# Simon-Kotchou/ViT.rs

Measured on AMD Instinct MI355X. Metric: images/sec (train step) ViT-B/16 224² bf16 at 1/2/4/8 MI355X; % MFMA roofline, higher is better.
Workload: dtype bf16; 1 GPU; vit_b16 224x224 train step (fwd+bwd+SGD), batch 256/GPU, bf16; model=vit_b16, global_batch=256, seq_len=197, parallelism=dp1

## Files before the change

include/vit_ops.h:

```cpp
#ifndef VIT_OPS_H
#define VIT_OPS_H

#include <stddef.h>
#include <stdint.h>

#ifdef __cplusplus
extern "C" {
#endif

int vit_init(int device);
void vit_set_stream(void* hip_stream);
void* vit_get_stream(void);
int vit_sync(void);
int vit_last_error(const char** msg);
void vit_clear_error(void);
void* vit_malloc(size_t bytes);
void vit_free(void* p);
int vit_memcpy_h2d(void* dst, const void* src, size_t bytes);
int vit_memcpy_d2h(void* dst, const void* src, size_t bytes);
int vit_memcpy_d2d(void* dst, const void* src, size_t bytes);
int vit_memset(void* dst, int value, size_t bytes);
enum {
    VIT_HIT_GEMM_128 = 0,
    VIT_HIT_GEMM_256x256 = 16,
    VIT_HIT_GEMM_256x128 = 32,
    VIT_HIT_GEMM_FP8 = 48,
    VIT_HIT_GEMM_F32 = 64,
    VIT_HIT_SPLITK_REDUCE = 80,
    VIT_HIT_ATTN_FWD_MFMA = 81,
    VIT_HIT_ATTN_BWD_PERSISTENT = 82,
    VIT_HIT_ATTN_BWD_ONEPASS = 83,
    VIT_HIT_ATTN_BWD_PAIR = 84,
    VIT_HIT_ATTN_GENERIC = 85,
    VIT_HIT_ATTN_BWD_XKEY = 86,
    VIT_HIT_QUANT_ROWCOL = 87,
    VIT_HIT_GEMM_PP = 88,
    VIT_HIT_LN_MX = 89,
    VIT_HIT_LNB_MX = 90,
    VIT_HIT_AUGMENT = 91,
    VIT_HIT_COUNT = 96
};
int vit_kernel_hits(long long* out, int n);
void vit_kernel_hits_reset(void);
void* vit_event_create(void);
void vit_event_destroy(void* ev);
int vit_event_record(void* ev);
float vit_event_elapsed_ms(void* start, void* stop);

void residual_forward(float* out, const float* inp1, const float* inp2, int N);
void matmul_forward(float* out, const float* inp, const float* weight, const float* bias,
                    int B, int T, int C, int OC);
void attention_forward(float* out, float* preatt, float* att, const float* inp,
                       int B, int T, int C, int NH);
void layernorm_forward(float* out, float* mean, float* rstd, const float* inp,
                       const float* weight, const float* bias, int B, int T, int C);
void gelu_forward(float* out, const float* inp, int N);
void softmax_forward(float* probs, const float* logits, int B, int T, int V);
void crossentropy_forward(float* losses, const float* probs, const int* targets,
                          int B, int T, int V);
void residual_backward(float* dinp1, float* dinp2, const float* dout, int N);
void matmul_backward(float* dinp, float* dweight, float* dbias, const float* dout,
                     const float* inp, const float* weight, int B, int T, int C, int OC);
void attention_backward(float* dinp, float* dpreatt, float* datt, const float* dout,
                        const float* inp, const float* att, int B, int T, int C, int NH);
void layernorm_backward(float* dinp, float* dweight, float* dbias, const float* dout,
                        const float* inp, const float* weight, const float* mean,
                        const float* rstd, int B, int T, int C);
void gelu_backward(float* dinp, const float* inp, const float* dout, int N);
void crossentropy_softmax_backward(float* dlogits, const float* dlosses, const float* probs,
                                   const int* targets, int B, int T, int V);
void softmax_crossentropy_soft_forward(float* probs, float* losses, const float* logits,
                                       const int* ta, const int* tb, float lam, float eps,
                                       int B, int T, int V);
void crossentropy_soft_softmax_backward(float* dlogits, const float* dlosses, const float* probs,
                                        const int* ta, const int* tb, float lam, float eps,
                                        int B, int T, int V);
void patch_embed_forward(float* encoded, const float* pixels, const float* patch_w,
                         const float* patch_b, const float* cls, const float* wpe,
                         int B, int IMG, int P, int C);
void patch_embed_backward(float* dpatch_w, float* dpatch_b, float* dcls, float* dwpe,
                          const float* dencoded, const float* pixels, int B, int IMG, int P,
                          int C);
void sgd_step(float* params, const float* grads, long long n, float lr);
void grad_sumsq(double* out, const float* x, long long n);

void matmul_forward_bf16(uint16_t* out, const uint16_t* inp, const uint16_t* weight,
                         const float* bias, int B, int T, int C, int OC);
void matmul_backward_bf16(float* dinp, float* dweight, float* dbias, const uint16_t* dout,
                          const uint16_t* inp, const uint16_t* weight, int B, int T, int C,
                          int OC);
int vit_attention_kernel_kind(int T, int C, int NH);
void attention_forward_fused_bf16(uint16_t* out, float* lse, const uint16_t* inp,
                                  int B, int T, int C, int NH);
void attention_backward_fused_bf16(uint16_t* dinp, const uint16_t* dout, const uint16_t* inp,
                                   const uint16_t* out, const float* lse, int B, int T, int C,
                                   int NH);
void attention_backward_fused_bf16_ex(uint16_t* dinp, const uint16_t* dout, const uint16_t* inp,
                                      const uint16_t* out, const float* lse, int B, int T, int C, int NH,
                                      float* dqkv_bias);
void layernorm_forward_bf16(uint16_t* out, float* mean, float* rstd, const float* inp,
                            const float* weight, const float* bias, int B, int T, int C);
void layernorm_backward_bf16(float* dinp, float* dweight, float* dbias, const uint16_t* dout,
                             const float* inp, const float* weight, const float* mean,
                             const float* rstd, int B, int T, int C);
void gelu_forward_bf16(uint16_t* out, const uint16_t* inp, int N);
void gelu_backward_bf16(float* dinp, const uint16_t* inp, const uint16_t* dout, int N);
void gemm_bf16_ex(void* C, long long ldc, const uint16_t* A, long long lda, int a_kcontig,
                  const uint16_t* B, long long ldb, int b_kcontig, const float* bias,
                  float* dbias, int M, int N, int K, int epi, int splitk);
void gemm_bf16_fused(void* C, void* C2, long long ldc, const void* aux, long long ldaux,
                     const uint16_t* A, long long lda, int a_kcontig, const uint16_t* B,
                     long long ldb, int b_kcontig, const float* bias, float* colsum_out, int M,
                     int N, int K, int epi);
long long mx_scale_size(long long rows, int K);
void quantize_mx_bf16_ex(uint8_t* q, uint8_t* scales, const uint16_t* x, long long R, int K,
                         long long ldx, long long ldq);
void quantize_mx_f32_ex(uint8_t* q, uint8_t* scales, const float* x, long long R, int K,
                        long long ldx, long long ldq);
long long mx_cols_padded(long long R);
void quantize_mx_cols_bf16_ex(uint8_t* q, uint8_t* scales, const uint16_t* x, long long R, int C,
                              long long ldx);
void quantize_mx_rowcol_bf16_ex(uint8_t* qr, uint8_t* scales_r, uint8_t* qc, uint8_t* scales_c,
                                const uint16_t* x, long long R, int C, long long ldx, long long ldqc,
                                long long tok_off, long long ntok);
void layernorm_backward_stream(uint16_t* dres_out, uint8_t* lo_out, const uint16_t* dres_in, const uint8_t* lo_in,
                               float* dweight, float* dbias, float* dres_colsum, const uint16_t* dout, const float* inp,
                               const float* weight, const float* mean, const float* rstd, long long R, int C);
void layernorm_backward_stream_mx(uint16_t* dres_out, uint8_t* lo_out, const uint16_t* dres_in, const uint8_t* lo_in,
                                  float* dweight, float* dbias, float* dres_colsum, const uint16_t* dout,
                                  const float* inp, const float* weight, const float* mean, const float* rstd,
                                  long long R, int C, uint8_t* qr, uint8_t* scales_r, uint8_t* qc, uint8_t* scales_c,
                                  long long ldqc, long long tok_off, long long ntok);
void layernorm_forward_mx(uint8_t* qr, uint8_t* scales_r, uint8_t* qc, uint8_t* scales_c, float* mean,
                          float* rstd, const float* inp, const float* weight, const float* bias, long long R,
                          int C, long long ldqc, long long tok_off, long long ntok);
void gemm_fp8_fused(void* C, void* C2, long long ldc, const void* aux, long long ldaux,
                    const uint8_t* A, const uint8_t* a_scale, long long lda, const uint8_t* B,
                    const uint8_t* b_scale, long long ldb, const float* bias, float* colsum_out,
                    int M, int N, int K, int epi);
void gemm_fp8_fused_mx(void* C, void* C2, long long ldc, const void* aux, long long ldaux, const uint8_t* A,
                       const uint8_t* a_scale, long long lda, const uint8_t* B, const uint8_t* b_scale,
                       long long ldb, const float* bias, float* colsum_out, int M, int N, int K, int epi,
                       uint8_t* mx_q, uint8_t* mx_s);
void gemm_fp8_fused_mxc(void* C, void* C2, long long ldc, const void* aux, long long ldaux, const uint8_t* A,
                        const uint8_t* a_scale, long long lda, const uint8_t* B, const uint8_t* b_scale,
                        long long ldb, const float* bias, float* colsum_out, int M, int N, int K, int epi,
                        uint8_t* mx_q, uint8_t* mx_s, uint8_t* mxc_q, uint8_t* mxc_s, long long mxc_ld,
                        long long mxc_off);
void gemm_bf16_set_variant(int variant);
void gemm_bf16_set_debug(int flags);
void gemm_bf16_set_trace(unsigned long long* trace);
void convert_f32_to_bf16(uint16_t* out, const float* inp, long long n);
void convert_bf16_to_f32(float* out, const uint16_t* inp, long long n);

#ifdef __cplusplus
}
#endif
#endif
```

vit.rs_amd/__init__.py:

```python
import ctypes
import os
import sys

import numpy as np

HERE = os.path.dirname(os.path.abspath(__file__))
LIB_PATH = os.environ.get("VIT_LIB") or os.path.join(HERE, "libvit_hip.so")

from . import data
from . import mix
from . import groups
from . import augment

VIT_FP32, VIT_BF16, VIT_FP8 = 0, 1, 2
MIX_NONE, MIX_MIXUP, MIX_CUTMIX = 0, 1, 2
_lib = None


class VitError(RuntimeError):
    pass


class VitConfigC(ctypes.Structure):
    _fields_ = [("img", ctypes.c_int), ("patch", ctypes.c_int), ("in_ch", ctypes.c_int),
                ("channels", ctypes.c_int), ("num_layers", ctypes.c_int),
                ("num_heads", ctypes.c_int), ("num_classes", ctypes.c_int)]


class AdamWC(ctypes.Structure):
    _fields_ = [("beta1", ctypes.c_float), ("beta2", ctypes.c_float), ("eps", ctypes.c_float),
                ("weight_decay", ctypes.c_float)]


class CheckpointInfoC(ctypes.Structure):
    _fields_ = [("cfg", VitConfigC), ("num_params", ctypes.c_longlong), ("has_opt", ctypes.c_int),
                ("step", ctypes.c_int), ("adamw", AdamWC)]


def _cfg_c(cfg):
    return VitConfigC(cfg.img, cfg.patch, cfg.in_ch, cfg.channels, cfg.num_layers, cfg.num_heads,
                      cfg.num_classes)


def build(quiet=True):
    import subprocess
    jobs = str(min(8, os.cpu_count() or 1))
    subprocess.run(["make", "-s", "-j", jobs, "-C", HERE], check=True,
                   stdout=subprocess.DEVNULL if quiet else None)


_VOID = [("vit_clear_error", []), ("vit_set_stream", [ctypes.c_void_p]),
         ("vit_free", [ctypes.c_void_p]), ("vit_event_destroy", [ctypes.c_void_p]),
         ("vit_trainer_destroy", [ctypes.c_void_p]), ("vit_trainer_timing_reset", [ctypes.c_void_p]),
         ("vit_loader_close", [ctypes.c_void_p]), ("vit_jpeg_loader_close", [ctypes.c_void_p]), ("vit_kernel_hits_reset", [])]

P, I, LL, F, S = ctypes.c_void_p, ctypes.c_int, ctypes.c_longlong, ctypes.c_float, ctypes.c_size_t
_SIGS = {
    "vit_init": (I, [I]), "vit_get_stream": (P, []), "vit_sync": (I, []),
    "vit_last_error": (I, [ctypes.POINTER(ctypes.c_char_p)]),
    "vit_malloc": (P, [S]), "vit_memcpy_h2d": (I, [P, P, S]), "vit_memcpy_d2h": (I, [P, P, S]),
    "vit_memcpy_d2d": (I, [P, P, S]), "vit_memset": (I, [P, I, S]),
    "vit_event_create": (P, []), "vit_event_record": (I, [P]), "vit_event_elapsed_ms": (F, [P, P]),
    "residual_forward": (None, [P, P, P, I]),
    "matmul_forward": (None, [P, P, P, P, I, I, I, I]),
    "attention_forward": (None, [P, P, P, P, I, I, I, I]),
    "layernorm_forward": (None, [P, P, P, P, P, P, I, I, I]),
    "gelu_forward": (None, [P, P, I]),
    "softmax_forward": (None, [P, P, I, I, I]),
    "crossentropy_forward": (None, [P, P, P, I, I, I]),
    "residual_backward": (None, [P, P, P, I]),
    "matmul_backward": (None, [P, P, P, P, P, P, I, I, I, I]),
    "attention_backward": (None, [P, P, P, P, P, P, I, I, I, I]),
    "layernorm_backward": (None, [P, P, P, P, P, P, P, P, I, I, I]),
    "gelu_backward": (None, [P, P, P, I]),
    "crossentropy_softmax_backward": (None, [P, P, P, P, I, I, I]),
    "softmax_crossentropy_soft_forward": (None, [P, P, P, P, P, F, F, I, I, I]),
    "crossentropy_soft_softmax_backward": (None, [P, P, P, P, P, F, F, I, I, I]),
    "patch_embed_forward": (None, [P, P, P, P, P, P, I, I, I, I]),
    "patch_embed_backward": (None, [P, P, P, P, P, P, I, I, I, I]),
    "sgd_step": (None, [P, P, LL, F]),
    "grad_sumsq": (None, [P, P, LL]),
    "matmul_forward_bf16": (None, [P, P, P, P, I, I, I, I]),
    "matmul_backward_bf16": (None, [P, P, P, P, P, P, I, I, I, I]),
    "attention_forward_fused_bf16": (None, [P, P, P, I, I, I, I]),
    "vit_attention_kernel_kind": (I, [I, I, I]),
    "attention_backward_fused_bf16": (None, [P, P, P, P, P, I, I, I, I]),
    "attention_backward_fused_bf16_ex": (None, [P, P, P, P, P, I, I, I, I, P]),
    "layernorm_forward_bf16": (None, [P, P, P, P, P, P, I, I, I]),
    "layernorm_backward_bf16": (None, [P, P, P, P, P, P, P, P, I, I, I]),
    "gelu_forward_bf16": (None, [P, P, I]),
    "gelu_backward_bf16": (None, [P, P, P, I]),
    "gemm_bf16_ex": (None, [P, LL, P, LL, I, P, LL, I, P, P, I, I, I, I, I]),
    "gemm_bf16_fused": (None, [P, P, LL, P, LL, P, LL, I, P, LL, I, P, P, I, I, I, I]),
    "mx_scale_size": (LL, [LL, I]),
    "quantize_mx_bf16_ex": (None, [P, P, P, LL, I, LL, LL]),
    "quantize_mx_f32_ex": (None, [P, P, P, LL, I, LL, LL]),
    "mx_cols_padded": (LL, [LL]),
    "quantize_mx_cols_bf16_ex": (None, [P, P, P, LL, I, LL]),
    "quantize_mx_rowcol_bf16_ex": (None, [P, P, P, P, P, LL, I, LL, LL, LL, LL]),
    "layernorm_forward_mx": (None, [P, P, P, P, P, P, P, P, P, LL, I, LL, LL, LL]),
    "layernorm_backward_stream": (None, [P, P, P, P, P, P, P, P, P, P, P, P, LL, I]),
    "layernorm_backward_stream_mx": (None, [P, P, P, P, P, P, P, P, P, P, P, P, LL, I, P, P, P, P, LL, LL, LL]),
    "gemm_fp8_fused": (None, [P, P, LL, P, LL, P, P, LL, P, P, LL, P, P, I, I, I, I]),
    "gemm_fp8_fused_mx": (None, [P, P, LL, P, LL, P, P, LL, P, P, LL, P, P, I, I, I, I, P, P]),
    "gemm_fp8_fused_mxc": (None, [P, P, LL, P, LL, P, P, LL, P, P, LL, P, P, I, I, I, I, P, P, P, P, LL, LL]),
    "gemm_bf16_set_variant": (None, [I]), "gemm_bf16_set_debug": (None, [I]),
    "gemm_bf16_set_trace": (None, [P]),
    "vit_kernel_hits": (I, [P, I]),
    "convert_f32_to_bf16": (None, [P, P, LL]),
    "convert_bf16_to_f32": (None, [P, P, LL]),
    "vit_trainer_create": (P, [ctypes.POINTER(VitConfigC), I, I, I]),
    "vit_trainer_num_params": (LL, [P]), "vit_trainer_device_bytes": (LL, [P]),
    "vit_trainer_set_params": (I, [P, P]), "vit_trainer_get_params": (I, [P, P]),
    "vit_trainer_get_grads": (I, [P, P]), "vit_trainer_set_batch": (I, [P, P, P]),
    "vit_trainer_set_batch_device": (I, [P, P, P]),
    "vit_trainer_set_label_smoothing": (I, [P, F]),
    "vit_trainer_mix_batch": (I, [P, I, F, I, I, I, I]),
    "vit_trainer_get_pixels": (I, [P, P]),
    "vit_trainer_forward": (I, [P, I]), "vit_trainer_zero_grad": (I, [P]),
    "vit_trainer_backward": (I, [P]), "vit_trainer_step": (I, [P, F]),
    "vit_trainer_train_step": (I, [P, F, I]), "vit_trainer_mean_loss": (F, [P]),
    "vit_trainer_get_logits": (I, [P, P]), "vit_trainer_sync": (I, [P]),
    "vit_trainer_stream": (P, [P]),
    "vit_layout_query": (I, [ctypes.POINTER(VitConfigC), P, P, ctypes.POINTER(LL)]),
    "vit_dp_unique_id_size": (I, []), "vit_dp_get_unique_id": (I, [ctypes.c_char_p]),
    "vit_trainer_dp_init": (I, [P, I, I, ctypes.c_char_p, I]),
    "vit_trainer_dp_ranks": (I, [P]),
    "vit_trainer_get_dp_snapshot": (I, [P, P]),
    "vit_trainer_set_timing": (I, [P, I]), "vit_trainer_set_concurrency": (I, [P, I]),
    "vit_trainer_set_option": (I, [P, ctypes.c_char_p, I]),
    "vit_trainer_timing": (I, [P, ctypes.POINTER(ctypes.c_char_p), ctypes.POINTER(ctypes.c_double),
                               ctypes.POINTER(ctypes.c_longlong), ctypes.POINTER(ctypes.c_double), I]),
    "vit_trainer_step_adamw": (I, [P, F, F, F, F, F]),
    "vit_trainer_get_adamw_state": (I, [P, P, P, ctypes.POINTER(I)]),
    "vit_trainer_set_grad_clip": (I, [P, F]), "vit_trainer_grad_norm": (F, [P]),
    "vit_trainer_set_param_groups": (I, [P, P, P]),
    "vit_trainer_get_param_groups": (I, [P, P, P, ctypes.POINTER(I)]),
    "vit_trainer_eval": (I, [P, P, ctypes.POINTER(I)]),
    "vit_config_num_params": (LL, [ctypes.POINTER(VitConfigC)]),
    "vit_checkpoint_read_info": (I, [ctypes.c_char_p, P]),
    "vit_checkpoint_write": (I, [ctypes.c_char_p, ctypes.POINTER(VitConfigC), P, P, P, I, P]),
    "vit_checkpoint_read": (I, [ctypes.c_char_p, ctypes.POINTER(VitConfigC), P, P, P]),
    "vit_loader_open": (P, [ctypes.c_char_p, ctypes.c_char_p, I, I, ctypes.c_ulonglong, I, I, I, I, I]),
    "vit_loader_num_records": (LL, [P]), "vit_loader_steps_per_epoch": (I, [P]),
    "vit_loader_next": (I, [P, ctypes.POINTER(P), ctypes.POINTER(P), ctypes.POINTER(LL), ctypes.POINTER(I)]),
    "vit_trainer_set_batch_u8": (I, [P, P, P, P, P]),
    "vit_augment_u8": (I, [P, I, I, P, I, P, P]),
    "vit_randaugment_draw": (I, [ctypes.c_ulonglong, LL, I, I, I, P]),
    "vit_trainer_set_augment_plan": (I, [P, P, I, P]),
    "vit_jpeg_probe": (I, [P, LL, ctypes.POINTER(I), ctypes.POINTER(I), ctypes.POINTER(I)]),
    "vit_jpeg_coefficients": (I, [P, LL, P, LL, P]),
    "vit_jpeg_loader_open": (P, [ctypes.c_char_p, ctypes.c_char_p, ctypes.c_char_p, I, ctypes.c_ulonglong, I, I,
                                 I, I, I, I]),
    "vit_jpeg_loader_num_records": (LL, [P]), "vit_jpeg_loader_steps_per_epoch": (I, [P]),
    "vit_jpeg_loader_next": (I, [P, ctypes.POINTER(P), ctypes.POINTER(LL), ctypes.POINTER(I)]),
    "vit_jpeg_loader_boxes": (I, [P, P]),
    "vit_jpeg_loader_decode_u8": (I, [P, P, I]),
    "vit_trainer_set_batch_jpeg": (I, [P, P, P, P]),
    "vit_jpeg_loader_set_randaugment": (I, [P, I, I, P]),
    "vit_jpeg_loader_plan": (I, [P, I, P, ctypes.POINTER(I)]),
    "vit_trainer_save_checkpoint": (I, [P, ctypes.c_char_p]),
    "vit_trainer_load_checkpoint": (I, [P, ctypes.c_char_p]),
}


def exported_symbols():
    return sorted(set(_SIGS) | {n for n, _ in _VOID})


def lib():
    global _lib
    if _lib is not None:
        return _lib
    if not os.path.exists(LIB_PATH):
        raise VitError(f"{LIB_PATH} not built; run __graft_entry__.build() or make -C vit.rs_amd")
    L = ctypes.CDLL(LIB_PATH, mode=ctypes.RTLD_GLOBAL)
    for name, (res, args) in _SIGS.items():
        if os.environ.get("VIT_LIB") and not hasattr(L, name):
            continue
        f = getattr(L, name)
        f.restype = res
        f.argtypes = args
    for name, args in _VOID:
        f = getattr(L, name)
        f.restype = None
        f.argtypes = args
    _lib = L
    return L


HIT_GEMM_128, HIT_GEMM_256x256, HIT_GEMM_256x128, HIT_GEMM_FP8, HIT_GEMM_F32 = 0, 16, 32, 48, 64
HIT_SPLITK_REDUCE, HIT_ATTN_FWD_MFMA, HIT_ATTN_BWD_PERSISTENT = 80, 81, 82
HIT_ATTN_BWD_ONEPASS, HIT_ATTN_BWD_PAIR, HIT_ATTN_GENERIC = 83, 84, 85
HIT_ATTN_BWD_XKEY, HIT_QUANT_ROWCOL = 86, 87
HIT_GEMM_PP = 88
HIT_LN_MX = 89
HIT_LNB_MX = 90
HIT_AUGMENT = 91


def kernel_hits():
    n = lib().vit_kernel_hits(None, 0)
    out = (ctypes.c_longlong * n)()
    lib().vit_kernel_hits(ctypes.cast(out, ctypes.c_void_p), n)
    return np.array(out[:], dtype=np.int64)


def kernel_hits_reset():
    lib().vit_kernel_hits_reset()


def check(what=""):
    msg = ctypes.c_char_p()
    if lib().vit_last_error(ctypes.byref(msg)):
        text = msg.value.decode() if msg.value else "unknown"
        lib().vit_clear_error()
        raise VitError(f"{what}: {text}" if what else text)


class DeviceArray:

    def __init__(self, shape, dtype):
        self.shape = tuple(shape) if isinstance(shape, (tuple, list)) else (int(shape),)
        self.dtype = np.dtype(dtype)
        self.nbytes = int(np.prod(self.shape)) * self.dtype.itemsize
        self.ptr = lib().vit_malloc(max(self.nbytes, 16))
        if not self.ptr:
            check("vit_malloc")
            raise VitError("vit_malloc returned NULL")

    @classmethod
    def from_numpy(cls, a, dtype=None):
        a = np.ascontiguousarray(a if dtype is None else a.astype(dtype))
        d = cls(a.shape, a.dtype)
        d.upload(a)
        return d

    @classmethod
    def zeros(cls, shape, dtype):
        d = cls(shape, dtype)
        lib().vit_memset(d.ptr, 0, d.nbytes)
        check("vit_memset")
        return d

    def upload(self, a):
        a = np.ascontiguousarray(a, dtype=self.dtype)
# ... 485 lines not shown
```

vit.rs_amd/csrc/gemm.h:

```cpp
#pragma once
#include "common.h"

namespace vit {

enum Epi {
    EPI_F32_STORE = 0,
    EPI_F32_ACC = 1,
    EPI_F32_ATOMIC = 2,
    EPI_BF16_STORE = 3,
    EPI_BF16_GELU = 4,
    EPI_F32_RESID = 5,
    EPI_BF16_DGELU = 6,
    EPI_F32_SLAB = 7,
    EPI_BF16_GELU_D = 8,
    EPI_BF16_MUL = 9,
};
constexpr bool epi_aux16(int e) { return e == EPI_BF16_DGELU || e == EPI_BF16_MUL; }
constexpr bool epi_bias(int e) { return e != EPI_F32_ATOMIC && e != EPI_F32_SLAB && !epi_aux16(e); }
constexpr bool epi_mx(int e) { return e == EPI_BF16_GELU || e == EPI_BF16_GELU_D || epi_aux16(e); }

struct GemmArgs {
    const void* A = nullptr;
    long long lda = 0;
    bool a_kcontig = true;
    const void* B = nullptr;
    long long ldb = 0;
    bool b_kcontig = true;
    void* C = nullptr;
    long long ldc = 0;
    void* C2 = nullptr;
    const void* aux = nullptr;
    long long ldaux = 0;
    const float* bias = nullptr;
    float* dbias = nullptr;
    float* colsum_out = nullptr;
    float* colsum_part = nullptr;
    int M = 0, N = 0, K = 0;
    int epi = EPI_F32_STORE;
    int splitk = 0;
    int fill_pct = 0;
    bool rows_gathered = false;
    float* ws = nullptr;
    size_t ws_bytes = 0;
    const void* a_scale = nullptr;
    const void* b_scale = nullptr;
    uint8_t* mx_q = nullptr;
    uint8_t* mx_s = nullptr;
    uint8_t* mxc_q = nullptr;
    uint8_t* mxc_s = nullptr;
    long long mxc_ld = 0;
    long long mxc_off = 0;
};

void gemm_f32(const GemmArgs& a, hipStream_t s);
void gemm_bf16(const GemmArgs& a, hipStream_t s);
bool gemm_bf16_supported(const GemmArgs& a);
void gemm_set_variant(int v);
void gemm_set_debug(int flags);
int gemm_cu_count();
int gemm_persist_grid();
struct GemmParams;
void gemm_set_trace(unsigned long long* trace);
bool gemm_pp_shape(const GemmArgs& a);
void gemm_bf16_pp(const GemmArgs& a, const GemmParams& p, hipStream_t s);
int gemm_colsum_rows(const GemmArgs& a, bool fp8);
bool gemm_streaming();

void gemm_fp8(const GemmArgs& a, hipStream_t s);
bool gemm_fp8_supported(const GemmArgs& a);
void quantize_mx_bf16(uint8_t* q, uint8_t* sl, const bf16_t* x, long long R, int K, long long ldx,
                      long long ldq, hipStream_t s);
void quantize_mx_f32(uint8_t* q, uint8_t* sl, const float* x, long long R, int K, long long ldx,
                     long long ldq, hipStream_t s);
void quantize_mx_batched_bf16(uint8_t* q, uint8_t* sl, const bf16_t* x, long long R, int K, int count,
                              long long xs, long long qs, long long ss, hipStream_t s);
void quantize_mx_batched_f32(uint8_t* q, uint8_t* sl, const float* x, long long R, int K, int count,
                             long long xs, long long qs, long long ss, hipStream_t s);
void quantize_mx_cols_bf16(uint8_t* q, uint8_t* sl, const bf16_t* x, long long R, int C, long long ldx, hipStream_t s);
void quantize_mx_cols_batched_bf16(uint8_t* q, uint8_t* sl, const bf16_t* x, long long R, int C, long long ldx,
                                   int count, long long xs, long long qs, long long ss, hipStream_t s);
bool quantize_mx_rowcol_bf16(uint8_t* qr, uint8_t* slr, uint8_t* qc, uint8_t* slc, const bf16_t* x, long long R,
                             int C, long long ldx, long long ldqc, long long tok_off, long long ntok, hipStream_t s);
long long mx_cols_kp(long long R);
long long mx_rows_padded(long long rows);
size_t mx_scale_bytes(long long rows, int K);
bool ln_forward_mx_supported(int C);
bool ln_backward_mx_supported(int C);
bool ln_backward_bf16_stream_mx(bf16_t* dres_out, uint8_t* lo_out, const bf16_t* dres_in, const uint8_t* lo_in,
                                float* dw, float* db, float* dres_colsum, const bf16_t* dout, const float* inp,
                                const float* w, const float* mean, const float* rstd, long long R, int C,
                                hipStream_t s, float* part, uint8_t* qr, uint8_t* slr, uint8_t* qc, uint8_t* slc,
                                long long ldqc, long long tok_off, long long ntok, uint8_t* scratch);
size_t ln_backward_mx_scratch_bytes(int C);
bool ln_forward_mx(uint8_t* qr, uint8_t* slr, uint8_t* qc, uint8_t* slc, float* mean, float* rstd, const float* x,
                   const float* w, const float* b, long long R, int C, long long ldqc, long long tok_off, long long ntok,
                   hipStream_t s, uint8_t* scratch);
size_t ln_mx_scratch_bytes(int C);

void colsum_f32(float* dbias, const float* X, int M, int N, long long ld, hipStream_t s, float* ws = nullptr);
void colsum_bf16(float* dbias, const bf16_t* X, int M, int N, long long ld, hipStream_t s, float* ws = nullptr);
struct RowsJob {
    float* dst;
    const float* src;
    int nrows;
    long long ld;
    int ncols;
};
constexpr int ROWS_MAX_JOBS = 8;
void rows_reduce_add(const RowsJob* jobs, int njobs, hipStream_t s);

}
```

vit.rs_amd/csrc/gemm.hip:

```cpp
#include "gemm_common.h"

#include <cstdlib>

#ifndef VIT_G2_ONEPHASE
#define VIT_G2_ONEPHASE 0
#endif

namespace vit {

namespace bf {
constexpr int BM = 128, BN = 128, BK = 64, NT = 256;
constexpr int SK = 72;
constexpr int SMN = 144;
constexpr int TILE = 9216;
static_assert(BM * SK == TILE && BK * SMN == TILE, "image sizes");

template <bool KC, int ROWS>
struct Stager {
    uint4 r[4];
    __device__ __forceinline__ void load(const bf16_t* __restrict__ base, long long ld, int row0,
                                         int rows_lim, int k0, int k_lim, int tid) {
#pragma unroll
        for (int c = 0; c < 4; c++) {
            const int idx = c * NT + tid;
// ... 470 lines not shown
        bar();
        if (lagging) {
            __builtin_amdgcn_s_setprio(1);
            bar();
        }
        for (int kt = 0; kt < nk; kt++) {
            const char* img = smem + sl * SLOT_BYTES;
            const int sl2 = (sl + 2) & 3;
#pragma unroll
            for (int b = 0; b < 4; b++) fb[b] = frag<true>(img + IMG_BYTES, wn * 64 + b * 16, lane);
#pragma unroll
            for (int a = 0; a < 4; a++) alo[a] = frag<true>(img, wm * 128 + a * 16, lane);
#if VIT_G2_ONEPHASE
#pragma unroll
            for (int a = 0; a < 4; a++) ahi[a] = frag<true>(img, wm * 128 + (4 + a) * 16, lane);
            issue_a(kt + 2, sl2, more);
            issue_b(kt + 2, sl2, more);
            if (kt > 0 || j == 0) {
                if (kt + 2 < nk || more) wait_vm(4);
                else wait_vm(0);
            }
            bar();
            mfma_half(0, alo, fb);
            mfma_half(1, ahi, fb);
            bar();
            sl = (sl + 1) & 3;
            continue;
#endif
            issue_a(kt + 2, sl2, more);
            bar();
            mfma_half(0, alo, fb);
            bar();
#pragma unroll
            for (int a = 0; a < 4; a++) ahi[a] = frag<true>(img, wm * 128 + (4 + a) * 16, lane);
            if (kt > 0 || j == 0) {
                if (kt + 2 < nk || more) wait_vm(2);
                else wait_vm(0);
            }
            issue_b(kt + 2, sl2, more);
            bar();
            mfma_half(1, ahi, fb);
            bar();
            sl = (sl + 1) & 3;
        }
        if (!lagging) bar();
        if (p.trace && tid == 0) p.trace[(long long)cur.t * TRACE_WORDS + 1] = __builtin_amdgcn_s_memrealtime();
        float bpre[8];
        staged_bias_prefetch<EPI>(p, lane, cur.tn0 + wn * 64, bpre);
#if VIT_G2_EPI_WAIT_ASM
        asm volatile("s_waitcnt vmcnt(0) lgkmcnt(0)" ::: "memory");
#else
        __builtin_amdgcn_s_waitcnt(0x0070);
#endif
        __builtin_amdgcn_s_setprio(0);
        __builtin_amdgcn_s_barrier();
        asm volatile("" ::: "memory");
        if (!skip_epilogue(p, acc)) {
            char* stg = smem + ((wave < 4 ? sl + 2 : sl + 3) & 3) * SLOT_BYTES + (wave & 3) * 8192;
            staged_epilogue_q<EPI>(p, acc, reinterpret_cast<float*>(stg), lane, cur.tm0 + wm * 128,
                                   cur.tn0 + wn * 64, bpre);
        }
        if (p.trace && (tid & 63) == 0) {
            const long long rec = (long long)cur.t * TRACE_WORDS;
            const unsigned long long t = __builtin_amdgcn_s_memrealtime();
            p.trace[rec + 4 + wave] = t;
            if (wave == 0) {
                p.trace[rec + 2] = t;
                p.trace[rec + 3] = ((unsigned long long)__builtin_amdgcn_s_getreg((31 << 11) | 20) << 32) |
                                   __builtin_amdgcn_s_getreg((31 << 11) | 4);
            }
        }
        if (p.dbg & 16) asm volatile("s_waitcnt vmcnt(0)" ::: "memory");
        zero_acc();
        if (more) tile_src(j + 1, cur);
        if (j + 2 < my_tiles) tile_src(j + 2, nxt);
    }
}

}

namespace g4 {
constexpr int BM = 256, BN = 128, BK = 32, NT = 256;
constexpr int NSLOT = 3;
constexpr int A_BYTES = BM * BK * 2;
constexpr int B_BYTES = BN * BK * 2;
constexpr int SLOT_BYTES = A_BYTES + B_BYTES;
constexpr int KTILE = BK;
constexpr int PIECES = BM / 64 + BN / 64;
static_assert(PIECES == 6, "vmcnt literal below");
static_assert(NSLOT * SLOT_BYTES >= 4 * STG_WAVE_BYTES, "staged epilogue area");

template <int R>
__device__ __forceinline__ int mn_swz(int k) {
    if constexpr (R == 256) return ((k & 3) << 2) | (((k >> 3) & 1) << 1);
    else return ((k & 3) << 1) | (((k >> 3) & 1) << 3);
}

template <int R>
__device__ __forceinline__ void stage(const bf16_t* __restrict__ base, long long ld, int row0,
                                      int rows_lim, int k0, char* img, int wave, int lane) {
#pragma unroll
    for (int j = 0; j < R / 64; j++) {
        const int blk = j * 4 + wave;
        constexpr int CPR = R / 8;
        constexpr int KPB = 64 / CPR;
        const int k = blk * KPB + lane / CPR;
        const int c = (lane % CPR) ^ mn_swz<R>(k);
        const int gc = min(row0 + c * 8, rows_lim - 8);
        const bf16_t* src = base + (long long)(k0 + k) * ld + gc;
        __builtin_amdgcn_global_load_lds((const __attribute__((address_space(1))) void*)src,
                                         (__attribute__((address_space(3))) void*)(img + blk * 1024),
                                         16, 0, 0);
    }
}

template <int R>
__device__ __forceinline__ bf16x8_t frag(const char* img, int r0, int lane) {
    const int i = lane & 15, g = lane >> 4;
    const int q = i >> 2, p = i & 3;
    const int ch = (r0 >> 3) + (p >> 1);
    const int k0 = 8 * g + q, k1 = k0 + 4;
    (void)k1;
    const char* a0 = img + k0 * (2 * R) + ((ch ^ mn_swz<R>(k0)) << 4) + (p & 1) * 8;
    const bf16x4_t lo = ds_read_tr16_asm<0>(a0);
    const bf16x4_t hi = ds_read_tr16_asm<4 * 2 * R>(a0);
    return __builtin_shufflevector(lo, hi, 0, 1, 2, 3, 4, 5, 6, 7);
}

__device__ __forceinline__ void group_order(int t, int ntm, int ntn, int& tm, int& tn) {
    constexpr int GM = 8;
    const int per = GM * ntn;
    const int grp = t / per;
    const int first = grp * GM;
    const int gsz = min(GM, ntm - first);
    const int r = t - grp * per;
    tm = first + r % gsz;
    tn = r / gsz;
}

template <int EPI>
__global__ __launch_bounds__(NT, 2) void gemm_kernel(GemmParams p) {
    __shared__ __attribute__((aligned(1024))) char smem[NSLOT * SLOT_BYTES];
    first_round_stagger(p.stagger);
    const int tid = threadIdx.x, lane = tid & 63;
    const int wave = __builtin_amdgcn_readfirstlane(tid >> 6);
    const int wm = wave >> 1, wn = wave & 1;
    const int ntm = cdiv(p.M, BM), ntn = cdiv(p.N, BN);
    int tm, tn, wg, split;
    split_remap(ntm * ntn, wg, split);
    group_order(wg, ntm, ntn, tm, tn);
    const int tm0 = tm * BM, tn0 = tn * BN;
    const int kbeg = split * p.kchunk;
    const int kend = min(p.K, kbeg + p.kchunk);
    const int nk = (kend - kbeg) / BK;
    const bf16_t* A = (const bf16_t*)p.A;
    const bf16_t* B = (const bf16_t*)p.B;

    f32x4_t acc[8][4];
#pragma unroll
    for (int a = 0; a < 8; a++)
#pragma unroll
        for (int b = 0; b < 4; b++) acc[a][b] = f32x4_t{0.f, 0.f, 0.f, 0.f};

    auto issue = [&](int st) {
        char* sl = smem + (st % NSLOT) * SLOT_BYTES;
        const int k0 = kbeg + st * BK;
        stage<BM>(A, p.lda, tm0, p.M, k0, sl, wave, lane);
        stage<BN>(B, p.ldb, tn0, p.N, k0, sl + A_BYTES, wave, lane);
    };
    if (nk > 0) issue(0);
    if (nk > 1) issue(1);
    for (int kt = 0; kt < nk; kt++) {
        __builtin_amdgcn_sched_barrier(0);
        if (kt + 1 < nk) asm volatile("s_waitcnt vmcnt(6)" ::: "memory");
        else asm volatile("s_waitcnt vmcnt(0)" ::: "memory");
        asm volatile("s_waitcnt lgkmcnt(0)" ::: "memory");
        __builtin_amdgcn_s_barrier();
        asm volatile("" ::: "memory");
        __builtin_amdgcn_sched_barrier(0);
        if (kt + 2 < nk) issue(kt + 2);
        const char* img = smem + (kt % NSLOT) * SLOT_BYTES;
        bf16x8_t fa[8], fb[4];
#pragma unroll
        for (int b = 0; b < 4; b++) fb[b] = frag<BN>(img + A_BYTES, wn * 64 + b * 16, lane);
#pragma unroll
        for (int a = 0; a < 8; a++) fa[a] = frag<BM>(img, wm * 128 + a * 16, lane);
        __builtin_amdgcn_sched_barrier(0);
        asm volatile("s_waitcnt lgkmcnt(0)" ::: "memory");
        __builtin_amdgcn_sched_barrier(0);
#pragma unroll
        for (int a = 0; a < 8; a++)
#pragma unroll
            for (int b = 0; b < 4; b++)
                acc[a][b] = __builtin_amdgcn_mfma_f32_16x16x32_bf16(fb[b], fa[a], acc[a][b], 0, 0, 0);
    }

    if (skip_epilogue(p, acc)) return;
    asm volatile("s_waitcnt vmcnt(0) lgkmcnt(0)" ::: "memory");
    __builtin_amdgcn_s_barrier();
    asm volatile("" ::: "memory");
    staged_epilogue<EPI>(p, acc, smem + wave * STG_WAVE_BYTES, lane, tm0 + wm * 128, tn0 + wn * 64);
}
}

namespace f32 {
constexpr int BM = 64, BN = 64, BK = 16, NT = 256, S = 80;

template <int EPI>
__global__ __launch_bounds__(NT) void gemm_f32_kernel(GemmParams p, int a_kc, int b_kc) {
    __shared__ float As[BK * S];
    __shared__ float Bs[BK * S];
    const int tid = threadIdx.x, lane = tid & 63, wave = tid >> 6;
    const int wm = wave >> 1, wn = wave & 1;
    const int ntm = cdiv(p.M, BM), ntn = cdiv(p.N, BN);
    const int wg = blockIdx.x;
    const int tm0 = (wg / ntn) * BM, tn0 = (wg % ntn) * BN;
    (void)ntm;
    const int kbeg = blockIdx.y * p.kchunk;
    const int kend = min(p.K, kbeg + p.kchunk);
    const float* A = (const float*)p.A;
    const float* B = (const float*)p.B;
    f32x4_t acc[2][2];
#pragma unroll
    for (int a = 0; a < 2; a++)
#pragma unroll
        for (int b = 0; b < 2; b++) acc[a][b] = f32x4_t{0.f, 0.f, 0.f, 0.f};

    for (int k0 = kbeg; k0 < kend; k0 += BK) {
#pragma unroll
        for (int e = 0; e < 4; e++) {
            const int idx = e * NT + tid;
            int m, k;
            if (a_kc) { m = idx >> 4; k = idx & 15; } else { k = idx >> 6; m = idx & 63; }
            const int gm = tm0 + m, gk = k0 + k;
            float v = 0.f;
            if (gm < p.M && gk < kend)
                v = a_kc ? A[(long long)gm * p.lda + gk] : A[(long long)gk * p.lda + gm];
            As[k * S + m] = v;
            int n;
            if (b_kc) { n = idx >> 4; k = idx & 15; } else { k = idx >> 6; n = idx & 63; }
            const int gn = tn0 + n;
            const int gk2 = k0 + k;
            float w = 0.f;
            if (gn < p.N && gk2 < kend)
                w = b_kc ? B[(long long)gn * p.ldb + gk2] : B[(long long)gk2 * p.ldb + gn];
            Bs[k * S + n] = w;
        }
        __syncthreads();
#pragma unroll
        for (int kk = 0; kk < BK / 4; kk++) {
            const int kr = kk * 4 + (lane >> 4);
            float af[2], bfv[2];
#pragma unroll
            for (int t = 0; t < 2; t++) {
                af[t] = As[kr * S + wm * 32 + t * 16 + (lane & 15)];
                bfv[t] = Bs[kr * S + wn * 32 + t * 16 + (lane & 15)];
            }
#pragma unroll
            for (int a = 0; a < 2; a++)
#pragma unroll
                for (int b = 0; b < 2; b++)
                    acc[a][b] = __builtin_amdgcn_mfma_f32_16x16x4f32(af[a], bfv[b], acc[a][b], 0, 0, 0);
        }
        __syncthreads();
    }
#pragma unroll
    for (int a = 0; a < 2; a++)
#pragma unroll
        for (int b = 0; b < 2; b++)
#pragma unroll
            for (int r = 0; r < 4; r++) {
                const int m = tm0 + wm * 32 + a * 16 + (lane >> 4) * 4 + r;
                const int n = tn0 + wn * 32 + b * 16 + (lane & 15);
                if (m >= p.M || n >= p.N) continue;
                float v = acc[a][b][r];
                float* q = (float*)p.C + (long long)m * p.ldc + n;
                if constexpr (EPI == EPI_F32_STORE) {
                    *q = p.bias ? v + p.bias[n] : v;
                } else if constexpr (EPI == EPI_F32_ACC) {
                    *q += p.bias ? v + p.bias[n] : v;
                } else {
                    q[(long long)blockIdx.y * p.M * p.ldc] = v;
                }
            }
}
}

template <typename TX>
__global__ __launch_bounds__(256) void colsum_part_k(float* __restrict__ out, const TX* __restrict__ X, int M, int N,
                                                     long long ld, int rpb, int add_direct) {
    const int n = blockIdx.x * 256 + threadIdx.x;
    const int r0 = blockIdx.y * rpb;
    const int r1 = min(M, r0 + rpb);
    if (n >= N) return;
    float s = 0.f;
    for (int r = r0; r < r1; r++) {
        if constexpr (sizeof(TX) == 2)
            s += bf2f(X[(long long)r * ld + n]);
        else
            s += X[(long long)r * ld + n];
    }
    if (add_direct) out[n] += s;
    else out[(long long)blockIdx.y * N + n] = s;
}

struct RowsJobs {
    RowsJob j[ROWS_MAX_JOBS];
    int blk0[ROWS_MAX_JOBS + 1];
    int vec;
};
__global__ __launch_bounds__(256) void rows_reduce_k(RowsJobs jobs) {
    __shared__ float4 red[16][17];
    int jb = 0;
#pragma unroll 1
    while (jb + 1 < ROWS_MAX_JOBS && (int)blockIdx.x >= jobs.blk0[jb + 1]) jb++;
    const RowsJob& J = jobs.j[jb];
    const int c0 = (blockIdx.x - jobs.blk0[jb]) * 64;
    if (jobs.vec) {
        const int q = threadIdx.x & 15, ph = threadIdx.x >> 4, c = c0 + 4 * q;
        float4 s0 = make_float4(0.f, 0.f, 0.f, 0.f), s1 = s0;
        if (c < J.ncols) {
            const float* base = J.src + c;
            int r = ph;
            for (; r + 16 < J.nrows; r += 32) {
                const float4 a = *reinterpret_cast<const float4*>(base + (long long)r * J.ld);
                const float4 b = *reinterpret_cast<const float4*>(base + (long long)(r + 16) * J.ld);
                s0.x += a.x; s0.y += a.y; s0.z += a.z; s0.w += a.w;
                s1.x += b.x; s1.y += b.y; s1.z += b.z; s1.w += b.w;
            }
            if (r < J.nrows) {
                const float4 a = *reinterpret_cast<const float4*>(base + (long long)r * J.ld);
                s0.x += a.x; s0.y += a.y; s0.z += a.z; s0.w += a.w;
            }
        }
        red[ph][q] = make_float4(s0.x + s1.x, s0.y + s1.y, s0.z + s1.z, s0.w + s1.w);
        __syncthreads();
        if (threadIdx.x < 64) {
            const int qq = threadIdx.x >> 2, e = threadIdx.x & 3, cc = c0 + threadIdx.x;
            float t = 0.f;
#pragma unroll
            for (int p = 0; p < 16; p++) t += reinterpret_cast<const float*>(&red[p][qq])[e];
            if (cc < J.ncols) J.dst[cc] += t;
        }
        return;
    }
    float* reds = reinterpret_cast<float*>(red);
    const int c = c0 + (threadIdx.x & 63), ph = threadIdx.x >> 6;
    float s0 = 0.f, s1 = 0.f;
    if (c < J.ncols) {
        int r = ph;
        for (; r + 4 < J.nrows; r += 8) {
            s0 += J.src[(long long)r * J.ld + c];
            s1 += J.src[(long long)(r + 4) * J.ld + c];
        }
        if (r < J.nrows) s0 += J.src[(long long)r * J.ld + c];
    }
    reds[ph * 64 + (threadIdx.x & 63)] = s0 + s1;
    __syncthreads();
    if (ph == 0 && c < J.ncols)
        J.dst[c] += ((reds[threadIdx.x] + reds[64 + threadIdx.x]) + reds[128 + threadIdx.x]) + reds[192 + threadIdx.x];
}
void rows_reduce_add(const RowsJob* jobs, int njobs, hipStream_t s) {
    for (int b = 0; b < njobs; b += ROWS_MAX_JOBS) {
        RowsJobs J{};
        J.vec = 1;
        int nb = 0, k = 0;
        for (; k < ROWS_MAX_JOBS && b + k < njobs; k++) {
            const RowsJob& x = jobs[b + k];
            J.j[k] = x;
            J.blk0[k] = nb;
            nb += x.nrows > 0 ? cdiv(x.ncols, 64) : 0;
            if (x.nrows > 0 && ((x.ncols | x.ld) % 4 || ((uintptr_t)x.src & 15))) J.vec = 0;
        }
        for (; k <= ROWS_MAX_JOBS; k++) J.blk0[k] = nb;
        if (nb == 0) continue;
        rows_reduce_k<<<nb, 256, 0, s>>>(J);
        after_launch("rows_reduce_add");
    }
}
template <typename TX>
static void colsum_any(float* dbias, const TX* X, int M, int N, long long ld, hipStream_t s, float* ws) {
    if (M <= 0 || N <= 0) return;
    if constexpr (sizeof(TX) == 4) {
        if (M <= 1024) {
            RowsJob j{dbias, X, M, ld, N};
            rows_reduce_add(&j, 1, s);
            return;
        }
    }
    const int rpb = 256, nch = cdiv(M, rpb);
    if (nch == 1) {
        colsum_part_k<TX><<<dim3(cdiv(N, 256), 1), 256, 0, s>>>(dbias, X, M, N, ld, rpb, 1);
        after_launch("colsum");
        return;
    }
    if (!ws) ws = (float*)workspace((size_t)nch * N * sizeof(float));
    if (!ws) return;
    colsum_part_k<TX><<<dim3(cdiv(N, 256), nch), 256, 0, s>>>(ws, X, M, N, ld, rpb, 0);
    after_launch("colsum");
    RowsJob j{dbias, ws, nch, N, N};
    rows_reduce_add(&j, 1, s);
}
static int gemm_variant();
static int g_debug_flags_fwd();
static bool pp_all() { return (g_debug_flags_fwd() & 512) != 0; }
static bool pp_taken(const GemmArgs& a) {
    return gemm_variant() == 11 && !a.a_scale && a.epi != EPI_F32_ATOMIC && gemm_bf16_supported(a) &&
           a.K % g2::KTILE == 0 && a.M >= 256 && a.N >= 256 && (a.N <= 1280 || pp_all()) && gemm_pp_shape(a);
}
int gemm_colsum_rows(const GemmArgs& a, bool fp8) { return cdiv(a.M, !fp8 && pp_taken(a) ? 96 : 128); }
float* colsum_rows_begin(const GemmArgs& a) {
    if (!epi_aux16(a.epi) || !(a.colsum_out || a.colsum_part)) return nullptr;
    float* r = a.colsum_part ? a.colsum_part
                             : (float*)workspace((size_t)gemm_colsum_rows(a, a.a_scale != nullptr) * a.N * sizeof(float));
    return r;
}
void colsum_rows_end(const GemmArgs& a, float* rows, hipStream_t s) {
    if (!rows || !a.colsum_out) return;
    RowsJob j{a.colsum_out, rows, gemm_colsum_rows(a, a.a_scale != nullptr), a.N, a.N};
    rows_reduce_add(&j, 1, s);
}

__global__ __launch_bounds__(256) void slab_reduce1_k(float* __restrict__ C, long long ldc,
                                                      const float* __restrict__ slab, int M, int N,
                                                      int splits) {
    const long long n1 = (long long)M * N;
    for (long long e = blockIdx.x * 256LL + threadIdx.x; e < n1; e += (long long)gridDim.x * 256) {
        const int m = (int)(e / N), n = (int)(e - (long long)m * N);
        float acc = slab[e];
        for (int z = 1; z < splits; z++) acc += slab[z * n1 + e];
        C[(long long)m * ldc + n] += acc;
    }
}
__global__ __launch_bounds__(256) void slab_reduce_k(float* __restrict__ C, long long ldc,
                                                     const float* __restrict__ slab, int M, int N,
                                                     int splits) {
    const long long n4 = (long long)M * N / 4;
    const long long plane = (long long)M * N;
    for (long long i = blockIdx.x * 256LL + threadIdx.x; i < n4; i += (long long)gridDim.x * 256) {
        const long long e = i * 4;
        const int m = (int)(e / N), n = (int)(e - (long long)m * N);
        float4 acc = reinterpret_cast<const float4*>(slab)[i];
        for (int z = 1; z < splits; z++) {
            const float4 t = *reinterpret_cast<const float4*>(slab + z * plane + e);
            acc.x += t.x; acc.y += t.y; acc.z += t.z; acc.w += t.w;
        }
        float4* c = reinterpret_cast<float4*>(C + (long long)m * ldc + n);
        float4 o = *c;
        o.x += acc.x; o.y += acc.y; o.z += acc.z; o.w += acc.w;
        *c = o;
    }
}

static int g_variant = -1;
static int g_debug_flags = 0;
static bool known_variant(int v) { return v == 1 || v == 2 || v == 7 || v == 11; }
static constexpr int kDefaultVariant = 7;
static int gemm_variant() {
    if (g_variant < 0) {
        const char* e = getenv("VIT_GEMM");
        g_variant = e ? atoi(e) : kDefaultVariant;
        if (!known_variant(g_variant)) g_variant = kDefaultVariant;
    }
    return g_variant;
}
void gemm_set_variant(int v) { g_variant = known_variant(v) ? v : -1; }
int gemm_cu_count() {
    static int n = [] {
        int dev = 0, cu = 0;
        (void)hipGetDevice(&dev);
        (void)hipDeviceGetAttribute(&cu, hipDeviceAttributeMultiprocessorCount, dev);
        return cu > 0 ? cu : 256;
    }();
    return n;
}
int gemm_persist_grid() {
    static const int n = [] {
        const char* e = getenv("VIT_PERSIST_CUS");
        const int v = e ? atoi(e) : 0;
        return v >= 64 && v <= gemm_cu_count() ? v : gemm_cu_count();
    }();
    return n;
}
bool gemm_streaming() { return gemm_variant() == 7 || gemm_variant() == 11; }
void gemm_set_debug(int flags) { g_debug_flags = flags; }
static int g_debug_flags_fwd() { return g_debug_flags; }
static unsigned long long* g_trace = nullptr;
void gemm_set_trace(unsigned long long* trace) { g_trace = trace; }

GemmParams make_gemm_params(const GemmArgs& a, int kchunk) {
    GemmParams p;
    p.A = a.A; p.B = a.B; p.C = a.C; p.C2 = a.C2; p.aux = a.aux; p.bias = a.bias; p.dbias = a.dbias; p.colsum_out = nullptr;
    p.lda = a.lda; p.ldb = a.ldb; p.ldc = a.ldc; p.ldaux = a.ldaux;
    if (g_debug_flags & 32) p.ldc = 0;
    p.M = a.M; p.N = a.N; p.K = a.K; p.kchunk = kchunk;
    p.no_epi = (g_debug_flags & 2) ? 1 : 0;
    p.dbg = g_debug_flags & 0xF0;
    static const int gm_env = [] {
        const char* e = getenv("VIT_GEMM_GM");
        return e && *e ? atoi(e) : -1;
    }();
    const int gm_dbg = (g_debug_flags >> 16) & 0xF;
    p.gm = gm_dbg ? gm_dbg - 1 : gm_env >= 0 ? gm_env : (a.K <= 768 ? 8 : 0);
    p.stagger = ((g_debug_flags >> 8) & 0xFF) * 50;
    p.trace = g_trace;
    p.mx_q = a.mx_q;
    p.mx_s = a.mx_s;
    p.mx_rg = (int)(mx_rows_padded(a.M) / 32);
    p.mxc_q = a.mxc_q;
    p.mxc_s = a.mxc_s;
    p.mxc_ld = a.mxc_ld;
    p.mxc_off = (int)a.mxc_off;
    p.mxc_rg = (int)(mx_rows_padded(a.N) / 32);
    p.tiles = 1;
    return p;
}

int choose_split_waves(int tiles, int nk) {
    const int slots = 256;
    int best = 1;
    double best_eff = 0.0;
    for (int s = 1; s <= 32 && nk / s >= 16; s++) {
        const int blocks = tiles * s;
        const int waves = (blocks + slots - 1) / slots;
        const double eff = (double)blocks / (waves * (double)slots) * (blocks >= slots / 2 ? 1.0 : blocks / (slots / 2.0));
        if (eff > best_eff + 1e-9) { best_eff = eff; best = s; }
        if (eff >= 0.9) break;
    }
    return best;
}

static int choose_split(int tiles, int K, int ktile, int want_blocks) {
    int nk = cdiv(K, ktile);
    int s = 1;
    while (tiles * s < want_blocks && nk / (s * 2) >= 8) s *= 2;
    return s;
}

static int grid_blocks(long long n) {
    long long b = (n + 255) / 256;
    return (int)(b < 1 ? 1 : (b > 4096 ? 4096 : b));
}
float* slab_buffer(const GemmArgs& a, int split) {
    const size_t need = (size_t)split * a.M * a.N * sizeof(float);
    float* slab = a.ws ? (a.ws_bytes >= need ? a.ws : nullptr) : (float*)workspace(need);
    if (!slab) set_error("gemm: split-K workspace of %zu bytes unavailable", need);
    return slab;
}
void slab_reduce(const GemmArgs& a, float* slab, int split, hipStream_t s) {
    if (a.N % 4 == 0)
        slab_reduce_k<<<grid_blocks((long long)a.M * a.N / 4), 256, 0, s>>>((float*)a.C, a.ldc, slab, a.M, a.N, split);
    else
        slab_reduce1_k<<<grid_blocks((long long)a.M * a.N), 256, 0, s>>>((float*)a.C, a.ldc, slab, a.M, a.N, split);
    after_launch("gemm_slab_reduce");
    count_hit(VIT_HIT_SPLITK_REDUCE);
}

void gemm_f32(const GemmArgs& a, hipStream_t s) {
    if (a.M <= 0 || a.N <= 0) return;
    if (a.mx_q || a.mxc_q) {
        set_error("gemm_f32: the fused MX output is an fp8-engine feature");
        return;
    }
    const int tiles = cdiv(a.M, f32::BM) * cdiv(a.N, f32::BN);
    int split = 1;
    if (a.epi == EPI_F32_ATOMIC) split = a.splitk > 0 ? a.splitk : choose_split(tiles, a.K, f32::BK, 512);
    int kchunk = cdiv(cdiv(a.K, split), f32::BK) * f32::BK;
    if (kchunk <= 0) kchunk = f32::BK;
    split = cdiv(a.K > 0 ? a.K : 1, kchunk);
    GemmArgs b = a;
    float* slab = nullptr;
    if (a.epi == EPI_F32_ATOMIC) {
        if (split > 1) {
            if (!(slab = slab_buffer(a, split))) return;
            b.epi = EPI_F32_SLAB; b.C = slab; b.ldc = a.N;
        } else {
            b.epi = EPI_F32_ACC;
        }
    }
    GemmParams p = make_gemm_params(b, kchunk);
    dim3 grid(tiles, split);
    int akc = a.a_kcontig, bkc = a.b_kcontig;
    switch (b.epi) {
        case EPI_F32_STORE: f32::gemm_f32_kernel<EPI_F32_STORE><<<grid, f32::NT, 0, s>>>(p, akc, bkc); break;
        case EPI_F32_ACC: f32::gemm_f32_kernel<EPI_F32_ACC><<<grid, f32::NT, 0, s>>>(p, akc, bkc); break;
        case EPI_F32_SLAB: f32::gemm_f32_kernel<EPI_F32_SLAB><<<grid, f32::NT, 0, s>>>(p, akc, bkc); break;
        default: set_error("gemm_f32: unsupported epilogue %d", a.epi); return;
    }
    after_launch("gemm_f32");
    count_hit(VIT_HIT_GEMM_F32 + b.epi);
    if (slab) slab_reduce(a, slab, split, s);
}

bool gemm_bf16_supported(const GemmArgs& a) {
    auto al16 = [](const void* q) { return ((uintptr_t)q & 15) == 0; };
    if ((a.a_kcontig || a.b_kcontig) && a.K % 8) return false;
    if (a.lda % 8 || a.ldb % 8 || a.N % 4 || a.ldc % 4) return false;
    if (!al16(a.A) || !al16(a.B)) return false;
    if (!a.a_kcontig && a.M % 8) return false;
    if (!a.b_kcontig && a.N % 8) return false;
    return true;
}

template <bool AK, bool BKC>
static void launch_bf16(const GemmArgs& a, const GemmParams& p, dim3 grid, hipStream_t s) {
    switch (a.epi) {
#define VIT_CASE(E) \
    case E: bf::gemm_bf16_kernel<AK, BKC, E><<<grid, bf::NT, 0, s>>>(p); break;
        VIT_CASE(EPI_F32_STORE)
        VIT_CASE(EPI_F32_ACC)
        VIT_CASE(EPI_F32_SLAB)
        VIT_CASE(EPI_BF16_STORE)
        VIT_CASE(EPI_BF16_GELU)
        VIT_CASE(EPI_F32_RESID)
        VIT_CASE(EPI_BF16_DGELU)
        VIT_CASE(EPI_BF16_GELU_D)
        VIT_CASE(EPI_BF16_MUL)
#undef VIT_CASE
        default: set_error("gemm_bf16: unsupported epilogue %d", a.epi); return;
    }
}

template <bool AK, bool BKC>
static void launch_g2(const GemmArgs& a, const GemmParams& p, dim3 grid, hipStream_t s) {
    if constexpr (AK && BKC) {
        if ((gemm_variant() == 7 || gemm_variant() == 11) && grid.y == 1 && p.K >= 2 * g2::BK &&
            (long long)p.M * p.lda * 2 < (1LL << 31) &&
            (long long)p.N * p.ldb * 2 < (1LL << 31)) {
            const int cus = gemm_persist_grid();
            const dim3 pg((int)grid.x < cus ? grid.x : cus);
            switch (a.epi) {
#define VIT_CASE(E) \
    case E: g2::gemm_kernel_s<E><<<pg, g2::NT, 0, s>>>(p); return;
                VIT_CASE(EPI_F32_STORE)
                VIT_CASE(EPI_F32_ACC)
                VIT_CASE(EPI_BF16_STORE)
                VIT_CASE(EPI_BF16_GELU)
                VIT_CASE(EPI_F32_RESID)
                VIT_CASE(EPI_BF16_DGELU)
                VIT_CASE(EPI_BF16_GELU_D)
                VIT_CASE(EPI_BF16_MUL)
#undef VIT_CASE
                default: break;
            }
        }
    }
    switch (a.epi) {
#define VIT_CASE(E) \
    case E: g2::gemm_kernel<AK, BKC, E, 2><<<grid, g2::NT, 0, s>>>(p); break;
        VIT_CASE(EPI_F32_STORE)
        VIT_CASE(EPI_F32_ACC)
        VIT_CASE(EPI_BF16_STORE)
        VIT_CASE(EPI_BF16_GELU)
        VIT_CASE(EPI_F32_RESID)
        VIT_CASE(EPI_BF16_DGELU)
        VIT_CASE(EPI_F32_SLAB)
        VIT_CASE(EPI_BF16_GELU_D)
        VIT_CASE(EPI_BF16_MUL)
#undef VIT_CASE
        default: set_error("gemm_bf16: unsupported epilogue %d", a.epi); return;
    }
}

static int choose_split_g4(int tiles, int nk, int fill_pct = 0) {
    static const int slots = [] {
        const char* e = getenv("VIT_G4_SLOTS");
        const int v = e ? atoi(e) : 512;
        return v >= 64 && v <= 2048 ? v : 512;
    }();
    static const bool one_round = [] {
        const char* e = getenv("VIT_G4_RULE");
        return !(e && e[0] == '0');
    }();
    static const double fill = [] {
        const char* e = getenv("VIT_G4_FILL");
        const int v = e ? atoi(e) : 45;
        return (v >= 20 && v <= 100 ? v : 45) / 100.0;
    }();
    if (one_round) {
        const double f = fill_pct > 0 ? fill_pct / 100.0 : fill;
        const int s1 = (int)((f * slots + tiles - 1) / tiles);
        if (s1 >= 1 && (long long)tiles * s1 <= slots && nk / s1 >= 32) return s1;
    }
    int best = 1;
    double best_eff = 0.0;
    for (int s = 1; s <= 64 && nk / s >= 32; s++) {
        const int blocks = tiles * s;
        const int rounds = (blocks + slots - 1) / slots;
        const double eff = (double)blocks / (rounds * (double)slots) * (blocks >= slots / 2 ? 1.0 : blocks / (slots / 2.0));
        if (eff > best_eff + 1e-9) { best_eff = eff; best = s; }
        if (eff >= 0.9) break;
    }
    return best;
}

static void gemm_bf16_g4(const GemmArgs& a, hipStream_t s) {
    const int tiles = cdiv(a.M, g4::BM) * cdiv(a.N, g4::BN);
    int split = a.splitk > 0 ? a.splitk : choose_split_g4(tiles, a.K / g4::KTILE, a.fill_pct);
    int kchunk = cdiv(cdiv(a.K, split), g4::KTILE) * g4::KTILE;
    split = cdiv(a.K, kchunk);
    GemmArgs b = a;
    float* slab = nullptr;
    if (split > 1) {
        if (!(slab = slab_buffer(a, split))) return;
        b.epi = EPI_F32_SLAB;
        b.C = slab;
        b.ldc = a.N;
    } else {
        b.epi = EPI_F32_ACC;
    }
    GemmParams p = make_gemm_params(b, kchunk);
    p.tiles = tiles;
    dim3 grid(tiles, split);
    if (slab) g4::gemm_kernel<EPI_F32_SLAB><<<grid, g4::NT, 0, s>>>(p);
    else g4::gemm_kernel<EPI_F32_ACC><<<grid, g4::NT, 0, s>>>(p);
    after_launch("gemm_bf16_256x128");
    count_hit(VIT_HIT_GEMM_256x128 + b.epi);
    if (slab) slab_reduce(a, slab, split, s);
    if (a.dbias) colsum_bf16(a.dbias, (const bf16_t*)a.A, a.K, a.M, a.lda, s);
}

void gemm_bf16(const GemmArgs& a, hipStream_t s) {
    if (a.M <= 0 || a.N <= 0) return;
    if (a.mx_q || a.mxc_q) {
        set_error("gemm_bf16: the fused MX output is an fp8-engine feature");
        return;
    }
    if (!gemm_bf16_supported(a)) {
        set_error("gemm_bf16: unsupported shape/alignment M=%d N=%d K=%d lda=%lld ldb=%lld",
                  a.M, a.N, a.K, a.lda, a.ldb);
        return;
    }
    if (gemm_variant() != 1 && a.epi == EPI_F32_ATOMIC && !a.a_kcontig && !a.b_kcontig &&
        a.K % g4::KTILE == 0 && a.M >= 256 && a.N >= 128 && a.N % 4 == 0 &&
        (a.splitk > 0 || !a.ws ||
         (size_t)choose_split_g4(cdiv(a.M, g4::BM) * cdiv(a.N, g4::BN), a.K / g4::KTILE) * a.M * a.N * sizeof(float) <=
             a.ws_bytes)) {
        gemm_bf16_g4(a, s);
        return;
    }
    const bool gathered = a.rows_gathered && a.M >= 1 && a.a_kcontig && a.epi != EPI_F32_ATOMIC;
    const bool big = a.K % g2::KTILE == 0 && (a.M >= 256 || gathered) && a.N >= 256 && gemm_variant() != 1;
    if (big) {
        const int tiles = cdiv(a.M, g2::BM) * cdiv(a.N, g2::BN);
        int split = 1;
        if (a.epi == EPI_F32_ATOMIC) split = a.splitk > 0 ? a.splitk : choose_split_waves(tiles, a.K / g2::KTILE);
        int kchunk = cdiv(cdiv(a.K, split), g2::KTILE) * g2::KTILE;
        split = cdiv(a.K, kchunk);
        GemmArgs b = a;
        float* slab = nullptr;
        if (a.epi == EPI_F32_ATOMIC) {
            if (split > 1) {
                if (!(slab = slab_buffer(a, split))) return;
                b.epi = EPI_F32_SLAB;
                b.C = slab;
                b.ldc = a.N;
            } else {
                b.epi = EPI_F32_ACC;
            }
        }
        GemmParams p = make_gemm_params(b, kchunk);
        p.tiles = tiles;
        float* cs_rows = colsum_rows_begin(a);
        if ((a.colsum_out || a.colsum_part) && epi_aux16(a.epi) && !cs_rows) return;
        p.colsum_out = cs_rows;
        const bool late_db = a.dbias && !a.a_kcontig && split > 1;
        if (late_db) p.dbias = nullptr;
        if (split == 1 && pp_taken(b)) {
            gemm_bf16_pp(b, p, s);
            after_launch("gemm_bf16_pp");
            count_hit(VIT_HIT_GEMM_256x256 + b.epi);
            count_hit(VIT_HIT_GEMM_PP);
            colsum_rows_end(a, cs_rows, s);
            return;
        }
        dim3 grid(tiles, split);
        if (a.a_kcontig && a.b_kcontig) launch_g2<true, true>(b, p, grid, s);
        else if (a.a_kcontig && !a.b_kcontig) launch_g2<true, false>(b, p, grid, s);
        else if (!a.a_kcontig && !a.b_kcontig) launch_g2<false, false>(b, p, grid, s);
        else launch_g2<false, true>(b, p, grid, s);
        after_launch("gemm_bf16_256");
        count_hit(VIT_HIT_GEMM_256x256 + b.epi);
        if (slab) slab_reduce(a, slab, split, s);
        colsum_rows_end(a, cs_rows, s);
        if (late_db) colsum_bf16(a.dbias, (const bf16_t*)a.A, a.K, a.M, a.lda, s);
        return;
    }
    const int tiles = cdiv(a.M, bf::BM) * cdiv(a.N, bf::BN);
    int split = 1;
    if (a.epi == EPI_F32_ATOMIC) split = a.splitk > 0 ? a.splitk : choose_split(tiles, a.K, bf::BK, 512);
    int kchunk = cdiv(cdiv(a.K, split), bf::BK) * bf::BK;
    if (kchunk <= 0) kchunk = bf::BK;
    split = cdiv(a.K > 0 ? a.K : 1, kchunk);
    GemmArgs b = a;
    float* slab = nullptr;
    if (a.epi == EPI_F32_ATOMIC) {
        if (split > 1) {
            if (!(slab = slab_buffer(a, split))) return;
            b.epi = EPI_F32_SLAB; b.C = slab; b.ldc = a.N;
        } else {
            b.epi = EPI_F32_ACC;
        }
    }
    GemmParams p = make_gemm_params(b, kchunk);
    const bool late_db = a.dbias && !a.a_kcontig && split > 1;
    if (late_db) p.dbias = nullptr;
    dim3 grid(tiles, split);
    if (a.a_kcontig && a.b_kcontig) launch_bf16<true, true>(b, p, grid, s);
    else if (a.a_kcontig && !a.b_kcontig) launch_bf16<true, false>(b, p, grid, s);
    else if (!a.a_kcontig && !a.b_kcontig) launch_bf16<false, false>(b, p, grid, s);
    else launch_bf16<false, true>(b, p, grid, s);
    after_launch("gemm_bf16");
    count_hit(VIT_HIT_GEMM_128 + b.epi);
    if (slab) slab_reduce(a, slab, split, s);
    if (late_db) colsum_bf16(a.dbias, (const bf16_t*)a.A, a.K, a.M, a.lda, s);
    if ((a.colsum_out || a.colsum_part) && epi_aux16(a.epi)) {
        float* rows = colsum_rows_begin(a);
        if (!rows) return;
        colsum_part_k<bf16_t><<<dim3(cdiv(a.N, 256), cdiv(a.M, 128)), 256, 0, s>>>(
            rows, (const bf16_t*)a.C, a.M, a.N, a.ldc, 128, 0);
        after_launch("colsum_rows");
        colsum_rows_end(a, rows, s);
    }
}

void colsum_f32(float* dbias, const float* X, int M, int N, long long ld, hipStream_t s, float* ws) {
    colsum_any(dbias, X, M, N, ld, s, ws);
}
void colsum_bf16(float* dbias, const bf16_t* X, int M, int N, long long ld, hipStream_t s, float* ws) {
    colsum_any(dbias, X, M, N, ld, s, ws);
}

}
```

vit.rs_amd/csrc/gemm_common.h:

```cpp
#pragma once
#include "gemm.h"

namespace vit {

struct GemmParams {
    const void* A;
    const void* B;
    void* C;
    void* C2;
    const void* aux;
    const float* bias;
    float* dbias;
    float* colsum_out;
    long long lda, ldb, ldc, ldaux;
    int M, N, K;
    int kchunk;
    int no_epi;
    int dbg;
    int stagger;
    unsigned long long* trace;
    int tiles;
    int gm;
    uint8_t* mx_q;
    uint8_t* mx_s;
    int mx_rg;
    uint8_t* mxc_q;
    uint8_t* mxc_s;
    long long mxc_ld;
    int mxc_off, mxc_rg;
};

__device__ __forceinline__ int mx_scale_byte(float amax) {
    if (!(amax > 0.f)) return 127;
    const uint32_t u = __float_as_uint(amax);
    const int e = (int)((u >> 23) & 0xff), mant = (int)(u & 0x7fffff);
    int s = e - 8 + (mant > 0x600000 ? 1 : 0);
    return s < 0 ? 0 : (s > 254 ? 254 : s);
}
__device__ __forceinline__ void mx_out8(const GemmParams& p, int m, int n, uint32_t w0, uint32_t w1, uint32_t w2,
                                        uint32_t w3, int lane) {
    const uint32_t w[4] = {w0, w1, w2, w3};
    float v[8];
#pragma unroll
    for (int e = 0; e < 4; e++) {
        v[2 * e] = __uint_as_float(w[e] << 16);
        v[2 * e + 1] = __uint_as_float(w[e] & 0xffff0000u);
    }
    float amax = 0.f;
#pragma unroll
    for (int j = 0; j < 8; j++) amax = fmaxf(amax, fabsf(v[j]));
    amax = fmaxf(amax, __shfl_xor(amax, 1, 64));
    amax = fmaxf(amax, __shfl_xor(amax, 2, 64));
    const int sb = mx_scale_byte(amax);
    if ((lane & 3) == 0) {
        const int kb = n >> 5;
        p.mx_s[((long long)(kb >> 1) * p.mx_rg + (m >> 5)) * 64 + (kb & 1) * 32 + (m & 31)] = (uint8_t)sb;
    }
    const float inv = __uint_as_float((uint32_t)(254 - sb) << 23);
    int t0 = __builtin_amdgcn_cvt_pk_fp8_f32(v[0] * inv, v[1] * inv, 0, false);
    t0 = __builtin_amdgcn_cvt_pk_fp8_f32(v[2] * inv, v[3] * inv, t0, true);
    int t1 = __builtin_amdgcn_cvt_pk_fp8_f32(v[4] * inv, v[5] * inv, 0, false);
    t1 = __builtin_amdgcn_cvt_pk_fp8_f32(v[6] * inv, v[7] * inv, t1, true);
    *reinterpret_cast<uint2*>(p.mx_q + (long long)m * p.N + n) = make_uint2((uint32_t)t0, (uint32_t)t1);
}

__device__ __forceinline__ void stage_back8(float* w, uint32_t w0, uint32_t w1, uint32_t w2, uint32_t w3) {
    typedef float f4 __attribute__((ext_vector_type(4)));
    *reinterpret_cast<f4*>(w) = f4{__uint_as_float(w0 << 16), __uint_as_float(w0 & 0xffff0000u),
                                   __uint_as_float(w1 << 16), __uint_as_float(w1 & 0xffff0000u)};
    *reinterpret_cast<f4*>(w + 4) = f4{__uint_as_float(w2 << 16), __uint_as_float(w2 & 0xffff0000u),
                                       __uint_as_float(w3 << 16), __uint_as_float(w3 & 0xffff0000u)};
}

float* colsum_rows_begin(const GemmArgs& a);
void colsum_rows_end(const GemmArgs& a, float* rows, hipStream_t s);
int choose_split_waves(int tiles, int nk);
float* slab_buffer(const GemmArgs& a, int split);
void slab_reduce(const GemmArgs& a, float* slab, int split, hipStream_t s);

__device__ __forceinline__ void split_remap(int tiles, int& tile, int& split) {
    const int nwg = gridDim.x * gridDim.y;
    const int l = xcd_remap(blockIdx.y * gridDim.x + blockIdx.x, nwg);
    split = l / tiles;
    tile = l - split * tiles;
}
__device__ __forceinline__ int split_index(int tiles) {
    int t, s;
    split_remap(tiles, t, s);
    return s;
}

typedef unsigned int epi_u32x4 __attribute__((ext_vector_type(4)));
__device__ __forceinline__ void epi_st16(const GemmParams&, void* q, epi_u32x4 v) {
    *reinterpret_cast<epi_u32x4*>(q) = v;
}
__device__ __forceinline__ epi_u32x4 epi_ld16(const GemmParams&, const void* q) {
    return *reinterpret_cast<const epi_u32x4*>(q);
}

__device__ __forceinline__ void first_round_stagger(int ticks, bool one_per_cu = false) {
    if (ticks <= 0) return;
    const int lin = blockIdx.y * gridDim.x + blockIdx.x;
    if (one_per_cu ? (lin >= 256 || !((lin >> 3) & 1)) : (lin < 256 || lin >= 512)) return;
    const uint64_t t0 = __builtin_amdgcn_s_memrealtime();
    while (__builtin_amdgcn_s_memrealtime() - t0 < (uint64_t)ticks) __builtin_amdgcn_s_sleep(8);
}

constexpr int TRACE_WORDS = 16;
__device__ __forceinline__ void trace_stamp(const GemmParams& p, int k) {
    if (!p.trace || (threadIdx.x & 63) != 0) return;
    const int w = threadIdx.x >> 6;
    if (w != 0 && k != 2) return;
    const long long rec = ((long long)blockIdx.y * gridDim.x + blockIdx.x) * TRACE_WORDS;
    const unsigned long long t = __builtin_amdgcn_s_memrealtime();
    if (k == 2) {
        p.trace[rec + 4 + w] = t;
        if (w != 0) return;
        const unsigned hw = __builtin_amdgcn_s_getreg((31 << 11) | 4);
        const unsigned xcc = __builtin_amdgcn_s_getreg((31 << 11) | 20);
        p.trace[rec + 3] = ((unsigned long long)xcc << 32) | hw;
    }
    p.trace[rec + k] = t;
}

template <int NA, int NB>
__device__ __forceinline__ bool skip_epilogue(const GemmParams& p, f32x4_t (&acc)[NA][NB]) {
    if (!(p.no_epi & 1)) return false;
#pragma unroll
    for (int a = 0; a < NA; a++)
#pragma unroll
        for (int b = 0; b < NB; b++) asm volatile("" ::"v"(acc[a][b]));
    return true;
}

template <int EPI>
__device__ __forceinline__ void epilogue(const GemmParams& p, int m, int n, f32x4_t& v) {
    static_assert(EPI != EPI_F32_ATOMIC, "split-K partials go through slabs");
    if constexpr (epi_bias(EPI)) {
        if (p.bias) {
            const float4 bb = *reinterpret_cast<const float4*>(p.bias + n);
            v[0] += bb.x; v[1] += bb.y; v[2] += bb.z; v[3] += bb.w;
        }
    }
    const long long off = (long long)m * p.ldc + n;
    if constexpr (EPI == EPI_F32_STORE) {
        *reinterpret_cast<float4*>((float*)p.C + off) = make_float4(v[0], v[1], v[2], v[3]);
    } else if constexpr (EPI == EPI_F32_ACC) {
        float4* q = reinterpret_cast<float4*>((float*)p.C + off);
        float4 o = *q;
        o.x += v[0]; o.y += v[1]; o.z += v[2]; o.w += v[3];
        *q = o;
    } else if constexpr (EPI == EPI_BF16_STORE) {
        *reinterpret_cast<uint2*>((bf16_t*)p.C + off) =
            make_uint2(pack_bf16x2(v[0], v[1]), pack_bf16x2(v[2], v[3]));
    } else if constexpr (EPI == EPI_BF16_GELU) {
        *reinterpret_cast<uint2*>((bf16_t*)p.C + off) =
            make_uint2(pack_bf16x2(v[0], v[1]), pack_bf16x2(v[2], v[3]));
        *reinterpret_cast<uint2*>((bf16_t*)p.C2 + off) =
            make_uint2(pack_bf16x2(gelu_fast_f(v[0]), gelu_fast_f(v[1])),
                       pack_bf16x2(gelu_fast_f(v[2]), gelu_fast_f(v[3])));
    } else if constexpr (EPI == EPI_F32_RESID) {
        const float4 r = *reinterpret_cast<const float4*>((const float*)p.aux +
                                                          (long long)m * p.ldaux + n);
        *reinterpret_cast<float4*>((float*)p.C + off) =
            make_float4(v[0] + r.x, v[1] + r.y, v[2] + r.z, v[3] + r.w);
    } else if constexpr (EPI == EPI_F32_SLAB) {
        float* slab = (float*)p.C + (long long)split_index(p.tiles) * p.M * p.ldc;
        *reinterpret_cast<float4*>(slab + off) = make_float4(v[0], v[1], v[2], v[3]);
    } else if constexpr (EPI == EPI_BF16_GELU_D) {
        float g[4], d[4];
#pragma unroll
        for (int j = 0; j < 4; j++) gelu_pair_fast_f(v[j], g[j], d[j]);
        *reinterpret_cast<uint2*>((bf16_t*)p.C + off) = make_uint2(pack_bf16x2(d[0], d[1]), pack_bf16x2(d[2], d[3]));
        *reinterpret_cast<uint2*>((bf16_t*)p.C2 + off) = make_uint2(pack_bf16x2(g[0], g[1]), pack_bf16x2(g[2], g[3]));
    } else if constexpr (epi_aux16(EPI)) {
#pragma clang fp contract(off)
        const uint2 h = *reinterpret_cast<const uint2*>((const bf16_t*)p.aux +
                                                        (long long)m * p.ldaux + n);
        const float x0 = __uint_as_float(h.x << 16), x1 = __uint_as_float(h.x & 0xffff0000u);
        const float x2 = __uint_as_float(h.y << 16), x3 = __uint_as_float(h.y & 0xffff0000u);
        if constexpr (EPI == EPI_BF16_DGELU) {
            v[0] *= gelu_grad_fast_f(x0); v[1] *= gelu_grad_fast_f(x1);
            v[2] *= gelu_grad_fast_f(x2); v[3] *= gelu_grad_fast_f(x3);
        } else {
            v[0] *= x0; v[1] *= x1; v[2] *= x2; v[3] *= x3;
        }
        *reinterpret_cast<uint2*>((bf16_t*)p.C + off) =
            make_uint2(pack_bf16x2(v[0], v[1]), pack_bf16x2(v[2], v[3]));
    }
}

template <int EPI, bool MX = true>
__device__ __forceinline__ void epilogue8(const GemmParams& p, int m, int n, float (&v)[8],
                                          float (&cs)[8], int lane = 0, float* wb = nullptr) {
    if constexpr (epi_bias(EPI)) {
        if (p.bias) {
            const float4 b0 = *reinterpret_cast<const float4*>(p.bias + n);
            const float4 b1 = *reinterpret_cast<const float4*>(p.bias + n + 4);
            v[0] += b0.x; v[1] += b0.y; v[2] += b0.z; v[3] += b0.w;
            v[4] += b1.x; v[5] += b1.y; v[6] += b1.z; v[7] += b1.w;
        }
    }
    const long long off = (long long)m * p.ldc + n;
    auto st_f32 = [&](float* q) {
        reinterpret_cast<float4*>(q)[0] = make_float4(v[0], v[1], v[2], v[3]);
        reinterpret_cast<float4*>(q)[1] = make_float4(v[4], v[5], v[6], v[7]);
    };
    auto pack8 = [&](const float (&w)[8]) {
        return make_uint4(pack_bf16x2(w[0], w[1]), pack_bf16x2(w[2], w[3]), pack_bf16x2(w[4], w[5]),
                          pack_bf16x2(w[6], w[7]));
    };
    if constexpr (EPI == EPI_F32_STORE) {
        st_f32((float*)p.C + off);
    } else if constexpr (EPI == EPI_F32_ACC) {
        float* q = (float*)p.C + off;
        const float4 o0 = reinterpret_cast<const float4*>(q)[0];
        const float4 o1 = reinterpret_cast<const float4*>(q)[1];
        v[0] += o0.x; v[1] += o0.y; v[2] += o0.z; v[3] += o0.w;
        v[4] += o1.x; v[5] += o1.y; v[6] += o1.z; v[7] += o1.w;
        st_f32(q);
    } else if constexpr (EPI == EPI_F32_SLAB) {
        st_f32((float*)p.C + (long long)split_index(p.tiles) * p.M * p.ldc + off);
    } else if constexpr (EPI == EPI_BF16_STORE) {
        *reinterpret_cast<uint4*>((bf16_t*)p.C + off) = pack8(v);
    } else if constexpr (EPI == EPI_BF16_GELU) {
        float gv[8];
#pragma unroll
        for (int j = 0; j < 8; j++) gv[j] = gelu_fast_f(v[j]);
        *reinterpret_cast<uint4*>((bf16_t*)p.C + off) = pack8(v);
        const uint4 g8 = pack8(gv);
        if (p.C2) *reinterpret_cast<uint4*>((bf16_t*)p.C2 + off) = g8;
        if constexpr (MX) {
            if (p.mx_q) mx_out8(p, m, n, g8.x, g8.y, g8.z, g8.w, lane);
            if (wb) stage_back8(wb, g8.x, g8.y, g8.z, g8.w);
        }
    } else if constexpr (EPI == EPI_F32_RESID) {
        const float* r = (const float*)p.aux + (long long)m * p.ldaux + n;
        const float4 r0 = reinterpret_cast<const float4*>(r)[0];
        const float4 r1 = reinterpret_cast<const float4*>(r)[1];
        v[0] += r0.x; v[1] += r0.y; v[2] += r0.z; v[3] += r0.w;
        v[4] += r1.x; v[5] += r1.y; v[6] += r1.z; v[7] += r1.w;
        st_f32((float*)p.C + off);
    } else if constexpr (EPI == EPI_BF16_GELU_D) {
        float gv[8], dv[8];
#pragma unroll
        for (int j = 0; j < 8; j++) gelu_pair_fast_f(v[j], gv[j], dv[j]);
        *reinterpret_cast<uint4*>((bf16_t*)p.C + off) = pack8(dv);
        const uint4 g8 = pack8(gv);
        if (p.C2) *reinterpret_cast<uint4*>((bf16_t*)p.C2 + off) = g8;
        if constexpr (MX) {
            if (p.mx_q) mx_out8(p, m, n, g8.x, g8.y, g8.z, g8.w, lane);
            if (wb) stage_back8(wb, g8.x, g8.y, g8.z, g8.w);
        }
    } else if constexpr (epi_aux16(EPI)) {
        const uint4 h = *reinterpret_cast<const uint4*>((const bf16_t*)p.aux + (long long)m * p.ldaux + n);
        const uint32_t hw[4] = {h.x, h.y, h.z, h.w};
        {
#pragma clang fp contract(off)
#pragma unroll
        for (int j = 0; j < 4; j++) {
            const float lo = __uint_as_float(hw[j] << 16), hi = __uint_as_float(hw[j] & 0xffff0000u);
            if constexpr (EPI == EPI_BF16_DGELU) {
                v[2 * j] *= gelu_grad_fast_f(lo);
                v[2 * j + 1] *= gelu_grad_fast_f(hi);
            } else {
                v[2 * j] *= lo;
                v[2 * j + 1] *= hi;
            }
        }
#pragma unroll
        for (int j = 0; j < 8; j++) cs[j] += v[j];
        }
        const uint4 d8 = pack8(v);
        if (p.C) *reinterpret_cast<uint4*>((bf16_t*)p.C + off) = d8;
        if constexpr (MX) {
            if (p.mx_q) mx_out8(p, m, n, d8.x, d8.y, d8.z, d8.w, lane);
            if (wb) stage_back8(wb, d8.x, d8.y, d8.z, d8.w);
        }
    }
}

constexpr int STG_LD = 68;
constexpr int STG_WAVE_BYTES = 64 * STG_LD * 4;
typedef unsigned int epi_u32x4v __attribute__((ext_vector_type(4)));
template <int EPI>
struct EpiAux {
    static constexpr bool AUX16 = epi_aux16(EPI);
    static constexpr bool AUX32 = EPI == EPI_F32_RESID || EPI == EPI_F32_ACC;
    static constexpr int N = AUX16 ? 8 : (AUX32 ? 16 : 0);
    epi_u32x4v ax[N > 0 ? N : 1];
    __device__ __forceinline__ void load(const GemmParams& p, int rr, int mrow, int n) {
        if constexpr (AUX16) {
#pragma unroll
            for (int it = 0; it < 8; it++)
                ax[it] = epi_ld16(p, (const bf16_t*)p.aux + (long long)(mrow + it * 8 + rr) * p.ldaux + n);
        } else if constexpr (AUX32) {
            const float* src = EPI == EPI_F32_RESID ? (const float*)p.aux : (const float*)p.C;
            const long long ld = EPI == EPI_F32_RESID ? p.ldaux : p.ldc;
#pragma unroll
            for (int it = 0; it < 8; it++) {
                const float* q = src + (long long)(mrow + it * 8 + rr) * ld + n;
                ax[2 * it] = epi_ld16(p, q);
                ax[2 * it + 1] = epi_ld16(p, q + 4);
            }
        }
    }
};
template <int EPI>
__device__ __forceinline__ void staged_pass_interior(const GemmParams& p, const float* st, int rr,
                                                     int cc, int mrow, int n, float (&cs)[8],
                                                     const float* bpre, const EpiAux<EPI>* pre = nullptr) {
    const int cc_lane = cc >> 3;
    typedef unsigned int u32x4 __attribute__((ext_vector_type(4)));
    float bv[8] = {0.f, 0.f, 0.f, 0.f, 0.f, 0.f, 0.f, 0.f};
    if constexpr (epi_bias(EPI)) {
        if (bpre) {
#pragma unroll
            for (int j = 0; j < 8; j++) bv[j] = bpre[j];
        } else if (p.bias) {
            const float4 b0 = *reinterpret_cast<const float4*>(p.bias + n);
            const float4 b1 = *reinterpret_cast<const float4*>(p.bias + n + 4);
            bv[0] = b0.x; bv[1] = b0.y; bv[2] = b0.z; bv[3] = b0.w;
            bv[4] = b1.x; bv[5] = b1.y; bv[6] = b1.z; bv[7] = b1.w;
        }
    }
    constexpr bool AUX16 = epi_aux16(EPI);
    constexpr bool AUX32 = EPI == EPI_F32_RESID || EPI == EPI_F32_ACC;
    EpiAux<EPI> own;
    if (!pre) own.load(p, rr, mrow, n);
    const u32x4* ax = pre ? pre->ax : own.ax;
    float* slab = nullptr;
    if constexpr (EPI == EPI_F32_SLAB) slab = (float*)p.C + (long long)split_index(p.tiles) * p.M * p.ldc;
#pragma unroll
    for (int it = 0; it < 8; it++) {
        const int r = it * 8 + rr;
        const f32x4_t lo = *reinterpret_cast<const f32x4_t*>(st + r * STG_LD + cc);
        const f32x4_t hi = *reinterpret_cast<const f32x4_t*>(st + r * STG_LD + cc + 4);
        float v[8] = {lo[0], lo[1], lo[2], lo[3], hi[0], hi[1], hi[2], hi[3]};
        const long long off = (long long)(mrow + r) * p.ldc + n;
#pragma unroll
        for (int j = 0; j < 8; j++) v[j] += bv[j];
        auto pack8 = [](const float (&w)[8]) {
            return u32x4{pack_bf16x2(w[0], w[1]), pack_bf16x2(w[2], w[3]), pack_bf16x2(w[4], w[5]),
                         pack_bf16x2(w[6], w[7])};
        };
        auto st_f32 = [&](float* q) {
            epi_st16(p, q, u32x4{__float_as_uint(v[0]), __float_as_uint(v[1]), __float_as_uint(v[2]), __float_as_uint(v[3])});
            epi_st16(p, q + 4, u32x4{__float_as_uint(v[4]), __float_as_uint(v[5]), __float_as_uint(v[6]), __float_as_uint(v[7])});
        };
        if constexpr (EPI == EPI_F32_STORE) {
            st_f32((float*)p.C + off);
        } else if constexpr (EPI == EPI_F32_SLAB) {
            st_f32(slab + off);
        } else if constexpr (AUX32) {
#pragma unroll
            for (int j = 0; j < 4; j++) {
                v[j] += __uint_as_float(ax[2 * it][j]);
                v[4 + j] += __uint_as_float(ax[2 * it + 1][j]);
            }
            st_f32((float*)p.C + off);
        } else if constexpr (EPI == EPI_BF16_STORE) {
            epi_st16(p, (bf16_t*)p.C + off, pack8(v));
        } else if constexpr (EPI == EPI_BF16_GELU) {
            float gv[8];
#pragma unroll
            for (int j = 0; j < 8; j++) gv[j] = gelu_fast_f(v[j]);
            epi_st16(p, (bf16_t*)p.C + off, pack8(v));
            const u32x4 g8 = pack8(gv);
            if (p.C2) epi_st16(p, (bf16_t*)p.C2 + off, g8);
            if (p.mx_q) mx_out8(p, mrow + r, n, g8[0], g8[1], g8[2], g8[3], cc_lane);
            if (p.mxc_q) stage_back8(const_cast<float*>(st) + r * STG_LD + cc, g8[0], g8[1], g8[2], g8[3]);
        } else if constexpr (EPI == EPI_BF16_GELU_D) {
            float gv[8], dv[8];
#pragma unroll
            for (int j = 0; j < 8; j++) gelu_pair_fast_f(v[j], gv[j], dv[j]);
            epi_st16(p, (bf16_t*)p.C + off, pack8(dv));
            const u32x4 g8 = pack8(gv);
            if (p.C2) epi_st16(p, (bf16_t*)p.C2 + off, g8);
            if (p.mx_q) mx_out8(p, mrow + r, n, g8[0], g8[1], g8[2], g8[3], cc_lane);
            if (p.mxc_q) stage_back8(const_cast<float*>(st) + r * STG_LD + cc, g8[0], g8[1], g8[2], g8[3]);
        } else if constexpr (AUX16) {
#pragma clang fp contract(off)
#pragma unroll
            for (int j = 0; j < 4; j++) {
                const float lo = __uint_as_float(ax[it][j] << 16), hi = __uint_as_float(ax[it][j] & 0xffff0000u);
                if constexpr (EPI == EPI_BF16_DGELU) {
                    v[2 * j] *= gelu_grad_fast_f(lo);
                    v[2 * j + 1] *= gelu_grad_fast_f(hi);
                } else {
                    v[2 * j] *= lo;
                    v[2 * j + 1] *= hi;
                }
            }
#pragma unroll
            for (int j = 0; j < 8; j++) cs[j] += v[j];
            const u32x4 d8 = pack8(v);
            if (p.C) epi_st16(p, (bf16_t*)p.C + off, d8);
            if (p.mx_q) mx_out8(p, mrow + r, n, d8[0], d8[1], d8[2], d8[3], cc_lane);
            if (p.mxc_q) stage_back8(const_cast<float*>(st) + r * STG_LD + cc, d8[0], d8[1], d8[2], d8[3]);
        }
    }
}

GemmParams make_gemm_params(const GemmArgs& a, int kchunk);

template <int EPI>
__device__ __forceinline__ void staged_pass(const GemmParams& p, const float* st, int lane, int m0,
                                            int n0, int pass, bool interior, float (&cs)[8],
                                            const float* bpre = nullptr, const EpiAux<EPI>* pre = nullptr) {
    const int rr = lane >> 3, cc = (lane & 7) * 8;
    if (interior) {
        staged_pass_interior<EPI>(p, st, rr, cc, m0 + pass * 64, n0 + cc, cs, bpre, pre);
        return;
    }
#pragma unroll
    for (int it = 0; it < 8; it++) {
        const int r = it * 8 + rr;
        float v[8];
        const f32x4_t lo = *reinterpret_cast<const f32x4_t*>(st + r * STG_LD + cc);
        const f32x4_t hi = *reinterpret_cast<const f32x4_t*>(st + r * STG_LD + cc + 4);
        v[0] = lo[0]; v[1] = lo[1]; v[2] = lo[2]; v[3] = lo[3];
        v[4] = hi[0]; v[5] = hi[1]; v[6] = hi[2]; v[7] = hi[3];
        const int m = m0 + pass * 64 + r, n = n0 + cc;
        if (m >= p.M) continue;
        if (n + 8 <= p.N) {
            epilogue8<EPI>(p, m, n, v, cs, lane,
                           epi_mx(EPI) && p.mxc_q ? const_cast<float*>(st) + r * STG_LD + cc : nullptr);
        } else if (n + 4 <= p.N) {
            f32x4_t t = lo;
            epilogue<EPI>(p, m, n, t);
            if constexpr (epi_aux16(EPI)) {
#pragma clang fp contract(off)
                cs[0] += t[0];
                cs[1] += t[1];
                cs[2] += t[2];
                cs[3] += t[3];
            }
        }
    }
}
__device__ __forceinline__ void mx_cols_pass(const GemmParams& p, const float* st, int lane, int mrow, int n0) {
    if (mrow >= p.M) return;
    typedef unsigned int u32x4 __attribute__((ext_vector_type(4)));
    const int c = n0 + lane;
#pragma unroll
    for (int b = 0; b < 2; b++) {
        float v[32];
        float amax = 0.f;
#pragma unroll
        for (int i = 0; i < 32; i++) {
            v[i] = st[(32 * b + i) * STG_LD + lane];
            amax = fmaxf(amax, fabsf(v[i]));
        }
        const int sb = mx_scale_byte(amax);
        const int tok = p.mxc_off + mrow + 32 * b, kb = tok >> 5;
        p.mxc_s[((long long)(kb >> 1) * p.mxc_rg + (c >> 5)) * 64 + (kb & 1) * 32 + (c & 31)] = (uint8_t)sb;
        const float inv = __uint_as_float((uint32_t)(254 - sb) << 23);
        uint32_t w[8];
#pragma unroll
        for (int j = 0; j < 8; j++) {
            int t = __builtin_amdgcn_cvt_pk_fp8_f32(v[4 * j] * inv, v[4 * j + 1] * inv, 0, false);
            t = __builtin_amdgcn_cvt_pk_fp8_f32(v[4 * j + 2] * inv, v[4 * j + 3] * inv, t, true);
            w[j] = (uint32_t)t;
        }
        uint8_t* dst = p.mxc_q + (long long)c * p.mxc_ld + tok;
        *reinterpret_cast<u32x4*>(dst) = u32x4{w[0], w[1], w[2], w[3]};
        *reinterpret_cast<u32x4*>(dst + 16) = u32x4{w[4], w[5], w[6], w[7]};
    }
}
template <int EPI>
__device__ __forceinline__ bool staged_interior(const GemmParams& p, int m0, int n0) {
    return EPI != EPI_F32_ATOMIC && m0 + 128 <= p.M && n0 + 64 <= p.N;
}
template <int EPI>
__device__ __forceinline__ void staged_colsum(const GemmParams& p, int lane, int m0, int n0, float (&cs)[8]) {
    if constexpr (epi_aux16(EPI)) {
        if (p.colsum_out) {
            const int rr = lane >> 3, cc = (lane & 7) * 8;
#pragma unroll
            for (int j = 0; j < 8; j++) {
                float t = cs[j];
                t += __shfl_xor(t, 8, 64);
                t += __shfl_xor(t, 16, 64);
                t += __shfl_xor(t, 32, 64);
                cs[j] = t;
            }
            if (rr == 0 && m0 < p.M) {
#pragma unroll
                for (int j = 0; j < 8; j++)
                    if (n0 + cc + j < p.N) p.colsum_out[(long long)(m0 >> 7) * p.N + n0 + cc + j] = cs[j];
            }
        }
    }
}

template <int EPI>
__device__ __forceinline__ void staged_bias_prefetch(const GemmParams& p, int lane, int n0, float (&bv)[8]) {
#pragma unroll
    for (int j = 0; j < 8; j++) bv[j] = 0.f;
    if constexpr (epi_bias(EPI)) {
        const int n = n0 + (lane & 7) * 8;
        if (p.bias && n + 8 <= p.N) {
            const float4 b0 = *reinterpret_cast<const float4*>(p.bias + n);
            const float4 b1 = *reinterpret_cast<const float4*>(p.bias + n + 4);
            bv[0] = b0.x; bv[1] = b0.y; bv[2] = b0.z; bv[3] = b0.w;
            bv[4] = b1.x; bv[5] = b1.y; bv[6] = b1.z; bv[7] = b1.w;
        }
    }
}
template <int EPI>
__device__ __forceinline__ void staged_epilogue(const GemmParams& p, f32x4_t (&acc)[8][4],
                                                char* stage, int lane, int m0, int n0,
                                                const float* bpre = nullptr) {
    float* st = reinterpret_cast<float*>(stage);
    const int i = lane & 15, g = lane >> 4;
    float cs[8] = {0.f, 0.f, 0.f, 0.f, 0.f, 0.f, 0.f, 0.f};
    const bool interior = staged_interior<EPI>(p, m0, n0);
    auto stage_pass = [&](int pass) {
#pragma unroll
        for (int a = 0; a < 4; a++)
#pragma unroll
            for (int b = 0; b < 4; b++)
                *reinterpret_cast<f32x4_t*>(st + (a * 16 + i) * STG_LD + b * 16 + 4 * g) = acc[pass * 4 + a][b];
    };
    if (interior && EpiAux<EPI>::N > 0) {
        const int rr = lane >> 3, n = n0 + (lane & 7) * 8;
        EpiAux<EPI> a0, a1;
        a0.load(p, rr, m0, n);
        a1.load(p, rr, m0 + 64, n);
        stage_pass(0);
        staged_pass_interior<EPI>(p, st, rr, (lane & 7) * 8, m0, n, cs, bpre, &a0);
        stage_pass(1);
        staged_pass_interior<EPI>(p, st, rr, (lane & 7) * 8, m0 + 64, n, cs, bpre, &a1);
    } else {
#pragma unroll
        for (int pass = 0; pass < 2; pass++) {
            stage_pass(pass);
            staged_pass<EPI>(p, st, lane, m0, n0, pass, interior, cs, bpre);
        }
    }
    staged_colsum<EPI>(p, lane, m0, n0, cs);
}

__device__ __forceinline__ int sq_off(int r, int col) {
    return r * 64 + ((((col >> 2) ^ (r & 15)) << 2) | (col & 3));
}
template <int EPI>
struct EpiAuxQ {
    static constexpr bool AUX16 = epi_aux16(EPI);
    static constexpr bool AUX32 = EPI == EPI_F32_RESID || EPI == EPI_F32_ACC;
    static constexpr int N = AUX16 ? 4 : (AUX32 ? 8 : 0);
    epi_u32x4v ax[N > 0 ? N : 1];
    __device__ __forceinline__ void load(const GemmParams& p, int rr, int mrow, int n) {
        if constexpr (AUX16) {
#pragma unroll
            for (int it = 0; it < 4; it++)
                ax[it] = epi_ld16(p, (const bf16_t*)p.aux + (long long)(mrow + it * 8 + rr) * p.ldaux + n);
        } else if constexpr (AUX32) {
            const float* src = EPI == EPI_F32_RESID ? (const float*)p.aux : (const float*)p.C;
            const long long ld = EPI == EPI_F32_RESID ? p.ldaux : p.ldc;
#pragma unroll
            for (int it = 0; it < 4; it++) {
                const float* q = src + (long long)(mrow + it * 8 + rr) * ld + n;
                ax[2 * it] = epi_ld16(p, q);
                ax[2 * it + 1] = epi_ld16(p, q + 4);
            }
        }
    }
};
__device__ __forceinline__ void stage_back8_q(float* st, int r, int cc, uint32_t w0, uint32_t w1, uint32_t w2,
                                              uint32_t w3) {
    typedef float f4 __attribute__((ext_vector_type(4)));
    *reinterpret_cast<f4*>(st + sq_off(r, cc)) = f4{__uint_as_float(w0 << 16), __uint_as_float(w0 & 0xffff0000u),
                                                    __uint_as_float(w1 << 16), __uint_as_float(w1 & 0xffff0000u)};
    *reinterpret_cast<f4*>(st + sq_off(r, cc + 4)) = f4{__uint_as_float(w2 << 16), __uint_as_float(w2 & 0xffff0000u),
                                                        __uint_as_float(w3 << 16), __uint_as_float(w3 & 0xffff0000u)};
}
__device__ __forceinline__ void mx_cols_pass_q(const GemmParams& p, const float* st, int lane, int mrow, int n0) {
    if (mrow >= p.M) return;
    typedef unsigned int u32x4 __attribute__((ext_vector_type(4)));
    const int c = n0 + lane;
    float amax = 0.f;
#pragma unroll
    for (int i = 0; i < 32; i++) amax = fmaxf(amax, fabsf(st[sq_off(i, lane)]));
    const int sb = mx_scale_byte(amax);
    const int tok = p.mxc_off + mrow, kb = tok >> 5;
    p.mxc_s[((long long)(kb >> 1) * p.mxc_rg + (c >> 5)) * 64 + (kb & 1) * 32 + (c & 31)] = (uint8_t)sb;
    const float inv = __uint_as_float((uint32_t)(254 - sb) << 23);
    uint32_t w[8];
#pragma unroll
    for (int j = 0; j < 8; j++) {
        const float v0 = st[sq_off(4 * j, lane)], v1 = st[sq_off(4 * j + 1, lane)];
        const float v2 = st[sq_off(4 * j + 2, lane)], v3 = st[sq_off(4 * j + 3, lane)];
        int t = __builtin_amdgcn_cvt_pk_fp8_f32(v0 * inv, v1 * inv, 0, false);
        t = __builtin_amdgcn_cvt_pk_fp8_f32(v2 * inv, v3 * inv, t, true);
        w[j] = (uint32_t)t;
    }
    uint8_t* dst = p.mxc_q + (long long)c * p.mxc_ld + tok;
    *reinterpret_cast<u32x4*>(dst) = u32x4{w[0], w[1], w[2], w[3]};
    *reinterpret_cast<u32x4*>(dst + 16) = u32x4{w[4], w[5], w[6], w[7]};
}
template <int EPI, bool MX>
__device__ __forceinline__ void staged_pass_interior_q(const GemmParams& p, float* st, int rr, int cc,
                                                       int mrow, int n, float (&cs)[8], const float* bv,
                                                       const EpiAuxQ<EPI>& aux) {
    typedef unsigned int u32x4 __attribute__((ext_vector_type(4)));
    constexpr bool AUX16 = epi_aux16(EPI);
    constexpr bool AUX32 = EPI == EPI_F32_RESID || EPI == EPI_F32_ACC;
    const int cc_lane = cc >> 3;
#pragma unroll
    for (int it = 0; it < 4; it++) {
        const int r = it * 8 + rr;
        const f32x4_t lo = *reinterpret_cast<const f32x4_t*>(st + sq_off(r, cc));
        const f32x4_t hi = *reinterpret_cast<const f32x4_t*>(st + sq_off(r, cc + 4));
        float v[8] = {lo[0], lo[1], lo[2], lo[3], hi[0], hi[1], hi[2], hi[3]};
        const long long off = (long long)(mrow + r) * p.ldc + n;
#pragma unroll
        for (int j = 0; j < 8; j++) v[j] += bv[j];
        auto pack8 = [](const float (&w)[8]) {
            return u32x4{pack_bf16x2(w[0], w[1]), pack_bf16x2(w[2], w[3]), pack_bf16x2(w[4], w[5]),
                         pack_bf16x2(w[6], w[7])};
        };
        auto st_f32 = [&](float* q) {
            epi_st16(p, q, u32x4{__float_as_uint(v[0]), __float_as_uint(v[1]), __float_as_uint(v[2]), __float_as_uint(v[3])});
            epi_st16(p, q + 4, u32x4{__float_as_uint(v[4]), __float_as_uint(v[5]), __float_as_uint(v[6]), __float_as_uint(v[7])});
        };
        if constexpr (EPI == EPI_F32_STORE) {
            st_f32((float*)p.C + off);
        } else if constexpr (AUX32) {
#pragma unroll
            for (int j = 0; j < 4; j++) {
                v[j] += __uint_as_float(aux.ax[2 * it][j]);
                v[4 + j] += __uint_as_float(aux.ax[2 * it + 1][j]);
            }
            st_f32((float*)p.C + off);
        } else if constexpr (EPI == EPI_BF16_STORE) {
            epi_st16(p, (bf16_t*)p.C + off, pack8(v));
        } else if constexpr (EPI == EPI_BF16_GELU) {
            float gv[8];
#pragma unroll
            for (int j = 0; j < 8; j++) gv[j] = gelu_fast_f(v[j]);
            epi_st16(p, (bf16_t*)p.C + off, pack8(v));
            const u32x4 g8 = pack8(gv);
            if (p.C2) epi_st16(p, (bf16_t*)p.C2 + off, g8);
            if constexpr (MX) {
                if (p.mx_q) mx_out8(p, mrow + r, n, g8[0], g8[1], g8[2], g8[3], cc_lane);
                if (p.mxc_q) stage_back8_q(st, r, cc, g8[0], g8[1], g8[2], g8[3]);
            }
        } else if constexpr (EPI == EPI_BF16_GELU_D) {
            float gv[8], dv[8];
#pragma unroll
            for (int j = 0; j < 8; j++) gelu_pair_fast_f(v[j], gv[j], dv[j]);
            epi_st16(p, (bf16_t*)p.C + off, pack8(dv));
            const u32x4 g8 = pack8(gv);
            if (p.C2) epi_st16(p, (bf16_t*)p.C2 + off, g8);
            if constexpr (MX) {
                if (p.mx_q) mx_out8(p, mrow + r, n, g8[0], g8[1], g8[2], g8[3], cc_lane);
                if (p.mxc_q) stage_back8_q(st, r, cc, g8[0], g8[1], g8[2], g8[3]);
            }
        } else if constexpr (AUX16) {
            {
#pragma clang fp contract(off)
#pragma unroll
            for (int j = 0; j < 4; j++) {
                const float a0 = __uint_as_float(aux.ax[it][j] << 16), a1 = __uint_as_float(aux.ax[it][j] & 0xffff0000u);
                if constexpr (EPI == EPI_BF16_DGELU) {
                    v[2 * j] *= gelu_grad_fast_f(a0);
                    v[2 * j + 1] *= gelu_grad_fast_f(a1);
                } else {
                    v[2 * j] *= a0;
                    v[2 * j + 1] *= a1;
                }
            }
#pragma unroll
            for (int j = 0; j < 8; j++) cs[j] += v[j];
            }
            const u32x4 d8 = pack8(v);
            if (p.C) epi_st16(p, (bf16_t*)p.C + off, d8);
            if constexpr (MX) {
                if (p.mx_q) mx_out8(p, mrow + r, n, d8[0], d8[1], d8[2], d8[3], cc_lane);
                if (p.mxc_q) stage_back8_q(st, r, cc, d8[0], d8[1], d8[2], d8[3]);
            }
        }
    }
}
template <int EPI, bool MX, typename StagePass>
__device__ __forceinline__ void staged_epilogue_q_any(const GemmParams& p, StagePass stage_pass, float* st, int lane,
                                                      int m0, int n0, const float* bpre) {
    const int rr = lane >> 3, cc = (lane & 7) * 8, n = n0 + cc;
    float cs[8] = {0.f, 0.f, 0.f, 0.f, 0.f, 0.f, 0.f, 0.f};
    auto mx_cols = [&](int pass) {
        if constexpr (MX && epi_mx(EPI)) {
            if (p.mxc_q) {
                asm volatile("s_waitcnt lgkmcnt(0)" ::: "memory");
                mx_cols_pass_q(p, st, lane, m0 + pass * 32, n0);
            }
        }
    };
    if (staged_interior<EPI>(p, m0, n0)) {
        if constexpr (!MX) {
            EpiAuxQ<EPI> a0, a1;
            a0.load(p, rr, m0, n);
#pragma unroll
            for (int pass = 0; pass < 4; pass += 2) {
                a1.load(p, rr, m0 + (pass + 1) * 32, n);
                stage_pass(pass);
                staged_pass_interior_q<EPI, MX>(p, st, rr, cc, m0 + pass * 32, n, cs, bpre, a0);
                if (pass + 2 < 4) a0.load(p, rr, m0 + (pass + 2) * 32, n);
                stage_pass(pass + 1);
                staged_pass_interior_q<EPI, MX>(p, st, rr, cc, m0 + (pass + 1) * 32, n, cs, bpre, a1);
            }
        } else {
#pragma unroll
            for (int pass = 0; pass < 4; pass++) {
                EpiAuxQ<EPI> a0;
                a0.load(p, rr, m0 + pass * 32, n);
                stage_pass(pass);
                staged_pass_interior_q<EPI, MX>(p, st, rr, cc, m0 + pass * 32, n, cs, bpre, a0);
                mx_cols(pass);
            }
        }
    } else {
#pragma unroll
        for (int pass = 0; pass < 4; pass++) {
            stage_pass(pass);
#pragma unroll
            for (int it = 0; it < 4; it++) {
                const int r = it * 8 + rr;
                const f32x4_t lo = *reinterpret_cast<const f32x4_t*>(st + sq_off(r, cc));
                const f32x4_t hi = *reinterpret_cast<const f32x4_t*>(st + sq_off(r, cc + 4));
                float v[8] = {lo[0], lo[1], lo[2], lo[3], hi[0], hi[1], hi[2], hi[3]};
                const int m = m0 + pass * 32 + r;
                if (m >= p.M) continue;
                if (n + 8 <= p.N) {
                    if constexpr (MX && epi_mx(EPI)) {
                        float wb[8];
                        epilogue8<EPI>(p, m, n, v, cs, lane, p.mxc_q ? wb : nullptr);
                        if (p.mxc_q) {
                            typedef float f4 __attribute__((ext_vector_type(4)));
                            *reinterpret_cast<f4*>(st + sq_off(r, cc)) = f4{wb[0], wb[1], wb[2], wb[3]};
                            *reinterpret_cast<f4*>(st + sq_off(r, cc + 4)) = f4{wb[4], wb[5], wb[6], wb[7]};
                        }
                    } else {
                        epilogue8<EPI, false>(p, m, n, v, cs, lane, nullptr);
                    }
                } else if (n + 4 <= p.N) {
                    f32x4_t t = lo;
                    epilogue<EPI>(p, m, n, t);
                    if constexpr (epi_aux16(EPI)) {
#pragma clang fp contract(off)
                        cs[0] += t[0]; cs[1] += t[1]; cs[2] += t[2]; cs[3] += t[3];
                    }
                }
            }
            mx_cols(pass);
        }
    }
    staged_colsum<EPI>(p, lane, m0, n0, cs);
}
template <int EPI>
__device__ __forceinline__ void staged_epilogue_q(const GemmParams& p, f32x4_t (&acc)[8][4], float* st, int lane,
                                                  int m0, int n0, const float* bpre) {
    const int i = lane & 15, g = lane >> 4;
    auto stage_pass = [&](int pass) {
#pragma unroll
        for (int a = 0; a < 2; a++)
#pragma unroll
            for (int b = 0; b < 4; b++)
                *reinterpret_cast<f32x4_t*>(st + sq_off(a * 16 + i, b * 16 + 4 * g)) = acc[pass * 2 + a][b];
    };
    staged_epilogue_q_any<EPI, false>(p, stage_pass, st, lane, m0, n0, bpre);
}

}
```

vit.rs_amd/csrc/ops.hip:

```cpp
#include "ops_internal.h"
#include "ln_common.h"

namespace vit {

__global__ void residual_fwd_k(float* __restrict__ out, const float* __restrict__ a,
                               const float* __restrict__ b, long long n) {
    for (long long i = blockIdx.x * (long long)blockDim.x + threadIdx.x; i < n;
         i += (long long)gridDim.x * blockDim.x)
        out[i] = a[i] + b[i];
}
__global__ void residual_bwd_k(float* __restrict__ d1, float* __restrict__ d2,
                               const float* __restrict__ dout, long long n) {
    for (long long i = blockIdx.x * (long long)blockDim.x + threadIdx.x; i < n;
         i += (long long)gridDim.x * blockDim.x) {
        const float g = dout[i];
        d1[i] += g;
        d2[i] += g;
    }
}
__global__ void gelu_fwd_k(float* __restrict__ out, const float* __restrict__ inp, long long n) {
    for (long long i = blockIdx.x * (long long)blockDim.x + threadIdx.x; i < n;
         i += (long long)gridDim.x * blockDim.x)
        out[i] = gelu_f(inp[i]);
}
// ... 1045 lines not shown
        a.B = inp; a.ldb = C; a.b_kcontig = false;
        a.C = dweight; a.ldc = C;
        a.M = OC; a.N = C; a.K = BT;
        a.epi = (long long)BT > 4096 ? EPI_F32_ATOMIC : EPI_F32_ACC;
        gemm_f32(a, stream());
    }
    if (dbias) colsum_f32(dbias, dout, BT, OC, OC, stream());
}
void layernorm_forward(float* out, float* mean, float* rstd, const float* inp, const float* weight,
                       const float* bias, int B, int T, int C) {
    ln_forward_f32(out, mean, rstd, inp, weight, bias, (long long)B * T, C, stream());
}
void layernorm_backward(float* dinp, float* dweight, float* dbias, const float* dout,
                        const float* inp, const float* weight, const float* mean, const float* rstd,
                        int B, int T, int C) {
    ln_backward_f32(dinp, dweight, dbias, dout, inp, weight, mean, rstd, (long long)B * T, C,
                    stream());
}
void softmax_forward(float* probs, const float* logits, int B, int T, int V) {
    softmax_rows(probs, logits, (long long)B * T, V, stream());
}
void crossentropy_forward(float* losses, const float* probs, const int* targets, int B, int T,
                          int V) {
    ce_forward(losses, probs, targets, (long long)B * T, V, stream());
}
void softmax_crossentropy_soft_forward(float* probs, float* losses, const float* logits, const int* ta,
                                       const int* tb, float lam, float eps, int B, int T, int V) {
    softmax_ce_soft(probs, losses, logits, ta, tb, lam, eps, (long long)B * T, V, stream());
}
void crossentropy_soft_softmax_backward(float* dlogits, const float* dlosses, const float* probs,
                                        const int* ta, const int* tb, float lam, float eps, int B, int T,
                                        int V) {
    ce_soft_backward(dlogits, dlosses, probs, ta, tb, lam, eps, (long long)B * T, V, stream());
}
void crossentropy_softmax_backward(float* dlogits, const float* dlosses, const float* probs,
                                   const int* targets, int B, int T, int V) {
    ce_backward(dlogits, dlosses, probs, targets, (long long)B * T, V, stream());
}
void patch_embed_forward(float* encoded, const float* pixels, const float* patch_w,
                         const float* patch_b, const float* cls, const float* wpe, int B, int IMG,
                         int P, int C) {
    const int NP = (IMG / P) * (IMG / P), K = 3 * P * P;
    const size_t n_patch = (size_t)B * NP * K, n_emb = (size_t)B * NP * C;
    float* ws = (float*)workspace((n_patch + n_emb) * sizeof(float) + 256);
    if (!ws) return;
    float* patches = ws;
    float* emb = ws + ((n_patch + 63) & ~(size_t)63);
    hipStream_t s = stream();
    im2col_f32(patches, pixels, B, IMG, P, s);
    GemmArgs a;
    a.A = patches; a.lda = K; a.a_kcontig = true;
    a.B = patch_w; a.ldb = K; a.b_kcontig = true;
    a.C = emb; a.ldc = C; a.bias = patch_b;
    a.M = B * NP; a.N = C; a.K = K; a.epi = EPI_F32_STORE;
    gemm_f32(a, s);
    patch_assemble(encoded, emb, cls, wpe, B, NP, C, s);
}
void patch_embed_backward(float* dpatch_w, float* dpatch_b, float* dcls, float* dwpe,
                          const float* dencoded, const float* pixels, int B, int IMG, int P, int C) {
    const int NP = (IMG / P) * (IMG / P), K = 3 * P * P, T = NP + 1;
    const size_t n_patch = (size_t)B * NP * K, n_g = (size_t)B * NP * C;
    const size_t o_g = (n_patch + 63) & ~(size_t)63, o_t = (o_g + n_g + 63) & ~(size_t)63;
    float* ws = (float*)workspace((o_t + (size_t)T * C) * sizeof(float));
    if (!ws) return;
    float* patches = ws;
    float* g = ws + o_g;
    hipStream_t s = stream();
    im2col_f32(patches, pixels, B, IMG, P, s);
    patch_gather_f32(g, dencoded, B, NP, C, s);
    GemmArgs a;
    a.A = g; a.lda = C; a.a_kcontig = false;
    a.B = patches; a.ldb = K; a.b_kcontig = false;
    a.C = dpatch_w; a.ldc = K;
    a.M = C; a.N = K; a.K = B * NP;
    a.epi = (long long)B * NP > 4096 ? EPI_F32_ATOMIC : EPI_F32_ACC;
    gemm_f32(a, s);
    patch_small_grads(dcls, dwpe, dpatch_b, dencoded, B, T, C, s, ws + o_t);
}
void sgd_step(float* params, const float* grads, long long n, float lr) {
    sgd(params, grads, n, lr, stream());
}
void grad_sumsq(double* out, const float* x, long long n) {
    VIT_REQUIRE(n >= 0, "grad_sumsq: n %lld", n);
    const int nb = sumsq_blocks(n);
    double* slots = nb ? (double*)workspace((size_t)nb * sizeof(double)) : nullptr;
    if (nb && !slots) return;
    sumsq_partials(slots, x, n, stream());
    sumsq_finish(out, slots, nb, stream());
}

void matmul_forward_bf16(uint16_t* out, const uint16_t* inp, const uint16_t* weight,
                         const float* bias, int B, int T, int C, int OC) {
    GemmArgs a;
    a.A = inp; a.lda = C; a.a_kcontig = true;
    a.B = weight; a.ldb = C; a.b_kcontig = true;
    a.C = out; a.ldc = OC; a.bias = bias;
    a.M = B * T; a.N = OC; a.K = C; a.epi = EPI_BF16_STORE;
    gemm_bf16(a, stream());
}
void matmul_backward_bf16(float* dinp, float* dweight, float* dbias, const uint16_t* dout,
                          const uint16_t* inp, const uint16_t* weight, int B, int T, int C, int OC) {
    const int BT = B * T;
    if (dinp) {
        GemmArgs a;
        a.A = dout; a.lda = OC; a.a_kcontig = true;
        a.B = weight; a.ldb = C; a.b_kcontig = false;
        a.C = dinp; a.ldc = C;
        a.M = BT; a.N = C; a.K = OC; a.epi = EPI_F32_ACC;
        gemm_bf16(a, stream());
    }
    {
        GemmArgs a;
        a.A = dout; a.lda = OC; a.a_kcontig = false;
        a.B = inp; a.ldb = C; a.b_kcontig = false;
        a.C = dweight; a.ldc = C;
        a.M = OC; a.N = C; a.K = BT; a.epi = EPI_F32_ATOMIC;
        a.dbias = dbias;
        gemm_bf16(a, stream());
    }
}
void layernorm_backward_bf16(float* dinp, float* dweight, float* dbias, const uint16_t* dout,
                             const float* inp, const float* weight, const float* mean,
                             const float* rstd, int B, int T, int C) {
    LnbIo io{};
    io.dinp = dinp; io.dweight = dweight; io.dbias = dbias;
    ln_backward_any<bf16_t, false>(io, (const bf16_t*)dout, inp, weight,
                    mean, rstd, (long long)B * T, C, stream());
}
void gelu_forward_bf16(uint16_t* out, const uint16_t* inp, int N) {
    if (N <= 0) return;
    gelu_fwd_bf16_k<<<grid_for(N, 256), 256, 0, stream()>>>(out, inp, N);
    after_launch("gelu_forward_bf16");
}
void gelu_backward_bf16(float* dinp, const uint16_t* inp, const uint16_t* dout, int N) {
    if (N <= 0) return;
    gelu_bwd_bf16_k<<<grid_for(N, 256), 256, 0, stream()>>>(dinp, inp, dout, N);
    after_launch("gelu_backward_bf16");
}
void layernorm_forward_bf16(uint16_t* out, float* mean, float* rstd, const float* inp,
                            const float* weight, const float* bias, int B, int T, int C) {
    ln_forward_bf16(out, mean, rstd, inp, weight, bias, (long long)B * T, C, stream());
}
void gemm_bf16_ex(void* C, long long ldc, const uint16_t* A, long long lda, int a_kcontig,
                  const uint16_t* B, long long ldb, int b_kcontig, const float* bias,
                  float* dbias, int M, int N, int K, int epi, int splitk) {
    VIT_REQUIRE(epi >= EPI_F32_STORE && epi <= EPI_BF16_STORE, "gemm_bf16_ex: epi %d", epi);
    GemmArgs a;
    a.A = A; a.lda = lda; a.a_kcontig = a_kcontig != 0;
    a.B = B; a.ldb = ldb; a.b_kcontig = b_kcontig != 0;
    a.C = C; a.ldc = ldc; a.bias = bias; a.dbias = dbias;
    a.M = M; a.N = N; a.K = K; a.epi = epi; a.splitk = splitk;
    gemm_bf16(a, stream());
}
void gemm_bf16_fused(void* C, void* C2, long long ldc, const void* aux, long long ldaux,
                     const uint16_t* A, long long lda, int a_kcontig, const uint16_t* B,
                     long long ldb, int b_kcontig, const float* bias, float* colsum_out, int M,
                     int N, int K, int epi) {
    VIT_REQUIRE(epi == EPI_BF16_GELU || epi == EPI_F32_RESID || epi == EPI_BF16_DGELU ||
                    epi == EPI_F32_STORE || epi == EPI_BF16_STORE || epi == EPI_BF16_GELU_D ||
                    epi == EPI_BF16_MUL,
                "gemm_bf16_fused: epi %d", epi);
    GemmArgs a;
    a.A = A; a.lda = lda; a.a_kcontig = a_kcontig != 0;
    a.B = B; a.ldb = ldb; a.b_kcontig = b_kcontig != 0;
    a.C = C; a.C2 = C2; a.ldc = ldc; a.aux = aux; a.ldaux = ldaux; a.bias = bias;
    a.colsum_out = colsum_out;
    a.M = M; a.N = N; a.K = K; a.epi = epi;
    gemm_bf16(a, stream());
}
void gemm_bf16_set_variant(int variant) { gemm_set_variant(variant); }
void gemm_bf16_set_debug(int flags) { gemm_set_debug(flags); }
void gemm_bf16_set_trace(unsigned long long* trace) { gemm_set_trace(trace); }
void convert_f32_to_bf16(uint16_t* out, const float* inp, long long n) {
    convert_f2bf(out, inp, n, stream());
}
void convert_bf16_to_f32(float* out, const uint16_t* inp, long long n) {
    if (n <= 0) return;
    bf2f_k<<<grid_for(n, 256), 256, 0, stream()>>>(out, inp, n);
    after_launch("convert_bf16_to_f32");
}

}
```

vit.rs_amd/csrc/trainer.hip:

```cpp
#include <rccl/rccl.h>

#include <algorithm>
#include <cmath>
#include <cstdlib>
#include <cstring>
#include <string>
#include <vector>

#include "augment.h"
#include "ops_internal.h"
#include "../../include/vit_trainer.h"
#include "../../include/vit_checkpoint.h"
#include "../../include/vit_data.h"
#include "../../include/vit_jpeg.h"

namespace vit {
bool jpeg_loader_decode_to(vit_jpeg_loader_t* l, uint8_t* out, int img, hipStream_t st, const int** labels,
                           int expect_n);
namespace {

enum TIdx {
    P_PATCH_W, P_PATCH_B, P_CLS, P_WPE, P_LN1W, P_LN1B, P_QKVW, P_QKVB, P_ATTPROJW, P_ATTPROJB,
    P_LN2W, P_LN2B, P_FCW, P_FCB, P_FCPROJW, P_FCPROJB, P_LNFW, P_LNFB, P_HEADW, P_HEADB
};

enum TimerClass {
    TC_PATCH, TC_LN_FWD, TC_QKV_FWD, TC_ATTN_FWD, TC_PROJ_FWD, TC_FC_FWD, TC_FCPROJ_FWD, TC_HEAD,
    TC_FCPROJ_DGRAD, TC_FCPROJ_WGRAD, TC_FC_DGRAD, TC_FC_WGRAD, TC_PROJ_DGRAD, TC_PROJ_WGRAD,
    TC_ATTN_BWD, TC_QKV_DGRAD, TC_QKV_WGRAD, TC_LN_BWD, TC_COLSUM, TC_PATCH_BWD, TC_SGD, TC_MISC,
    TC_QUANT, TC_COUNT
};
const char* kTimerNames[TC_COUNT] = {
    "patch_embed_fwd", "layernorm_fwd", "gemm_qkv_fwd", "attention_fwd", "gemm_proj_fwd",
    "gemm_fc_fwd", "gemm_fcproj_fwd", "head", "gemm_fcproj_dgrad", "gemm_fcproj_wgrad",
    "gemm_fc_dgrad", "gemm_fc_wgrad", "gemm_proj_dgrad", "gemm_proj_wgrad", "attention_bwd",
    "gemm_qkv_dgrad", "gemm_qkv_wgrad", "layernorm_bwd", "bias_colsum", "patch_embed_bwd", "sgd",
    "misc", "quantize_mx"};

__global__ void bcast_rows_k(float* __restrict__ out, const float* __restrict__ vec, int rows, int n) {
    const long long i = (long long)blockIdx.x * blockDim.x + threadIdx.x;
    if (i < (long long)rows * n) out[i] = vec[i % n];
}
__global__ void rows_to_bf16_k(bf16_t* __restrict__ out, uint8_t* __restrict__ lo, long long ldo,
                               const float* __restrict__ in, int rows, int C) {
    const long long i = blockIdx.x * (long long)blockDim.x + threadIdx.x;
    if (i >= (long long)rows * C) return;
    const long long b = i / C, o = b * ldo + (i - b * C);
    const bf16_t h = f2bf(in[i]);
    out[o] = h;
    lo[o] = (uint8_t)lo8_encode(in[i], bf2f(h));
}
__global__ void add_cols_k(float* __restrict__ dst, const float* __restrict__ src, int rows, int n, int lds) {
    for (long long i = blockIdx.x * (long long)blockDim.x + threadIdx.x; i < (long long)rows * n;
         i += (long long)gridDim.x * blockDim.x) {
        const long long r = i / n;
        dst[i] += src[r * lds + (i - r * n)];
    }
}
__global__ void fill_k(float* p, float v, int n) {
    int i = blockIdx.x * blockDim.x + threadIdx.x;
    if (i < n) p[i] = v;
}
template <bool CLIP>
__device__ __forceinline__ void sgd_bf16_body(float* __restrict__ p, bf16_t* __restrict__ pbf,
                                              const float* __restrict__ g, long long n, float lr, float c) {
    const long long n4 = n / 4;
    for (long long i = blockIdx.x * (long long)blockDim.x + threadIdx.x; i < n4;
         i += (long long)gridDim.x * blockDim.x) {
        float4 pv = reinterpret_cast<float4*>(p)[i];
        float4 gv = reinterpret_cast<const float4*>(g)[i];
        sgd_update4<CLIP>(pv, gv, lr, c);
        reinterpret_cast<float4*>(p)[i] = pv;
        reinterpret_cast<uint2*>(pbf)[i] = make_uint2(pack_bf16x2(pv.x, pv.y), pack_bf16x2(pv.z, pv.w));
    }
    for (long long i = n4 * 4 + blockIdx.x * (long long)blockDim.x + threadIdx.x; i < n;
         i += (long long)gridDim.x * blockDim.x) {
        p[i] = sgd_update(p[i], CLIP ? clip_scale(c, g[i]) : g[i], lr);
        pbf[i] = f2bf(p[i]);
    }
}
__global__ void sgd_bf16_k(float* __restrict__ p, bf16_t* __restrict__ pbf,
                           const float* __restrict__ g, long long n, float lr) {
    sgd_bf16_body<false>(p, pbf, g, n, lr, 1.0f);
}
__global__ void sgd_bf16_clip_k(float* __restrict__ p, bf16_t* __restrict__ pbf,
                                const float* __restrict__ g, long long n, float lr,
                                const ClipRec* __restrict__ rec) {
    sgd_bf16_body<true>(p, pbf, g, n, lr, rec->c);
}
template <bool CLIP>
__device__ __forceinline__ void adamw_body(float* __restrict__ p, bf16_t* __restrict__ pbf,
                                           const float* __restrict__ g, float* __restrict__ m,
                                           float* __restrict__ v, long long n, float lr, float b1, float b2,
                                           float omb1, float omb2, float bc1, float bc2, float eps, float wd,
                                           float c) {
    const long long n4 = n / 4;
    for (long long i = blockIdx.x * (long long)blockDim.x + threadIdx.x; i < n4;
         i += (long long)gridDim.x * blockDim.x) {
        float4 pv = reinterpret_cast<float4*>(p)[i];
        float4 gv = reinterpret_cast<const float4*>(g)[i];
        float4 mv = reinterpret_cast<float4*>(m)[i];
        float4 vv = reinterpret_cast<float4*>(v)[i];
        adamw_update4<CLIP>(pv, gv, mv, vv, lr, b1, b2, omb1, omb2, bc1, bc2, eps, wd, c);
        reinterpret_cast<float4*>(p)[i] = pv;
        reinterpret_cast<float4*>(m)[i] = mv;
        reinterpret_cast<float4*>(v)[i] = vv;
        if (pbf)
            reinterpret_cast<uint2*>(pbf)[i] = make_uint2(pack_bf16x2(pv.x, pv.y), pack_bf16x2(pv.z, pv.w));
    }
    for (long long i = n4 * 4 + blockIdx.x * (long long)blockDim.x + threadIdx.x; i < n;
         i += (long long)gridDim.x * blockDim.x) {
        p[i] = adamw_update(p[i], CLIP ? clip_scale(c, g[i]) : g[i], m[i], v[i], lr, b1, b2, omb1, omb2, bc1,
                            bc2, eps, wd);
        if (pbf) pbf[i] = f2bf(p[i]);
    }
}
__global__ void adamw_k(float* __restrict__ p, bf16_t* __restrict__ pbf, const float* __restrict__ g,
                        float* __restrict__ m, float* __restrict__ v, long long n, float lr, float b1,
                        float b2, float omb1, float omb2, float bc1, float bc2, float eps, float wd) {
    adamw_body<false>(p, pbf, g, m, v, n, lr, b1, b2, omb1, omb2, bc1, bc2, eps, wd, 1.0f);
}
__global__ void adamw_clip_k(float* __restrict__ p, bf16_t* __restrict__ pbf, const float* __restrict__ g,
                             float* __restrict__ m, float* __restrict__ v, long long n, float lr, float b1,
                             float b2, float omb1, float omb2, float bc1, float bc2, float eps, float wd,
                             const ClipRec* __restrict__ rec) {
    adamw_body<true>(p, pbf, g, m, v, n, lr, b1, b2, omb1, omb2, bc1, bc2, eps, wd, rec->c);
}
template <bool CLIP>
__global__ __launch_bounds__(GROUP_THREADS) void sgd_bf16_groups_k(float* __restrict__ p, bf16_t* __restrict__ pbf,
                                                                   const float* __restrict__ g, GroupTab gt,
                                                                   int tile_begin, int ntiles, float lr,
                                                                   const ClipRec* __restrict__ rec) {
    const float c = CLIP ? rec->c : 1.0f;
    for (int t = blockIdx.x; t < ntiles; t += gridDim.x) {
        long long beg;
        int n4;
        const int seg = group_tile(gt, tile_begin + t, beg, n4);
        sgd_group_tile<CLIP, true>(p, pbf, g, beg, n4, group_hp(lr, gt.lr_mul[seg]), c);
    }
}
template <bool CLIP>
__global__ __launch_bounds__(GROUP_THREADS) void adamw_groups_k(float* __restrict__ p, bf16_t* __restrict__ pbf,
                                                                const float* __restrict__ g, float* __restrict__ m,
                                                                float* __restrict__ v, GroupTab gt, int tile_begin,
                                                                int ntiles, float lr, float b1, float b2, float omb1,
                                                                float omb2, float bc1, float bc2, float eps, float wd,
                                                                const ClipRec* __restrict__ rec) {
    const float c = CLIP ? rec->c : 1.0f;
    for (int t = blockIdx.x; t < ntiles; t += gridDim.x) {
        long long beg;
        int n4;
        const int seg = group_tile(gt, tile_begin + t, beg, n4);
        const float lr_e = group_hp(lr, gt.lr_mul[seg]), wd_e = group_hp(wd, gt.wd_mul[seg]);
        float4* __restrict__ p4 = reinterpret_cast<float4*>(p + beg);
        const float4* __restrict__ g4 = reinterpret_cast<const float4*>(g + beg);
        float4* __restrict__ m4 = reinterpret_cast<float4*>(m + beg);
        float4* __restrict__ v4 = reinterpret_cast<float4*>(v + beg);
        uint2* __restrict__ s2 = pbf ? reinterpret_cast<uint2*>(pbf + beg) : nullptr;
        if (n4 == GROUP_TILE4) {
            float4 pv[GROUP_UNROLL], gv[GROUP_UNROLL], mv[GROUP_UNROLL], vv[GROUP_UNROLL];
#pragma unroll
            for (int k = 0; k < GROUP_UNROLL; k++) {
                const int i = threadIdx.x + k * GROUP_THREADS;
                pv[k] = p4[i];
                gv[k] = g4[i];
                mv[k] = m4[i];
                vv[k] = v4[i];
            }
#pragma unroll
            for (int k = 0; k < GROUP_UNROLL; k++) {
                const int i = threadIdx.x + k * GROUP_THREADS;
                adamw_update4<CLIP>(pv[k], gv[k], mv[k], vv[k], lr_e, b1, b2, omb1, omb2, bc1, bc2, eps, wd_e, c);
                p4[i] = pv[k];
                m4[i] = mv[k];
                v4[i] = vv[k];
                if (s2) s2[i] = make_uint2(pack_bf16x2(pv[k].x, pv[k].y), pack_bf16x2(pv[k].z, pv[k].w));
            }
        } else {
            for (int i = threadIdx.x; i < n4; i += GROUP_THREADS) {
                float4 pv = p4[i], mv = m4[i], vv = v4[i];
                adamw_update4<CLIP>(pv, g4[i], mv, vv, lr_e, b1, b2, omb1, omb2, bc1, bc2, eps, wd_e, c);
                p4[i] = pv;
                m4[i] = mv;
                v4[i] = vv;
                if (s2) s2[i] = make_uint2(pack_bf16x2(pv.x, pv.y), pack_bf16x2(pv.z, pv.w));
            }
        }
    }
}
__global__ void argmax_rows_k(int* __restrict__ pred, int* __restrict__ correct,
                              const float* __restrict__ logits, const int* __restrict__ labels,
                              int B, int NC) {
    const int row = blockIdx.x * (blockDim.x / 64) + threadIdx.x / 64, lane = threadIdx.x & 63;
    if (row >= B) return;
    const float* x = logits + (long long)row * NC;
    float best = -INFINITY;
    int bi = NC;
    for (int j = lane; j < NC; j += 64) {
        const float xv = x[j];
        if (xv > best || bi == NC) { best = xv; bi = j; }
    }
#pragma unroll
    for (int o = 32; o > 0; o >>= 1) {
        const float ob = __shfl_xor(best, o, 64);
        const int oi = __shfl_xor(bi, o, 64);
        if (oi < NC && (bi == NC || ob > best || (ob == best && oi < bi))) { best = ob; bi = oi; }
    }
    if (lane == 0) {
        pred[row] = bi;
// ... 573 lines not shown
                a.ln2_rstd = alloc<float>(BT);
                a.fchf = alloc<float>(BT * 4 * C);
                a.fchgf = alloc<float>(BT * 4 * C);
                a.fcproj = alloc<float>(BT * C);
                a.res3 = alloc<float>(BT * C);
            }
            const long long sizes[11] = {BT * C, BT * C, BT * 4 * C, BT * 4 * C, BT * C, BT * C,
                                         BT * C, att_n, att_n, BT * 3 * C, BT * C};
            float** slots[11] = {&g_dres2, &g_dfcproj, &g_dfchg, &g_dfch, &g_dln2, &g_dattproj,
                                 &g_datty, &g_dpreatt, &g_datt, &g_dqkv, &g_dln1};
            g_block_elems = 0;
            for (int k = 0; k < 11; k++) g_block_elems += (sizes[k] + 63) & ~63LL;
            g_block = alloc<float>(g_block_elems);
            long long o = 0;
            for (int k = 0; k < 11; k++) {
                *slots[k] = g_block ? g_block + o : nullptr;
                o += (sizes[k] + 63) & ~63LL;
            }
        }
        VIT_HIP(hipMemsetAsync(grads, 0, arena_elems * 4, s));
        VIT_HIP(hipStreamSynchronize(s));
        return !has_error();
    }

    void destroy() {
        if (s_copy) (void)hipStreamSynchronize(s_copy);
        for (int k = 0; k < 2; k++) {
            if (u8_copied[k]) (void)hipEventDestroy(u8_copied[k]);
            if (u8_used[k]) (void)hipEventDestroy(u8_used[k]);
        }
        if (s_copy) (void)hipStreamDestroy(s_copy);
        if (s) (void)hipStreamSynchronize(s);
        if (s_comm) (void)hipStreamSynchronize(s_comm);
        if (s2) (void)hipStreamSynchronize(s2);
        for (int k = 1; k < MAXMB; k++) if (ms[k]) (void)hipStreamSynchronize(ms[k]);
        if (comm) ncclCommDestroy(comm);
        for (auto& a : allocs) (void)hipFree(a.p);
        for (auto e : chunk_ev) (void)hipEventDestroy(e);
        for (auto e : chunk_ev2) (void)hipEventDestroy(e);
        for (auto e : bev) if (e) (void)hipEventDestroy(e);
        for (auto& row : mev)
            for (auto e : row) if (e) (void)hipEventDestroy(e);
        if (fork_ev) (void)hipEventDestroy(fork_ev);
        for (auto e : join_ev) if (e) (void)hipEventDestroy(e);
        for (auto e : chunk_evm) if (e) (void)hipEventDestroy(e);
        for (int k = 1; k < MAXMB; k++) if (ms[k]) (void)hipStreamDestroy(ms[k]);
        for (auto e : ev_pool) (void)hipEventDestroy(e);
        if (comm_done) (void)hipEventDestroy(comm_done);
        if (s) (void)hipStreamDestroy(s);
        if (s_comm) (void)hipStreamDestroy(s_comm);
        if (s2) (void)hipStreamDestroy(s2);
    }

    bool pre_side = true;
    bool pre_side_on() const { return pre_side && two_streams && lowp() && !timing && s2; }
    hipStream_t pre_side_begin() {
        VIT_HIP(hipEventRecord(bev[EV_PRE_IN], s));
        VIT_HIP(hipStreamWaitEvent(s2, bev[EV_PRE_IN], 0));
        return s2;
    }
    void pre_side_end() {
        VIT_HIP(hipEventRecord(bev[EV_PRE], s2));
        pre_pending = true;
    }
    bool pre_pending = false;
    void pre_side_wait() {
        if (!pre_pending) return;
        VIT_HIP(hipStreamWaitEvent(s, bev[EV_PRE], 0));
        pre_pending = false;
    }
    void refresh_bf16() {
        if (!lowp()) return;
        pre_side_wait();
        to_bf16_k<<<grid_for(arena_elems, 256), 256, 0, s>>>(pbf, params, arena_elems);
        after_launch("params_to_bf16");
        refresh_transposed();
    }
    void refresh_transposed() {
        const int kinds[4] = {P_QKVW, P_ATTPROJW, P_FCW, P_FCPROJW};
        const int rows[4] = {3 * C, C, 4 * C, C}, cols[4] = {C, C, C, 4 * C};
        tbeg(TC_MISC, 0);
        const bool side = pre_side_on() && !fp8();
        hipStream_t ts = side ? pre_side_begin() : s;
        for (int k = 0; k < 4 && !(fp8() && wt_cols); k++) {
            const long long stride = L > 1 ? off[kinds[k] * L + 1] - off[kinds[k] * L] : 0;
            const int l0 = stride < 0 ? L - 1 : 0;
            transpose_bf16(WT(kinds[k], l0), W(kinds[k], l0), rows[k], cols[k], L, stride < 0 ? -stride : stride, ts);
        }
        if (side) pre_side_end();
        if (patch_pad)
            VIT_HIP(hipMemcpy2DAsync(wpatch_pad, (size_t)KPP * 2, W(P_PATCH_W), (size_t)KP * 2, (size_t)KP * 2, C,
                                     hipMemcpyDeviceToDevice, s));
        tend();
        if (fp8()) refresh_fp8();
    }
    void refresh_fp8() {
        tbeg(TC_QUANT, 0);
        for (int k = 0; k < NWK; k++) {
            const long long stride = L > 1 ? off[wkinds[k] * L + 1] - off[wkinds[k] * L] : 0;
            const int l0 = stride < 0 ? L - 1 : 0;
            const long long as = stride < 0 ? -stride : stride;
            const long long N = wq_n[k], K = wq_k[k];
            quantize_mx_batched_f32(wq[k].q, wq[k].s, P(wkinds[k], l0), N, (int)K, L, as, N * K,
                                    (long long)mx_scale_bytes(N, (int)K), s);
            if (wt_cols)
                quantize_mx_cols_batched_bf16(wtq[k].q, wtq[k].s, W(wkinds[k], l0), N, (int)K, K, L, as, N * K,
                                              (long long)mx_scale_bytes(K, (int)N), s);
            else
                quantize_mx_batched_bf16(wtq[k].q, wtq[k].s, WT(wkinds[k], l0), K, (int)N, L, as, N * K,
                                         (long long)mx_scale_bytes(K, (int)N), s);
        }
        tend();
    }
    QMat wq_of(int ti, int l) const {
        const int k = wkind_of(ti), j = wslot(k, l);
        return {wq[k].q + (long long)j * wq_n[k] * wq_k[k], wq[k].s + (long long)j * mx_scale_bytes(wq_n[k], (int)wq_k[k])};
    }
    QMat wtq_of(int ti, int l) const {
        const int k = wkind_of(ti), j = wslot(k, l);
        return {wtq[k].q + (long long)j * wq_n[k] * wq_k[k], wtq[k].s + (long long)j * mx_scale_bytes(wq_k[k], (int)wq_n[k])};
    }
    enum { PRE_NONE = 0, PRE_EPI = 1, PRE_LN = 2 };
    void gemm_w(int cls, GemmArgs a, int ti, int l, bool transposed, int mb, hipStream_t st, int pre = PRE_NONE,
                bool mx_out = false, const QMat* colq = nullptr, int rec_ev = -1) {
        if (!fp8()) { gemm(cls, a, true, st); return; }
        if (mx_out) { a.mx_q = act_q2[mb]; a.mx_s = act_s2[mb]; }
        const uint8_t* aq = act_q[mb];
        const uint8_t* as = act_s[mb];
        if (pre == PRE_EPI) {
            aq = act_q2[mb];
            as = act_s2[mb];
        } else if (pre == PRE_NONE) {
            tbeg(TC_QUANT, 0, st);
            if (colq) {
                const long long r0 = (long long)mb * (B / nmb) * T;
                const long long ntok = mb_ntok(mb, a.M);
                quantize_mx_rowcol_bf16(act_q[mb], act_s[mb], colq->q, colq->s, (const bf16_t*)a.A, a.M, a.K, a.lda,
                                        kp_tok, r0, ntok, st);
            } else {
                quantize_mx_bf16(act_q[mb], act_s[mb], (const bf16_t*)a.A, a.M, a.K, a.lda, a.K, st);
            }
            tend();
            if (rec_ev >= 0 && two_streams) VIT_HIP(hipEventRecord(mev[mb][rec_ev], st));
        }
        const QMat w = transposed ? wtq_of(ti, l) : wq_of(ti, l);
        a.A = aq; a.lda = a.K; a.a_scale = as;
        a.B = w.q; a.ldb = a.K; a.b_scale = w.s; a.b_kcontig = true;
        tbeg(cls, 2.0 * a.M * (double)a.N * a.K, st);
        gemm_fp8(a, st);
        tend();
    }

    bool last_cls = true;
    bool lc_active = false;
    bool lc_dirty = true;
    bool lc_pending = false;
    bool last_cls_on() const { return last_cls && prec == VIT_BF16; }
    void last_cls_clear() {
        if (!lc_dirty) return;
        hipStream_t cs = s;
        if (two_streams && s2) {
            VIT_HIP(hipEventRecord(bev[EV_LC_IN], s));
            VIT_HIP(hipStreamWaitEvent(s2, bev[EV_LC_IN], 0));
            cs = s2;
        }
        VIT_HIP(hipMemsetAsync(dln_bf, 0, (size_t)BT * C * 2, cs));
        VIT_HIP(hipMemsetAsync(datty, 0, (size_t)BT * C * 2, cs));
        if (cs != s) {
            VIT_HIP(hipEventRecord(bev[EV_LC], cs));
            lc_pending = true;
        }
        lc_dirty = false;
    }
    void last_cls_wait() {
        if (!lc_pending) return;
        VIT_HIP(hipStreamWaitEvent(s, bev[EV_LC], 0));
        lc_pending = false;
    }

    bool head_sk = true;
    bool patch_tail = true;
    int head_split(int M, int N, int K) const {
        if (!head_sk) return 0;
        int sp = std::min(16, std::max(1, K / 64));
        while (sp > 1 && (size_t)sp * M * N * sizeof(float) > gemm_ws_bytes) sp--;
        return sp;
    }
    void head_forward() {
        tbeg(TC_HEAD, 2.0 * B * C * NC);
        const float* last = la[L - 1].res3;
        VIT_HIP(hipMemcpy2DAsync(cls_x, C * 4, last, (size_t)T * C * 4, C * 4, B, hipMemcpyDeviceToDevice, s));
        ln_forward_f32(lnf, lnf_mean, lnf_rstd, cls_x, P(P_LNFW), P(P_LNFB), B, C, s);
        GemmArgs a;
        a.A = lnf; a.lda = C; a.B = P(P_HEADW); a.ldb = C; a.C = logits; a.ldc = NC;
        a.bias = P(P_HEADB); a.M = B; a.N = NC; a.K = C; a.epi = EPI_F32_STORE;
        if (lowp()) {
            bcast_rows_k<<<cdiv((long long)B * NC, 256), 256, 0, s>>>(logits, P(P_HEADB), B, NC);
            a.bias = nullptr;
            a.epi = EPI_F32_ATOMIC;
            a.splitk = head_split(a.M, a.N, a.K);
        }
        a.ws = gemm_ws; a.ws_bytes = gemm_ws_bytes;
        gemm_f32(a, s);
        if (has_targets && soft_targets()) {
            softmax_ce_soft(probs, losses, logits, labels, two_labels() ? labels_b : nullptr, mix_lam,
                            smooth_eps, B, NC, s);
        } else {
            softmax_rows(probs, logits, B, NC, s);
            if (has_targets) ce_forward(losses, probs, labels, B, NC, s);
        }
        tend();
    }
    void head_backward(float* dres, bf16_t* dres_bf = nullptr, uint8_t* dres_lo = nullptr) {
        tbeg(TC_HEAD, 4.0 * B * C * NC);
        fill_k<<<cdiv(B, 256), 256, 0, s>>>(dlosses, 1.0f / (float)b_global, B);
        VIT_HIP(hipMemsetAsync(dlogits, 0, (size_t)B * NC * 4, s));
        if (soft_targets())
            ce_soft_backward(dlogits, dlosses, probs, labels, two_labels() ? labels_b : nullptr, mix_lam,
                             smooth_eps, B, NC, s);
        else
            ce_backward(dlogits, dlosses, probs, labels, B, NC, s);
        VIT_HIP(hipMemsetAsync(dlnf, 0, (size_t)B * C * 4, s));
        GemmArgs a;
        a.A = dlogits; a.lda = NC; a.a_kcontig = true;
        a.B = P(P_HEADW); a.ldb = C; a.b_kcontig = false;
        a.C = dlnf; a.ldc = C; a.M = B; a.N = C; a.K = NC; a.epi = lowp() ? EPI_F32_ATOMIC : EPI_F32_ACC;
        if (lowp()) a.splitk = head_split(a.M, a.N, a.K);
        a.ws = gemm_ws; a.ws_bytes = gemm_ws_bytes;
        gemm_f32(a, s);
        GemmArgs w;
        w.A = dlogits; w.lda = NC; w.a_kcontig = false;
        w.B = lnf; w.ldb = C; w.b_kcontig = false;
        w.C = G(P_HEADW); w.ldc = C; w.M = NC; w.N = C; w.K = B; w.epi = lowp() ? EPI_F32_ATOMIC : EPI_F32_ACC;
        if (lowp()) w.splitk = head_split(w.M, w.N, w.K);
        w.ws = gemm_ws; w.ws_bytes = gemm_ws_bytes;
        gemm_f32(w, s);
        colsum_f32(G(P_HEADB), dlogits, B, NC, NC, s, red_ws);
        VIT_HIP(hipMemsetAsync(dcls_x, 0, (size_t)B * C * 4, s));
        ln_backward_f32(dcls_x, G(P_LNFW), G(P_LNFB), dlnf, cls_x, P(P_LNFW), lnf_mean, lnf_rstd, B, C, s, red_ws);
        if (dres_bf) {
            VIT_HIP(hipMemsetAsync(dres_bf, 0, (size_t)BT * C * 2, s));
            VIT_HIP(hipMemsetAsync(dres_lo, 0, (size_t)BT * C, s));
            rows_to_bf16_k<<<cdiv((long long)B * C, 256), 256, 0, s>>>(dres_bf, dres_lo, (long long)T * C, dcls_x, B, C);
        } else {
            VIT_HIP(hipMemsetAsync(dres, 0, (size_t)BT * C * 4, s));
            VIT_HIP(hipMemcpy2DAsync(dres, (size_t)T * C * 4, dcls_x, C * 4, C * 4, B, hipMemcpyDeviceToDevice, s));
        }
        tend();
    }

    void forward_bf16() {
        const int Bm = B / nmb;
        const long long R = (long long)Bm * T;
        lc_active = last_cls_on();
        if (lc_active) last_cls_clear();
        mb_fork();
        for (int mb = 0; mb < nmb; mb++) {
            hipStream_t st = ms[mb];
            const long long img0 = (long long)mb * Bm;
            tbeg(TC_PATCH, 2.0 * Bm * NP * (double)KP * C, st);
            GemmArgs a;
            a.C = emb_tmp + img0 * NP * C; a.ldc = C; a.bias = P(P_PATCH_B);
            a.M = Bm * NP; a.N = C; a.K = KP; a.epi = EPI_F32_STORE;
            if (patch_f32) {
                im2col_f32(patches_f + img0 * NP * KP, pixels + img0 * 3 * cfg.img * cfg.img, Bm, cfg.img,
                           cfg.patch, st);
                a.A = patches_f + img0 * NP * KP; a.lda = KP; a.B = P(P_PATCH_W); a.ldb = KP;
                gemm_f32(a, st);
            } else if (patch_pad) {
                im2col_pad_bf16(patches_bf + img0 * NP * KPP, pixels + img0 * 3 * cfg.img * cfg.img, Bm, cfg.img,
                                cfg.patch, KPP, st);
                a.A = patches_bf + img0 * NP * KPP; a.lda = KPP; a.B = wpatch_pad; a.ldb = KPP; a.K = KPP;
                gemm_bf16(a, st);
            } else {
                im2col_bf16(patches_bf + img0 * NP * KP, pixels + img0 * 3 * cfg.img * cfg.img, Bm, cfg.img,
                            cfg.patch, st);
                a.A = patches_bf + img0 * NP * KP; a.lda = KP; a.B = W(P_PATCH_W); a.ldb = KP;
                gemm_bf16(a, st);
            }
            patch_assemble(encoded + img0 * T * C, emb_tmp + img0 * NP * C, P(P_CLS), P(P_WPE), Bm, NP, C, st);
            tend();
        }
        for (int l = 0; l < L; l++) {
            LayerActs& a = la[l];
            const float* xl = l == 0 ? encoded : la[l - 1].res3;
            const bool lc = lc_active && l == L - 1;
            const int Mr = lc ? Bm : (int)R;
            const long long rs = lc ? T : 1;
            const bool lcg = lc && R >= 256;
            for (int mb = 0; mb < nmb; mb++) {
                hipStream_t st = ms[mb];
                const long long r0 = (long long)mb * R;
                const float* x = xl + r0 * C;
                const bool rc = rowcol_on(), lm = lnmx_on();
                QMat c_ln1 = rc ? actc_of(0, l) : QMat{}, c_atty = rc ? actc_of(1, l) : QMat{},
                     c_ln2 = rc ? actc_of(2, l) : QMat{};
                tbeg(TC_LN_FWD, 0, st);
                if (lm)
                    ln_forward_mx(act_q[mb], act_s[mb], c_ln1.q, c_ln1.s, a.ln1_mean + r0, a.ln1_rstd + r0, x,
                                  P(P_LN1W, l), P(P_LN1B, l), R, C, kp_tok, r0, mb_ntok(mb, R), st,
                                  ln_left ? lnb_scr[mb] : nullptr);
                else
                    ln_forward_bf16(a.ln1 + r0 * C, a.ln1_mean + r0, a.ln1_rstd + r0, x, P(P_LN1W, l), P(P_LN1B, l), R, C, st);
                tend();
                GemmArgs q;
                q.A = a.ln1 + r0 * C; q.lda = C; q.B = W(P_QKVW, l); q.ldb = C; q.C = a.qkv + r0 * 3 * C;
                q.ldc = 3 * C; q.bias = P(P_QKVB, l); q.M = (int)R; q.N = 3 * C; q.K = C; q.epi = EPI_BF16_STORE;
                gemm_w(TC_QKV_FWD, q, P_QKVW, l, false, mb, st, lm ? PRE_LN : PRE_NONE, false,
                       rc && !lm ? &c_ln1 : nullptr);
                tbeg(TC_ATTN_FWD, 4.0 * Bm * (double)T * T * C, st);
                attn_forward_fused(a.atty + r0 * C, a.lse + (long long)mb * Bm * NH * T, a.qkv + r0 * 3 * C, Bm, T, C, NH, st);
                tend();
                GemmArgs pr;
                pr.A = a.atty + r0 * C; pr.lda = rs * C; pr.B = W(P_ATTPROJW, l); pr.ldb = C; pr.C = a.res2 + r0 * C;
                pr.ldc = rs * C; pr.bias = P(P_ATTPROJB, l); pr.aux = x; pr.ldaux = rs * C;
                pr.M = Mr; pr.N = C; pr.K = C; pr.epi = EPI_F32_RESID; pr.rows_gathered = lcg;
                gemm_w(TC_PROJ_FWD, pr, P_ATTPROJW, l, false, mb, st, PRE_NONE, false, rc ? &c_atty : nullptr);
                tbeg(TC_LN_FWD, 0, st);
                if (lm)
                    ln_forward_mx(act_q[mb], act_s[mb], c_ln2.q, c_ln2.s, a.ln2_mean + r0, a.ln2_rstd + r0,
                                  a.res2 + r0 * C, P(P_LN2W, l), P(P_LN2B, l), R, C, kp_tok, r0, mb_ntok(mb, R), st,
                                  ln_left ? lnb_scr[mb] : nullptr);
                else
                    ln_forward_bf16(a.ln2 + r0 * C, a.ln2_mean + r0, a.ln2_rstd + r0, a.res2 + r0 * C, P(P_LN2W, l),
                                    P(P_LN2B, l), Mr, C, st, rs);
                tend();
                GemmArgs f;
                f.A = a.ln2 + r0 * C; f.lda = rs * C; f.B = W(P_FCW, l); f.ldb = C; f.C = a.fchd + r0 * 4 * C;
                f.C2 = a.fchg + r0 * 4 * C; f.ldc = rs * 4 * C; f.bias = P(P_FCB, l); f.M = Mr; f.N = 4 * C;
                f.K = C; f.epi = EPI_BF16_GELU_D; f.rows_gathered = lcg;
                if (epicol_on()) {
                    const QMat g = fchgc_of(l);
                    f.C2 = nullptr;
                    f.mxc_q = g.q; f.mxc_s = g.s; f.mxc_ld = kp_tok; f.mxc_off = r0;
                }
                gemm_w(TC_FC_FWD, f, P_FCW, l, false, mb, st, lm ? PRE_LN : PRE_NONE, fuse_mx,
                       rc && !lm ? &c_ln2 : nullptr);
                GemmArgs fp;
                fp.A = a.fchg + r0 * 4 * C; fp.lda = rs * 4 * C; fp.B = W(P_FCPROJW, l); fp.ldb = 4 * C;
                fp.C = a.res3 + r0 * C; fp.ldc = rs * C; fp.bias = P(P_FCPROJB, l); fp.aux = a.res2 + r0 * C;
                fp.ldaux = rs * C; fp.M = Mr; fp.N = C; fp.K = 4 * C; fp.epi = EPI_F32_RESID; fp.rows_gathered = lcg;
                gemm_w(TC_FCPROJ_FWD, fp, P_FCPROJW, l, false, mb, st, fuse_mx ? PRE_EPI : PRE_NONE);
            }
        }
        mb_join();
        head_forward();
    }

    void wgrad(int cls, const bf16_t* dout, int OC, const bf16_t* inp, int Cin, float* dW, int ready,
               int done, const QMat* dout_c = nullptr, const QMat* inp_c = nullptr) {
        GemmArgs w;
        w.A = dout; w.lda = OC; w.a_kcontig = false;
        w.B = inp; w.ldb = Cin; w.b_kcontig = false;
        w.C = dW; w.ldc = Cin; w.M = OC; w.N = Cin; w.K = (int)BT; w.epi = EPI_F32_ATOMIC;
        w.ws = gemm_ws; w.ws_bytes = gemm_ws_bytes;
        w.fill_pct = two_streams ? 0 : 80;
        hipStream_t st = two_streams ? s2 : s;
        if (two_streams) {
            for (int mb = 0; mb < nmb; mb++) {
                if (!dout_c) VIT_HIP(hipEventRecord(mev[mb][ready], ms[mb]));
                VIT_HIP(hipStreamWaitEvent(s2, mev[mb][ready], 0));
            }
        }
        if (fp8() && fp8_wgrad) {
            const long long kp = mx_cols_kp(BT);
            const QMat qa = dout_c ? *dout_c : wg_a, qb = inp_c ? *inp_c : wg_b;
            if (!dout_c || !inp_c) {
                tbeg(TC_QUANT, 0, st);
                if (!dout_c) quantize_mx_cols_bf16(wg_a.q, wg_a.s, dout, BT, OC, OC, st);
                if (!inp_c) quantize_mx_cols_bf16(wg_b.q, wg_b.s, inp, BT, Cin, Cin, st);
                tend();
            }
            w.A = qa.q; w.lda = kp; w.a_kcontig = true; w.a_scale = qa.s;
            w.B = qb.q; w.ldb = kp; w.b_kcontig = true; w.b_scale = qb.s;
            w.K = (int)kp;
            tbeg(cls, 2.0 * w.M * (double)w.N * BT, st);
            gemm_fp8(w, st);
            tend();
        } else {
            tbeg(cls, 2.0 * w.M * (double)w.N * w.K, st);
            gemm_bf16(w, st);
            tend();
        }
        if (two_streams) VIT_HIP(hipEventRecord(bev[done], s2));
    }
    void after_wgrad(int done, hipStream_t st) {
        if (two_streams) VIT_HIP(hipStreamWaitEvent(st, bev[done], 0));
    }

    float* sg_rows(int l, long long off) { return sg_part[l & 1] + off; }
    void sg_finalize(int l, long long R) {
        hipStream_t st = two_streams ? s2 : s;
        if (two_streams) {
            for (int mb = 0; mb < nmb; mb++) {
                VIT_HIP(hipEventRecord(mev[mb][EV_SG], ms[mb]));
                VIT_HIP(hipStreamWaitEvent(s2, mev[mb][EV_SG], 0));
            }
        }
        const int nb = nmb * ln_bwd_blocks(R), w1 = l > 0 ? 3 * C : 2 * C;
        const float* p2 = sg_rows(l, sg_ln2);
        const float* p1 = sg_rows(l, sg_ln1);
        RowsJob jobs[8] = {
            {G(P_LN2W, l), p2, nb, 3 * C, C},
            {G(P_LN2B, l), p2 + C, nb, 3 * C, C},
            {G(P_ATTPROJB, l), p2 + 2 * C, nb, 3 * C, C},
            {G(P_LN1W, l), p1, nb, w1, C},
            {G(P_LN1B, l), p1 + C, nb, w1, C},
            {G(P_FCB, l), sg_rows(l, sg_fcb), nmb * fcb_rows, 4 * C, 4 * C},
            {G(P_QKVB, l), sg_rows(l, sg_qkv), nmb, 3 * C, 3 * C},
            {l > 0 ? G(P_FCPROJB, l - 1) : nullptr, p1 + 2 * C, nb, w1, C},
        };
        tbeg(TC_COLSUM, 0, st);
        rows_reduce_add(jobs, l > 0 ? 8 : 7, st);
        tend();
    }

    void backward_bf16() {
        pre_side_wait();
        last_cls_wait();
        lc_dirty = true;
        bf16_t* rbA = dres_bf;
        bf16_t* rbB = dres_bf2;
        uint8_t* loA = dres_lo;
        uint8_t* loB = dres_lo2;
        head_backward(nullptr, rbA, loA);
        chunk_done(0);
        colsum_f32(G(P_FCPROJB, L - 1), dcls_x, B, C, C, s, red_ws);
        mb_fork();
        const int Bm = B / nmb;
        const long long R = (long long)Bm * T;
        for (int l = L - 1; l >= 0; l--) {
            LayerActs& a = la[l];
            const float* xl = l == 0 ? encoded : la[l - 1].res3;
            const bool lc = lc_active && l == L - 1;
            const int Mr = lc ? Bm : (int)R;
            const long long rs = lc ? T : 1;
            const bool lcg = lc && R >= 256;
            const bool rc = rowcol_on();
            QMat c_ln1 = rc ? actc_of(0, l) : QMat{}, c_atty = rc ? actc_of(1, l) : QMat{}, c_ln2 = rc ? actc_of(2, l) : QMat{};
            const bool lbm = lnbmx_on(), resa_pre = lbm && l < L - 1;
            const bool ec = epicol_on();
            QMat c_fchg = ec ? fchgc_of(l) : QMat{};
            if (!rc) wgrad(TC_FCPROJ_WGRAD, rbA, C, a.fchg, 4 * C, G(P_FCPROJW, l), EV_RESA, EV_W1);
            for (int mb = 0; mb < nmb; mb++) {
                const long long r0 = mb * R;
                after_wgrad(EV_W2, ms[mb]);
                GemmArgs d1;
                d1.A = rbA + r0 * C; d1.lda = C; dgrad_b(d1, P_FCPROJW, l, C, 4 * C);
                d1.C = dfch + r0 * 4 * C; d1.ldc = 4 * C; d1.aux = a.fchd + r0 * 4 * C; d1.ldaux = 4 * C;
                d1.M = (int)R; d1.N = 4 * C; d1.K = C; d1.epi = EPI_BF16_MUL;
                fcb_rows = gemm_colsum_rows(d1, fp8());
                d1.colsum_part = sg_rows(l, sg_fcb) + (long long)mb * fcb_rows * 4 * C;
                if (ec) {
                    d1.C = nullptr;
                    d1.mxc_q = dfchc.q; d1.mxc_s = dfchc.s; d1.mxc_ld = kp_tok; d1.mxc_off = r0;
                }
                gemm_w(TC_FCPROJ_DGRAD, d1, P_FCPROJW, l, true, mb, ms[mb], resa_pre ? PRE_LN : PRE_NONE, fuse_mx,
                       rc && !resa_pre ? &dcol[0] : nullptr, resa_pre ? -1 : EV_RESA);
                if (ec && two_streams) VIT_HIP(hipEventRecord(mev[mb][EV_DFCH], ms[mb]));
            }
            if (rc) wgrad(TC_FCPROJ_WGRAD, rbA, C, a.fchg, 4 * C, G(P_FCPROJW, l), EV_RESA, EV_W1, &dcol[0],
                          ec ? &c_fchg : nullptr);
            wgrad(TC_FC_WGRAD, dfch, 4 * C, a.ln2, C, G(P_FCW, l), EV_DFCH, EV_W2, ec ? &dfchc : nullptr,
                  rc ? &c_ln2 : nullptr);
            for (int mb = 0; mb < nmb; mb++) {
                const long long r0 = mb * R;
                GemmArgs d2;
                d2.A = dfch + r0 * 4 * C; d2.lda = rs * 4 * C; dgrad_b(d2, P_FCW, l, 4 * C, C);
                d2.C = dln_bf + r0 * C; d2.ldc = rs * C; d2.M = Mr; d2.N = C; d2.K = 4 * C; d2.epi = EPI_BF16_STORE;
                d2.rows_gathered = lcg;
                gemm_w(TC_FC_DGRAD, d2, P_FCW, l, true, mb, ms[mb], fuse_mx ? PRE_EPI : PRE_NONE);
                after_wgrad(EV_W3, ms[mb]);
                tbeg(TC_LN_BWD, 0, ms[mb]);
                if (lbm) {
                    ln_backward_bf16_stream_mx(rbB + r0 * C, loB + r0 * C, rbA + r0 * C, loA + r0 * C, G(P_LN2W, l),
                                               G(P_LN2B, l), G(P_ATTPROJB, l), dln_bf + r0 * C, a.res2 + r0 * C,
                                               P(P_LN2W, l), a.ln2_mean + r0, a.ln2_rstd + r0, R, C, ms[mb],
                                               sg_rows(l, sg_ln2) + (long long)mb * ln_bwd_blocks(R) * 3 * C,
                                               act_q[mb], act_s[mb], dcol[1].q, dcol[1].s, kp_tok, r0, mb_ntok(mb, R),
                                               lnb_scr[mb]);
                    if (two_streams) VIT_HIP(hipEventRecord(mev[mb][EV_RESB], ms[mb]));
                } else {
                    ln_backward_bf16_stream(rbB + r0 * C, loB + r0 * C, rbA + r0 * C, loA + r0 * C, G(P_LN2W, l),
                                            G(P_LN2B, l), G(P_ATTPROJB, l), dln_bf + r0 * C, a.res2 + r0 * C,
                                            P(P_LN2W, l), a.ln2_mean + r0, a.ln2_rstd + r0, R, C, ms[mb],
                                            sg_rows(l, sg_ln2) + (long long)mb * ln_bwd_blocks(R) * 3 * C);
                }
                tend();
            }
            if (!rc) wgrad(TC_PROJ_WGRAD, rbB, C, a.atty, C, G(P_ATTPROJW, l), EV_RESB, EV_W3);
            for (int mb = 0; mb < nmb; mb++) {
                const long long r0 = mb * R;
                GemmArgs d3;
                d3.A = rbB + r0 * C; d3.lda = rs * C; dgrad_b(d3, P_ATTPROJW, l, C, C);
                d3.C = datty + r0 * C; d3.ldc = rs * C; d3.M = Mr; d3.N = C; d3.K = C; d3.epi = EPI_BF16_STORE;
                d3.rows_gathered = lcg;
                gemm_w(TC_PROJ_DGRAD, d3, P_ATTPROJW, l, true, mb, ms[mb], lbm ? PRE_LN : PRE_NONE, false,
                       rc && !lbm ? &dcol[1] : nullptr, lbm ? -1 : EV_RESB);
                after_wgrad(EV_W4, ms[mb]);
                tbeg(TC_ATTN_BWD, 8.0 * Bm * (double)T * T * C, ms[mb]);
                attn_backward_fused(dqkv + r0 * 3 * C, datty + r0 * C, a.qkv + r0 * 3 * C, a.atty + r0 * C,
                                    a.lse + (long long)mb * Bm * NH * T, Bm, T, C, NH, ms[mb],
                                    sg_rows(l, sg_qkv) + (long long)mb * 3 * C,
                                    attn_part + (long long)attn_backward_ws_floats(mb * Bm, T, C, NH), true);
                tend();
            }
            if (rc) wgrad(TC_PROJ_WGRAD, rbB, C, a.atty, C, G(P_ATTPROJW, l), EV_RESB, EV_W3, &dcol[1], &c_atty);
            if (!rc) wgrad(TC_QKV_WGRAD, dqkv, 3 * C, a.ln1, C, G(P_QKVW, l), EV_DQKV, EV_W4);
            for (int mb = 0; mb < nmb; mb++) {
                const long long r0 = mb * R;
                GemmArgs d4;
                d4.A = dqkv + r0 * 3 * C; d4.lda = 3 * C; dgrad_b(d4, P_QKVW, l, 3 * C, C);
                d4.C = dln_bf + r0 * C; d4.ldc = C; d4.M = (int)R; d4.N = C; d4.K = 3 * C; d4.epi = EPI_BF16_STORE;
                gemm_w(TC_QKV_DGRAD, d4, P_QKVW, l, true, mb, ms[mb], PRE_NONE, false, rc ? &dcol[2] : nullptr, EV_DQKV);
                after_wgrad(EV_W1, ms[mb]);
                tbeg(TC_LN_BWD, 0, ms[mb]);
                if (lbm && l > 0) {
                    ln_backward_bf16_stream_mx(rbA + r0 * C, loA + r0 * C, rbB + r0 * C, loB + r0 * C, G(P_LN1W, l),
                                               G(P_LN1B, l), G(P_FCPROJB, l - 1), dln_bf + r0 * C, xl + r0 * C,
                                               P(P_LN1W, l), a.ln1_mean + r0, a.ln1_rstd + r0, R, C, ms[mb],
                                               sg_rows(l, sg_ln1) + (long long)mb * ln_bwd_blocks(R) * 3 * C,
                                               act_q[mb], act_s[mb], dcol[0].q, dcol[0].s, kp_tok, r0, mb_ntok(mb, R),
                                               lnb_scr[mb]);
                    if (two_streams) VIT_HIP(hipEventRecord(mev[mb][EV_RESA], ms[mb]));
                } else {
                    ln_backward_bf16_stream(rbA + r0 * C, loA + r0 * C, rbB + r0 * C, loB + r0 * C, G(P_LN1W, l),
                                            G(P_LN1B, l), l > 0 ? G(P_FCPROJB, l - 1) : nullptr, dln_bf + r0 * C,
                                            xl + r0 * C, P(P_LN1W, l), a.ln1_mean + r0, a.ln1_rstd + r0, R, C, ms[mb],
                                            sg_rows(l, sg_ln1) + (long long)mb * ln_bwd_blocks(R) * (l > 0 ? 3 : 2) * C);
                }
                tend();
            }
            if (rc) wgrad(TC_QKV_WGRAD, dqkv, 3 * C, a.ln1, C, G(P_QKVW, l), EV_DQKV, EV_W4, &dcol[2], &c_ln1);
            sg_finalize(l, R);
            chunk_done(L - l);
        }
        mb_join();
        if (two_streams) {
            VIT_HIP(hipEventRecord(bev[EV_JOIN], s2));
            VIT_HIP(hipStreamWaitEvent(s, bev[EV_JOIN], 0));
        }
        tbeg(TC_PATCH_BWD, 2.0 * B * NP * (double)KP * C);
        const bool psg_side = two_streams && lowp() && patch_tail;
        if (psg_side) {
            VIT_HIP(hipEventRecord(bev[EV_SG], s));
            VIT_HIP(hipStreamWaitEvent(s2, bev[EV_SG], 0));
            patch_small_grads(G(P_CLS), G(P_WPE), G(P_PATCH_B), rbA, loA, B, T, C, s2, pos_sums, psg_part);
            VIT_HIP(hipEventRecord(bev[EV_JOIN], s2));
        }
        if (patch_f32) {
            patch_gather_f32(dpatch_f, rbA, loA, B, NP, C, s);
            GemmArgs w;
            w.A = dpatch_f; w.lda = C; w.a_kcontig = false; w.B = patches_f; w.ldb = KP; w.b_kcontig = false;
            w.C = G(P_PATCH_W); w.ldc = KP; w.M = C; w.N = KP; w.K = B * NP; w.epi = EPI_F32_ATOMIC;
            gemm_f32(w, s);
        } else {
            patch_gather_bf16(dpatch_bf, rbA, B, NP, C, s);
            GemmArgs w;
            w.A = dpatch_bf; w.lda = C; w.a_kcontig = false;
            w.B = patches_bf; w.ldb = KPP; w.b_kcontig = false;
            w.C = G(P_PATCH_W); w.ldc = KP; w.M = C; w.N = KP; w.K = B * NP; w.epi = EPI_F32_ATOMIC;
            w.ws = gemm_ws; w.ws_bytes = gemm_ws_bytes;
            w.fill_pct = patch_tail ? 80 : 0;
            if (patch_pad) {
                VIT_HIP(hipMemsetAsync(dwpatch_pad, 0, (size_t)C * KPP * 4, s));
                w.C = dwpatch_pad; w.ldc = KPP; w.N = KPP;
            }
            gemm_bf16(w, s);
            if (patch_pad)
                add_cols_k<<<grid_for((long long)C * KP, 256), 256, 0, s>>>(G(P_PATCH_W), dwpatch_pad, C, KP, KPP);
        }
        if (psg_side)
            VIT_HIP(hipStreamWaitEvent(s, bev[EV_JOIN], 0));
        else
            patch_small_grads(G(P_CLS), G(P_WPE), G(P_PATCH_B), rbA, loA, B, T, C, s, pos_sums, psg_part);
        tend();
        chunk_done(L + 1);
    }

    void forward_f32() {
        im2col_f32(patches_f, pixels, B, cfg.img, cfg.patch, s);
        {
            GemmArgs a;
            a.A = patches_f; a.lda = KP; a.B = P(P_PATCH_W); a.ldb = KP; a.C = emb_tmp; a.ldc = C;
            a.bias = P(P_PATCH_B); a.M = B * NP; a.N = C; a.K = KP; a.epi = EPI_F32_STORE;
            gemm_f32(a, s);
        }
        patch_assemble(encoded, emb_tmp, P(P_CLS), P(P_WPE), B, NP, C, s);
        for (int l = 0; l < L; l++) {
            LayerActs& a = la[l];
            const float* x = l == 0 ? encoded : la[l - 1].res3;
            ln_forward_f32(a.ln1f, a.ln1_mean, a.ln1_rstd, x, P(P_LN1W, l), P(P_LN1B, l), BT, C, s);
            mm_fwd(a.qkvf, a.ln1f, P(P_QKVW, l), P(P_QKVB, l), C, 3 * C);
            attn_forward_f32(a.attyf, a.preatt, a.att, a.qkvf, B, T, C, NH, s);
            mm_fwd(a.attproj, a.attyf, P(P_ATTPROJW, l), P(P_ATTPROJB, l), C, C);
            add(a.res2, x, a.attproj, BT * C);
            ln_forward_f32(a.ln2f, a.ln2_mean, a.ln2_rstd, a.res2, P(P_LN2W, l), P(P_LN2B, l), BT, C, s);
            mm_fwd(a.fchf, a.ln2f, P(P_FCW, l), P(P_FCB, l), C, 4 * C);
            gelu(a.fchgf, a.fchf, BT * 4 * C);
            mm_fwd(a.fcproj, a.fchgf, P(P_FCPROJW, l), P(P_FCPROJB, l), 4 * C, C);
            add(a.res3, a.res2, a.fcproj, BT * C);
        }
        head_forward();
    }
    void mm_fwd(float* out, const float* inp, const float* w, const float* b, int Cin, int OC) {
        GemmArgs a;
        a.A = inp; a.lda = Cin; a.B = w; a.ldb = Cin; a.C = out; a.ldc = OC; a.bias = b;
        a.M = (int)BT; a.N = OC; a.K = Cin; a.epi = EPI_F32_STORE;
        gemm_f32(a, s);
    }
    void mm_bwd(float* dinp, float* dw, float* db, const float* dout, const float* inp,
                const float* w, int Cin, int OC) {
        GemmArgs d;
        d.A = dout; d.lda = OC; d.B = w; d.ldb = Cin; d.b_kcontig = false; d.C = dinp; d.ldc = Cin;
        d.M = (int)BT; d.N = Cin; d.K = OC; d.epi = EPI_F32_ACC;
        gemm_f32(d, s);
        GemmArgs g;
        g.A = dout; g.lda = OC; g.a_kcontig = false; g.B = inp; g.ldb = Cin; g.b_kcontig = false;
        g.C = dw; g.ldc = Cin; g.M = OC; g.N = Cin; g.K = (int)BT; g.epi = EPI_F32_ATOMIC;
        g.ws = gemm_ws; g.ws_bytes = gemm_ws_bytes;
        gemm_f32(g, s);
        colsum_f32(db, dout, (int)BT, OC, OC, s, red_ws);
    }
    void add(float* out, const float* a, const float* b, long long n);
    void gelu(float* out, const float* in, long long n);
    void gelu_bwd(float* dinp, const float* in, const float* dout, long long n);
    void res_bwd(float* d1, float* d2, const float* dout, long long n);

    void backward_f32() {
        float* dcur = dres_a;
        float* dnxt = dres_b;
        head_backward(dcur);
        chunk_done(0);
        for (int l = L - 1; l >= 0; l--) {
            LayerActs& a = la[l];
            const float* x = l == 0 ? encoded : la[l - 1].res3;
            VIT_HIP(hipMemsetAsync(g_block, 0, g_block_elems * 4, s));
            VIT_HIP(hipMemsetAsync(dnxt, 0, BT * C * 4, s));
            res_bwd(g_dres2, g_dfcproj, dcur, BT * C);
            mm_bwd(g_dfchg, G(P_FCPROJW, l), G(P_FCPROJB, l), g_dfcproj, a.fchgf, P(P_FCPROJW, l), 4 * C, C);
            gelu_bwd(g_dfch, a.fchf, g_dfchg, BT * 4 * C);
            mm_bwd(g_dln2, G(P_FCW, l), G(P_FCB, l), g_dfch, a.ln2f, P(P_FCW, l), C, 4 * C);
            ln_backward_f32(g_dres2, G(P_LN2W, l), G(P_LN2B, l), g_dln2, a.res2, P(P_LN2W, l),
// ... 677 lines not shown
                                                 t.has_targets ? t.labels : nullptr, t.B, t.NC);
    vit::after_launch("argmax_rows");
    std::vector<int> out(t.B + 1);
    VIT_HIP(hipMemcpyAsync(out.data(), t.preds, (size_t)(t.B + 1) * 4, hipMemcpyDeviceToHost, t.s));
    VIT_HIP(hipStreamSynchronize(t.s));
    if (vit::has_error()) return 1;
    if (host_pred) memcpy(host_pred, out.data(), (size_t)t.B * 4);
    if (host_correct && t.has_targets) *host_correct = out[t.B];
    return 0;
}
int vit_trainer_save_checkpoint(vit_trainer_t* h, const char* path) {
    auto& t = h->t;
    VIT_HIP(hipDeviceSynchronize());
    if (vit::has_error()) return 1;
    std::vector<float> p((size_t)t.n_params), m, v;
    t.device_to_canon(t.params, p.data());
    if (t.adam_m) {
        m.resize((size_t)t.n_params);
        v.resize((size_t)t.n_params);
        t.device_to_canon(t.adam_m, m.data());
        t.device_to_canon(t.adam_v, v.data());
    }
    if (vit::has_error()) return 1;
    return vit_checkpoint_write(path, &t.cfg, p.data(), t.adam_m ? m.data() : nullptr,
                                t.adam_m ? v.data() : nullptr, t.adam_t, &t.adam_hp);
}
int vit_trainer_load_checkpoint(vit_trainer_t* h, const char* path) {
    auto& t = h->t;
    vit_checkpoint_info_t info;
    if (vit_checkpoint_read_info(path, &info)) return 1;
    std::vector<float> p((size_t)t.n_params), m, v;
    if (info.has_opt) {
        m.resize((size_t)t.n_params);
        v.resize((size_t)t.n_params);
    }
    if (vit_checkpoint_read(path, &t.cfg, p.data(), info.has_opt ? m.data() : nullptr,
                            info.has_opt ? v.data() : nullptr))
        return 1;
    VIT_HIP(hipDeviceSynchronize());
    t.canon_to_device(p.data(), t.params);
    t.refresh_bf16();
    if (info.has_opt) {
        if (!t.ensure_adam()) return 1;
        t.canon_to_device(m.data(), t.adam_m);
        t.canon_to_device(v.data(), t.adam_v);
        t.adam_t = info.step;
        t.adam_hp = info.adamw;
    } else if (t.adam_m) {
        VIT_HIP(hipMemsetAsync(t.adam_m, 0, t.arena_elems * 4, t.s));
        VIT_HIP(hipMemsetAsync(t.adam_v, 0, t.arena_elems * 4, t.s));
        t.adam_t = 0;
    }
    VIT_HIP(hipStreamSynchronize(t.s));
    return vit::has_error();
}
float vit_trainer_mean_loss(vit_trainer_t* h) {
    auto& t = h->t;
    if (!t.has_targets) return -1.0f;
    std::vector<float> l(t.B);
    VIT_HIP(hipMemcpyAsync(l.data(), t.losses, t.B * 4, hipMemcpyDeviceToHost, t.s));
    VIT_HIP(hipStreamSynchronize(t.s));
    float m = 0.f;
    for (float v : l) m += v;
    return m / (float)t.B;
}
int vit_trainer_get_logits(vit_trainer_t* h, float* out) {
    auto& t = h->t;
    VIT_HIP(hipMemcpyAsync(out, t.logits, (size_t)t.B * t.NC * 4, hipMemcpyDeviceToHost, t.s));
    VIT_HIP(hipStreamSynchronize(t.s));
    return vit::has_error();
}
int vit_trainer_sync(vit_trainer_t* h) {
    h->t.pre_side_wait();
    VIT_HIP(hipStreamSynchronize(h->t.s_comm));
    VIT_HIP(hipStreamSynchronize(h->t.s));
    return vit::has_error();
}
void* vit_trainer_stream(vit_trainer_t* h) { return (void*)h->t.s; }

int vit_layout_query(const vit_config_t* cfg, long long* tensor_off, long long* chunk_off, long long* arena_elems) {
    if (!cfg || cfg->num_layers < 1 || cfg->num_layers > VIT_MAX_LAYERS || cfg->patch < 1 || cfg->img < cfg->patch ||
        cfg->channels < 1 || cfg->num_classes < 1) {
        set_error("vit_layout_query: bad config");
        return -1;
    }
    const int L = cfg->num_layers, np = (cfg->img / cfg->patch) * (cfg->img / cfg->patch);
    long long canon[20], n_params = 0, co[VIT_MAX_LAYERS + 3], arena = 0;
    std::vector<long long> off;
    int n_chunks = 0;
    vit::compute_layout(cfg->channels, L, np + 1, cfg->in_ch * cfg->patch * cfg->patch, cfg->num_classes, canon,
                        n_params, off, co, n_chunks, arena);
    if (tensor_off) memcpy(tensor_off, off.data(), off.size() * sizeof(long long));
    if (chunk_off) memcpy(chunk_off, co, (size_t)(n_chunks + 1) * sizeof(long long));
    if (arena_elems) *arena_elems = arena;
    return n_chunks;
}
int vit_dp_unique_id_size(void) { return (int)sizeof(ncclUniqueId); }
int vit_dp_get_unique_id(char* out) {
    ncclUniqueId id;
    ncclResult_t r = ncclGetUniqueId(&id);
    if (r != ncclSuccess) {
        set_error("ncclGetUniqueId: %s", ncclGetErrorString(r));
        return 1;
    }
    memcpy(out, &id, sizeof(id));
    return 0;
}
int vit_trainer_dp_init(vit_trainer_t* h, int rank, int world, const char* uid, int overlap) {
    auto& t = h->t;
    t.rank = rank;
    t.world = world;
    t.overlap = overlap;
    if (world < 1 || rank < 0 || rank >= world) {
        set_error("vit_trainer_dp_init: bad rank %d / world %d", rank, world);
        return 1;
    }
    ncclUniqueId id;
    memcpy(&id, uid, sizeof(id));
    VIT_HIP(hipSetDevice(t.device));
    ncclResult_t r = ncclCommInitRank(&t.comm, world, id, rank);
    if (r != ncclSuccess) {
        set_error("ncclCommInitRank(rank %d/%d): %s", rank, world, ncclGetErrorString(r));
        t.comm = nullptr;
        return 1;
    }
    return 0;
}
int vit_trainer_get_dp_snapshot(vit_trainer_t* h, float* host) {
    auto& t = h->t;
    if (!t.dp_probe_on) {
        set_error("vit_trainer_get_dp_snapshot: option dp_probe is off");
        return 1;
    }
    VIT_HIP(hipStreamSynchronize(t.s_comm));
    t.device_to_canon(t.dp_snap, host);
    return vit::has_error();
}
int vit_trainer_dp_ranks(vit_trainer_t* h) {
    if (!h->t.comm) return 0;
    int n = 0;
    ncclResult_t r = ncclCommCount(h->t.comm, &n);
    if (r != ncclSuccess) {
        set_error("ncclCommCount: %s", ncclGetErrorString(r));
        return -1;
    }
    return n;
}
int vit_trainer_set_concurrency(vit_trainer_t* h, int on) {
    auto& t = h->t;
    VIT_HIP(hipStreamSynchronize(t.s2));
    for (int k = 0; k < vit::Trainer::MAXMB; k++) if (t.ms[k]) VIT_HIP(hipStreamSynchronize(t.ms[k]));
    t.two_streams = on != 0;
    t.nmb = t.pick_nmb(t.mb_want);
    return vit::has_error();
}
int vit_trainer_set_option(vit_trainer_t* h, const char* name, int value) {
    auto& t = h->t;
    VIT_HIP(hipDeviceSynchronize());
    const std::string n = name ? name : "";
    if (n == "microbatch") {
        t.mb_want = value;
        t.nmb = t.pick_nmb(value);
    } else if (n == "dgrad_transposed") {
        t.dgrad_wt = value != 0;
    } else if (n == "fp8_ln_mx") {
        t.ln_mx = value != 0;
    } else if (n == "fp8_ln_leftover") {
        t.ln_left = value != 0;
    } else if (n == "early_sgd") {
        t.early_sgd = value < 0 ? -1 : value != 0;
    } else if (n == "pre_side") {
        t.pre_side_wait();
        t.pre_side = value != 0;
    } else if (n == "patch_tail") {
        t.patch_tail = value != 0;
    } else if (n == "head_splitk") {
        t.head_sk = value != 0;
    } else if (n == "fp8_lnb_mx") {
        t.lnb_mx = value != 0;
    } else if (n == "clip_overlap") {
        t.clip_overlap = value < 0 ? -1 : value != 0;
    } else if (n == "last_cls") {
        t.last_cls = value != 0;
    } else if (n == "dp_probe") {
        if (value && !t.dp_snap) {
            t.dp_snap = t.alloc<float>(t.arena_elems);
            if (t.dp_snap) VIT_HIP(hipMemset(t.dp_snap, 0, t.arena_elems * 4));
        }
        t.dp_probe_on = value != 0 && t.dp_snap != nullptr;
    } else {
        set_error("vit_trainer_set_option: unknown option '%s'", n.c_str());
        return 1;
    }
    return vit::has_error();
}
int vit_trainer_set_timing(vit_trainer_t* h, int on) {
    h->t.timing = on != 0;
    return 0;
}
int vit_trainer_timing(vit_trainer_t* h, const char** names, double* ms, long long* calls,
                       double* flops, int max) {
    auto& t = h->t;
    t.collect();
    int n = 0;
    for (int c = 0; c < vit::TC_COUNT && n < max; c++) {
        if (!t.t_calls[c]) continue;
        names[n] = vit::kTimerNames[c];
        ms[n] = t.t_ms[c];
        calls[n] = t.t_calls[c];
        flops[n] = t.t_flops[c];
        n++;
    }
    return n;
}
void vit_trainer_timing_reset(vit_trainer_t* h) {
    auto& t = h->t;
    t.collect();
    for (int c = 0; c < vit::TC_COUNT; c++) {
        t.t_ms[c] = 0;
        t.t_calls[c] = 0;
        t.t_flops[c] = 0;
    }
}
}
```

Measured before the change: 7428 images/s.

## Skip zero rows in last-layer CLS-only backward GEMMs via K-period and row-gathered colsum

In the last layer only the CLS token's gradient is nonzero, so the weight-gradient GEMMs now take a k_period that stages only one K tile per token period instead of the full BT reduction. The FC-proj dgrad runs on gathered CLS rows with a new row-scattered column-sum epilogue, which writes per-row partial sums into the bias-gradient slab. This relies on dfch and the slab being zero outside the CLS rows, so a clear kernel and memset are added to last_cls_clear. Both skips only apply when the CLS-only path and the kernel eligibility checks pass, and option changes invalidate the clean state.

Result: faster. 7577 images/s, median of 6 (+2.0%).

```diff
diff --git a/include/vit_ops.h b/include/vit_ops.h
--- a/include/vit_ops.h
+++ b/include/vit_ops.h
@@ -108,10 +108,17 @@
 void gemm_bf16_ex(void* C, long long ldc, const uint16_t* A, long long lda, int a_kcontig,
                   const uint16_t* B, long long ldb, int b_kcontig, const float* bias,
                   float* dbias, int M, int N, int K, int epi, int splitk);
+void gemm_bf16_kperiod(void* C, long long ldc, const uint16_t* A, long long lda, int a_kcontig,
+                       const uint16_t* B, long long ldb, int b_kcontig, int M, int N, int K, int epi,
+                       int splitk, int k_period);
 void gemm_bf16_fused(void* C, void* C2, long long ldc, const void* aux, long long ldaux,
                      const uint16_t* A, long long lda, int a_kcontig, const uint16_t* B,
                      long long ldb, int b_kcontig, const float* bias, float* colsum_out, int M,
                      int N, int K, int epi);
+void gemm_bf16_fused_rows(void* C, void* C2, long long ldc, const void* aux, long long ldaux,
+                          const uint16_t* A, long long lda, int a_kcontig, const uint16_t* B,
+                          long long ldb, int b_kcontig, const float* bias, float* colsum_out, int M,
+                          int N, int K, int epi, int rows_gathered, int colsum_row_period);
 long long mx_scale_size(long long rows, int K);
 void quantize_mx_bf16_ex(uint8_t* q, uint8_t* scales, const uint16_t* x, long long R, int K,
                          long long ldx, long long ldq);
diff --git a/vit.rs_amd/__init__.py b/vit.rs_amd/__init__.py
--- a/vit.rs_amd/__init__.py
+++ b/vit.rs_amd/__init__.py
@@ -91,7 +91,9 @@
     "gelu_forward_bf16": (None, [P, P, I]),
     "gelu_backward_bf16": (None, [P, P, P, I]),
     "gemm_bf16_ex": (None, [P, LL, P, LL, I, P, LL, I, P, P, I, I, I, I, I]),
+    "gemm_bf16_kperiod": (None, [P, LL, P, LL, I, P, LL, I, I, I, I, I, I, I]),
     "gemm_bf16_fused": (None, [P, P, LL, P, LL, P, LL, I, P, LL, I, P, P, I, I, I, I]),
+    "gemm_bf16_fused_rows": (None, [P, P, LL, P, LL, P, LL, I, P, LL, I, P, P, I, I, I, I, I, I]),
     "mx_scale_size": (LL, [LL, I]),
     "quantize_mx_bf16_ex": (None, [P, P, P, LL, I, LL, LL]),
     "quantize_mx_f32_ex": (None, [P, P, P, LL, I, LL, LL]),
diff --git a/vit.rs_amd/csrc/gemm.h b/vit.rs_amd/csrc/gemm.h
--- a/vit.rs_amd/csrc/gemm.h
+++ b/vit.rs_amd/csrc/gemm.h
@@ -14,8 +14,12 @@
     EPI_F32_SLAB = 7,
     EPI_BF16_GELU_D = 8,
     EPI_BF16_MUL = 9,
+    EPI_BF16_DGELU_ROWS = 10,
+    EPI_BF16_MUL_ROWS = 11,
 };
-constexpr bool epi_aux16(int e) { return e == EPI_BF16_DGELU || e == EPI_BF16_MUL; }
+constexpr bool epi_rows(int e) { return e == EPI_BF16_DGELU_ROWS || e == EPI_BF16_MUL_ROWS; }
+constexpr bool epi_aux16(int e) { return e == EPI_BF16_DGELU || e == EPI_BF16_MUL || epi_rows(e); }
+constexpr bool epi_dgelu(int e) { return e == EPI_BF16_DGELU || e == EPI_BF16_DGELU_ROWS; }
 constexpr bool epi_bias(int e) { return e != EPI_F32_ATOMIC && e != EPI_F32_SLAB && !epi_aux16(e); }
 constexpr bool epi_mx(int e) { return e == EPI_BF16_GELU || e == EPI_BF16_GELU_D || epi_aux16(e); }
 
@@ -39,7 +43,9 @@
     int epi = EPI_F32_STORE;
     int splitk = 0;
     int fill_pct = 0;
+    int k_period = 0;
     bool rows_gathered = false;
+    int colsum_row_period = 0;
     float* ws = nullptr;
     size_t ws_bytes = 0;
     const void* a_scale = nullptr;
@@ -55,6 +61,8 @@
 void gemm_f32(const GemmArgs& a, hipStream_t s);
 void gemm_bf16(const GemmArgs& a, hipStream_t s);
 bool gemm_bf16_supported(const GemmArgs& a);
+bool gemm_bf16_kskip(const GemmArgs& a);
+bool gemm_colsum_period_ok(const GemmArgs& a);
 void gemm_set_variant(int v);
 void gemm_set_debug(int flags);
 int gemm_cu_count();
diff --git a/vit.rs_amd/csrc/gemm.hip b/vit.rs_amd/csrc/gemm.hip
--- a/vit.rs_amd/csrc/gemm.hip
+++ b/vit.rs_amd/csrc/gemm.hip
@@ -646,7 +646,9 @@
     const int tm0 = tm * BM, tn0 = tn * BN;
     const int kbeg = split * p.kchunk;
     const int kend = min(p.K, kbeg + p.kchunk);
-    const int nk = (kend - kbeg) / BK;
+    const int kper = p.k_period;
+    const int i0 = kper > 0 ? (kbeg + kper - 1) / kper : 0;
+    const int nk = kper > 0 ? max((kend + kper - 1) / kper - i0, 0) : (kend - kbeg) / BK;
     const bf16_t* A = (const bf16_t*)p.A;
     const bf16_t* B = (const bf16_t*)p.B;
 
@@ -658,7 +660,7 @@
 
     auto issue = [&](int st) {
         char* sl = smem + (st % NSLOT) * SLOT_BYTES;
-        const int k0 = kbeg + st * BK;
+        const int k0 = kper > 0 ? ((i0 + st) * kper) & ~(BK - 1) : kbeg + st * BK;
         stage<BM>(A, p.lda, tm0, p.M, k0, sl, wave, lane);
         stage<BN>(B, p.ldb, tn0, p.N, k0, sl + A_BYTES, wave, lane);
     };
@@ -902,7 +904,10 @@
     return gemm_variant() == 11 && !a.a_scale && a.epi != EPI_F32_ATOMIC && gemm_bf16_supported(a) &&
            a.K % g2::KTILE == 0 && a.M >= 256 && a.N >= 256 && (a.N <= 1280 || pp_all()) && gemm_pp_shape(a);
 }
-int gemm_colsum_rows(const GemmArgs& a, bool fp8) { return cdiv(a.M, !fp8 && pp_taken(a) ? 96 : 128); }
+int gemm_colsum_rows(const GemmArgs& a, bool fp8) {
+    if (!fp8 && a.colsum_row_period > 0) return cdiv((long long)a.M * a.colsum_row_period, 128);
+    return cdiv(a.M, !fp8 && pp_taken(a) ? 96 : 128);
+}
 float* colsum_rows_begin(const GemmArgs& a) {
     if (!epi_aux16(a.epi) || !(a.colsum_out || a.colsum_part)) return nullptr;
     float* r = a.colsum_part ? a.colsum_part
@@ -1007,6 +1012,8 @@
     p.mxc_off = (int)a.mxc_off;
     p.mxc_rg = (int)(mx_rows_padded(a.N) / 32);
     p.tiles = 1;
+    p.k_period = 0;
+    p.colsum_row_period = 0;
     return p;
 }
 
@@ -1134,10 +1141,21 @@
                 VIT_CASE(EPI_BF16_DGELU)
                 VIT_CASE(EPI_BF16_GELU_D)
                 VIT_CASE(EPI_BF16_MUL)
+                VIT_CASE(EPI_BF16_DGELU_ROWS)
+                VIT_CASE(EPI_BF16_MUL_ROWS)
 #undef VIT_CASE
                 default: break;
             }
         }
+    }
+    if (epi_rows(a.epi)) {
+        if constexpr (AK) {
+            if (a.epi == EPI_BF16_MUL_ROWS) g2::gemm_kernel<AK, BKC, EPI_BF16_MUL_ROWS, 2><<<grid, g2::NT, 0, s>>>(p);
+            else g2::gemm_kernel<AK, BKC, EPI_BF16_DGELU_ROWS, 2><<<grid, g2::NT, 0, s>>>(p);
+        } else {
+            set_error("gemm_bf16: colsum_row_period needs a K-contiguous A");
+        }
+        return;
     }
     switch (a.epi) {
 #define VIT_CASE(E) \
@@ -1205,6 +1223,7 @@
     }
     GemmParams p = make_gemm_params(b, kchunk);
     p.tiles = tiles;
+    p.k_period = a.k_period > g4::BK ? a.k_period : 0;
     dim3 grid(tiles, split);
     if (slab) g4::gemm_kernel<EPI_F32_SLAB><<<grid, g4::NT, 0, s>>>(p);
     else g4::gemm_kernel<EPI_F32_ACC><<<grid, g4::NT, 0, s>>>(p);
@@ -1214,6 +1233,23 @@
     if (a.dbias) colsum_bf16(a.dbias, (const bf16_t*)a.A, a.K, a.M, a.lda, s);
 }
 
+static bool g4_taken(const GemmArgs& a) {
+    return gemm_variant() != 1 && a.epi == EPI_F32_ATOMIC && !a.a_kcontig && !a.b_kcontig &&
+           a.K % g4::KTILE == 0 && a.M >= 256 && a.N >= 128 && a.N % 4 == 0 &&
+           (a.splitk > 0 || !a.ws ||
+            (size_t)choose_split_g4(cdiv(a.M, g4::BM) * cdiv(a.N, g4::BN), a.K / g4::KTILE, a.fill_pct) * a.M * a.N *
+                    sizeof(float) <= a.ws_bytes);
+}
+bool gemm_bf16_kskip(const GemmArgs& a) {
+    return a.M > 0 && a.N > 0 && !a.mx_q && !a.mxc_q && gemm_bf16_supported(a) && g4_taken(a) && a.k_period > g4::BK;
+}
+bool gemm_colsum_period_ok(const GemmArgs& a) {
+    return epi_aux16(a.epi) && a.colsum_row_period >= 128 && (a.colsum_out || a.colsum_part) &&
+           a.rows_gathered && a.M >= 1 && a.a_kcontig && a.K % g2::KTILE == 0 && a.N >= 256 && a.N % 8 == 0 &&
+           gemm_variant() != 1 && gemm_variant() != 11 && !a.mx_q && !a.mxc_q && gemm_bf16_supported(a) &&
+           (long long)a.M * a.colsum_row_period < (1LL << 31) && ((uintptr_t)a.colsum_part & 15) == 0;
+}
+
 void gemm_bf16(const GemmArgs& a, hipStream_t s) {
     if (a.M <= 0 || a.N <= 0) return;
     if (a.mx_q || a.mxc_q) {
@@ -1225,11 +1261,16 @@
                   a.M, a.N, a.K, a.lda, a.ldb);
         return;
     }
-    if (gemm_variant() != 1 && a.epi == EPI_F32_ATOMIC && !a.a_kcontig && !a.b_kcontig &&
-        a.K % g4::KTILE == 0 && a.M >= 256 && a.N >= 128 && a.N % 4 == 0 &&
-        (a.splitk > 0 || !a.ws ||
-         (size_t)choose_split_g4(cdiv(a.M, g4::BM) * cdiv(a.N, g4::BN), a.K / g4::KTILE) * a.M * a.N * sizeof(float) <=
-             a.ws_bytes)) {
+    if (epi_rows(a.epi)) {
+        set_error("gemm_bf16: epilogue %d is internal (colsum_row_period)", a.epi);
+        return;
+    }
+    if (a.colsum_row_period != 0 && !gemm_colsum_period_ok(a)) {
+        set_error("gemm_bf16: colsum_row_period %d needs a row-gathered x-aux call on the 256x256 engine, "
+                  "period >= 128, N %% 8 == 0 (M=%d N=%d K=%d epi=%d)", a.colsum_row_period, a.M, a.N, a.K, a.epi);
+        return;
+    }
+    if (g4_taken(a)) {
         gemm_bf16_g4(a, s);
         return;
     }
@@ -1258,6 +1299,12 @@
         float* cs_rows = colsum_rows_begin(a);
         if ((a.colsum_out || a.colsum_part) && epi_aux16(a.epi) && !cs_rows) return;
         p.colsum_out = cs_rows;
+        if (a.colsum_row_period > 0) {
+            p.colsum_row_period = a.colsum_row_period;
+            b.epi = epi_dgelu(a.epi) ? EPI_BF16_DGELU_ROWS : EPI_BF16_MUL_ROWS;
+            if (!a.colsum_part)
+                VIT_HIP(hipMemsetAsync(cs_rows, 0, (size_t)gemm_colsum_rows(a, false) * a.N * sizeof(float), s));
+        }
         const bool late_db = a.dbias && !a.a_kcontig && split > 1;
         if (late_db) p.dbias = nullptr;
         if (split == 1 && pp_taken(b)) {
@@ -1274,7 +1321,7 @@
         else if (!a.a_kcontig && !a.b_kcontig) launch_g2<false, false>(b, p, grid, s);
         else launch_g2<false, true>(b, p, grid, s);
         after_launch("gemm_bf16_256");
-        count_hit(VIT_HIT_GEMM_256x256 + b.epi);
+        count_hit(VIT_HIT_GEMM_256x256 + (epi_rows(b.epi) ? a.epi : b.epi));
         if (slab) slab_reduce(a, slab, split, s);
         colsum_rows_end(a, cs_rows, s);
         if (late_db) colsum_bf16(a.dbias, (const bf16_t*)a.A, a.K, a.M, a.lda, s);
diff --git a/vit.rs_amd/csrc/gemm_common.h b/vit.rs_amd/csrc/gemm_common.h
--- a/vit.rs_amd/csrc/gemm_common.h
+++ b/vit.rs_amd/csrc/gemm_common.h
@@ -20,6 +20,8 @@
     int stagger;
     unsigned long long* trace;
     int tiles;
+    int colsum_row_period;
+    int k_period;
     int gm;
     uint8_t* mx_q;
     uint8_t* mx_s;
@@ -179,7 +181,7 @@
                                                         (long long)m * p.ldaux + n);
         const float x0 = __uint_as_float(h.x << 16), x1 = __uint_as_float(h.x & 0xffff0000u);
         const float x2 = __uint_as_float(h.y << 16), x3 = __uint_as_float(h.y & 0xffff0000u);
-        if constexpr (EPI == EPI_BF16_DGELU) {
+        if constexpr (epi_dgelu(EPI)) {
             v[0] *= gelu_grad_fast_f(x0); v[1] *= gelu_grad_fast_f(x1);
             v[2] *= gelu_grad_fast_f(x2); v[3] *= gelu_grad_fast_f(x3);
         } else {
@@ -260,7 +262,7 @@
 #pragma unroll
         for (int j = 0; j < 4; j++) {
             const float lo = __uint_as_float(hw[j] << 16), hi = __uint_as_float(hw[j] & 0xffff0000u);
-            if constexpr (EPI == EPI_BF16_DGELU) {
+            if constexpr (epi_dgelu(EPI)) {
                 v[2 * j] *= gelu_grad_fast_f(lo);
                 v[2 * j + 1] *= gelu_grad_fast_f(hi);
             } else {
@@ -268,8 +270,18 @@
                 v[2 * j + 1] *= hi;
             }
         }
-#pragma unroll
-        for (int j = 0; j < 8; j++) cs[j] += v[j];
+        if constexpr (epi_rows(EPI)) {
+            if (p.colsum_out) {
+                float z = 0.f;
+                asm volatile("" : "+v"(z));
+                float* q = p.colsum_out + (((long long)m * p.colsum_row_period) >> 7) * p.N + n;
+                reinterpret_cast<float4*>(q)[0] = make_float4(z + v[0], z + v[1], z + v[2], z + v[3]);
+                reinterpret_cast<float4*>(q)[1] = make_float4(z + v[4], z + v[5], z + v[6], z + v[7]);
+            }
+        } else {
+#pragma unroll
+            for (int j = 0; j < 8; j++) cs[j] += v[j];
+        }
         }
         const uint4 d8 = pack8(v);
         if (p.C) *reinterpret_cast<uint4*>((bf16_t*)p.C + off) = d8;
@@ -384,7 +396,7 @@
 #pragma unroll
             for (int j = 0; j < 4; j++) {
                 const float lo = __uint_as_float(ax[it][j] << 16), hi = __uint_as_float(ax[it][j] & 0xffff0000u);
-                if constexpr (EPI == EPI_BF16_DGELU) {
+                if constexpr (epi_dgelu(EPI)) {
                     v[2 * j] *= gelu_grad_fast_f(lo);
                     v[2 * j + 1] *= gelu_grad_fast_f(hi);
                 } else {
@@ -470,11 +482,12 @@
 }
 template <int EPI>
 __device__ __forceinline__ bool staged_interior(const GemmParams& p, int m0, int n0) {
+    if constexpr (epi_rows(EPI)) return false;
     return EPI != EPI_F32_ATOMIC && m0 + 128 <= p.M && n0 + 64 <= p.N;
 }
 template <int EPI>
 __device__ __forceinline__ void staged_colsum(const GemmParams& p, int lane, int m0, int n0, float (&cs)[8]) {
-    if constexpr (epi_aux16(EPI)) {
+    if constexpr (epi_aux16(EPI) && !epi_rows(EPI)) {
         if (p.colsum_out) {
             const int rr = lane >> 3, cc = (lane & 7) * 8;
 #pragma unroll
@@ -664,7 +677,7 @@
 #pragma unroll
             for (int j = 0; j < 4; j++) {
                 const float a0 = __uint_as_float(aux.ax[it][j] << 16), a1 = __uint_as_float(aux.ax[it][j] & 0xffff0000u);
-                if constexpr (EPI == EPI_BF16_DGELU) {
+                if constexpr (epi_dgelu(EPI)) {
                     v[2 * j] *= gelu_grad_fast_f(a0);
                     v[2 * j + 1] *= gelu_grad_fast_f(a1);
                 } else {
diff --git a/vit.rs_amd/csrc/ops.hip b/vit.rs_amd/csrc/ops.hip
--- a/vit.rs_amd/csrc/ops.hip
+++ b/vit.rs_amd/csrc/ops.hip
@@ -1221,6 +1221,18 @@
     a.M = M; a.N = N; a.K = K; a.epi = epi; a.splitk = splitk;
     gemm_bf16(a, stream());
 }
+void gemm_bf16_kperiod(void* C, long long ldc, const uint16_t* A, long long lda, int a_kcontig,
+                       const uint16_t* B, long long ldb, int b_kcontig, int M, int N, int K, int epi,
+                       int splitk, int k_period) {
+    VIT_REQUIRE(epi >= EPI_F32_STORE && epi <= EPI_BF16_STORE, "gemm_bf16_kperiod: epi %d", epi);
+    VIT_REQUIRE(k_period >= 0, "gemm_bf16_kperiod: k_period %d", k_period);
+    GemmArgs a;
+    a.A = A; a.lda = lda; a.a_kcontig = a_kcontig != 0;
+    a.B = B; a.ldb = ldb; a.b_kcontig = b_kcontig != 0;
+    a.C = C; a.ldc = ldc;
+    a.M = M; a.N = N; a.K = K; a.epi = epi; a.splitk = splitk; a.k_period = k_period;
+    gemm_bf16(a, stream());
+}
 void gemm_bf16_fused(void* C, void* C2, long long ldc, const void* aux, long long ldaux,
                      const uint16_t* A, long long lda, int a_kcontig, const uint16_t* B,
                      long long ldb, int b_kcontig, const float* bias, float* colsum_out, int M,
@@ -1237,6 +1249,24 @@
     a.M = M; a.N = N; a.K = K; a.epi = epi;
     gemm_bf16(a, stream());
 }
+void gemm_bf16_fused_rows(void* C, void* C2, long long ldc, const void* aux, long long ldaux,
+                          const uint16_t* A, long long lda, int a_kcontig, const uint16_t* B,
+                          long long ldb, int b_kcontig, const float* bias, float* colsum_out, int M,
+                          int N, int K, int epi, int rows_gathered, int colsum_row_period) {
+    VIT_REQUIRE(epi == EPI_BF16_GELU || epi == EPI_F32_RESID || epi == EPI_BF16_DGELU ||
+                    epi == EPI_F32_STORE || epi == EPI_BF16_STORE || epi == EPI_BF16_GELU_D ||
+                    epi == EPI_BF16_MUL,
+                "gemm_bf16_fused_rows: epi %d", epi);
+    VIT_REQUIRE(colsum_row_period >= 0, "gemm_bf16_fused_rows: colsum_row_period %d", colsum_row_period);
+    GemmArgs a;
+    a.A = A; a.lda = lda; a.a_kcontig = a_kcontig != 0;
+    a.B = B; a.ldb = ldb; a.b_kcontig = b_kcontig != 0;
+    a.C = C; a.C2 = C2; a.ldc = ldc; a.aux = aux; a.ldaux = ldaux; a.bias = bias;
+    a.colsum_out = colsum_out;
+    a.M = M; a.N = N; a.K = K; a.epi = epi;
+    a.rows_gathered = rows_gathered != 0; a.colsum_row_period = colsum_row_period;
+    gemm_bf16(a, stream());
+}
 void gemm_bf16_set_variant(int variant) { gemm_set_variant(variant); }
 void gemm_bf16_set_debug(int flags) { gemm_set_debug(flags); }
 void gemm_bf16_set_trace(unsigned long long* trace) { gemm_set_trace(trace); }
diff --git a/vit.rs_amd/csrc/trainer.hip b/vit.rs_amd/csrc/trainer.hip
--- a/vit.rs_amd/csrc/trainer.hip
+++ b/vit.rs_amd/csrc/trainer.hip
@@ -55,6 +55,14 @@
          i += (long long)gridDim.x * blockDim.x) {
         const long long r = i / n;
         dst[i] += src[r * lds + (i - r * n)];
+    }
+}
+__global__ void clear_cls_blocks_k(bf16_t* __restrict__ x, int T, long long rows, int n) {
+    const long long r0 = ((long long)blockIdx.y * T) & ~31LL;
+    const int cpr = n / 8;
+    for (int c = blockIdx.x * blockDim.x + threadIdx.x; c < 32 * cpr; c += gridDim.x * blockDim.x) {
+        const long long r = r0 + c / cpr;
+        if (r < rows) reinterpret_cast<uint4*>(x + r * n)[c % cpr] = make_uint4(0u, 0u, 0u, 0u);
     }
 }
 __global__ void fill_k(float* p, float v, int n) {
@@ -934,10 +942,41 @@
     }
 
     bool last_cls = true;
+    int lc_bwd = 2;
+    bool lc_d1_clean = false;
     bool lc_active = false;
     bool lc_dirty = true;
     bool lc_pending = false;
     bool last_cls_on() const { return last_cls && prec == VIT_BF16; }
+    GemmArgs wgrad_args(const bf16_t* dout, int OC, const bf16_t* inp, int Cin, float* dW, int k_period) const {
+        GemmArgs w;
+        w.A = dout; w.lda = OC; w.a_kcontig = false;
+        w.B = inp; w.ldb = Cin; w.b_kcontig = false;
+        w.C = dW; w.ldc = Cin; w.M = OC; w.N = Cin; w.K = (int)BT; w.epi = EPI_F32_ATOMIC;
+        w.ws = gemm_ws; w.ws_bytes = gemm_ws_bytes;
+        w.fill_pct = two_streams ? 0 : 80;
+        w.k_period = k_period;
+        return w;
+    }
+    bool lc_d1_gathered(int l, int mb, const bf16_t* dres3, GemmArgs& d1) {
+        const int Bm = B / nmb;
+        const long long R = (long long)Bm * T, r0 = mb * R;
+        LayerActs& a = la[l];
+        d1 = GemmArgs();
+        d1.A = dres3 + r0 * C; d1.lda = C; dgrad_b(d1, P_FCPROJW, l, C, 4 * C);
+        d1.C = dfch + r0 * 4 * C; d1.ldc = 4 * C; d1.aux = a.fchd + r0 * 4 * C; d1.ldaux = 4 * C;
+        d1.M = (int)R; d1.N = 4 * C; d1.K = C; d1.epi = EPI_BF16_MUL;
+        fcb_rows = gemm_colsum_rows(d1, fp8());
+        d1.colsum_part = sg_rows(l, sg_fcb) + (long long)mb * fcb_rows * 4 * C;
+        if (!(last_cls_on() && lc_bwd >= 2 && l == L - 1 && T >= 128 && R >= 256 && dgrad_wt)) return false;
+        GemmArgs g = d1;
+        g.M = Bm; g.lda = (long long)T * C; g.ldc = (long long)T * 4 * C; g.ldaux = (long long)T * 4 * C;
+        g.rows_gathered = true; g.colsum_row_period = T;
+        if (!gemm_colsum_period_ok(g) || gemm_colsum_rows(g, false) != fcb_rows) return false;
+        if (!gemm_bf16_kskip(wgrad_args(dfch, 4 * C, a.ln2, C, G(P_FCW, l), T))) return false;
+        d1 = g;
+        return true;
+    }
     void last_cls_clear() {
         if (!lc_dirty) return;
         hipStream_t cs = s;
@@ -948,6 +987,12 @@
         }
         VIT_HIP(hipMemsetAsync(dln_bf, 0, (size_t)BT * C * 2, cs));
         VIT_HIP(hipMemsetAsync(datty, 0, (size_t)BT * C * 2, cs));
+        GemmArgs d1;
+        lc_d1_clean = lc_d1_gathered(L - 1, 0, dres_bf, d1);
+        if (lc_d1_clean) {
+            VIT_HIP(hipMemsetAsync(sg_rows(L - 1, sg_fcb), 0, (size_t)nmb * fcb_rows * 4 * C * sizeof(float), cs));
+            clear_cls_blocks_k<<<dim3(8, B), 256, 0, cs>>>(dfch, T, BT, 4 * C);
+        }
         if (cs != s) {
             VIT_HIP(hipEventRecord(bev[EV_LC], cs));
             lc_pending = true;
@@ -1130,13 +1175,8 @@
     }
 
     void wgrad(int cls, const bf16_t* dout, int OC, const bf16_t* inp, int Cin, float* dW, int ready,
-               int done, const QMat* dout_c = nullptr, const QMat* inp_c = nullptr) {
-        GemmArgs w;
-        w.A = dout; w.lda = OC; w.a_kcontig = false;
-        w.B = inp; w.ldb = Cin; w.b_kcontig = false;
-        w.C = dW; w.ldc = Cin; w.M = OC; w.N = Cin; w.K = (int)BT; w.epi = EPI_F32_ATOMIC;
-        w.ws = gemm_ws; w.ws_bytes = gemm_ws_bytes;
-        w.fill_pct = two_streams ? 0 : 80;
+               int done, const QMat* dout_c = nullptr, const QMat* inp_c = nullptr, int k_period = 0) {
+        GemmArgs w = wgrad_args(dout, OC, inp, Cin, dW, k_period);
         hipStream_t st = two_streams ? s2 : s;
         if (two_streams) {
             for (int mb = 0; mb < nmb; mb++) {
@@ -1201,6 +1241,8 @@
         pre_side_wait();
         last_cls_wait();
         lc_dirty = true;
+        const bool d1_clean = lc_d1_clean;
+        lc_d1_clean = false;
         bf16_t* rbA = dres_bf;
         bf16_t* rbB = dres_bf2;
         uint8_t* loA = dres_lo;
@@ -1218,21 +1260,26 @@
             const int Mr = lc ? Bm : (int)R;
             const long long rs = lc ? T : 1;
             const bool lcg = lc && R >= 256;
+            const int kper = lc && lc_bwd >= 1 ? T : 0;
             const bool rc = rowcol_on();
             QMat c_ln1 = rc ? actc_of(0, l) : QMat{}, c_atty = rc ? actc_of(1, l) : QMat{}, c_ln2 = rc ? actc_of(2, l) : QMat{};
             const bool lbm = lnbmx_on(), resa_pre = lbm && l < L - 1;
             const bool ec = epicol_on();
             QMat c_fchg = ec ? fchgc_of(l) : QMat{};
-            if (!rc) wgrad(TC_FCPROJ_WGRAD, rbA, C, a.fchg, 4 * C, G(P_FCPROJW, l), EV_RESA, EV_W1);
+            if (!rc) wgrad(TC_FCPROJ_WGRAD, rbA, C, a.fchg, 4 * C, G(P_FCPROJW, l), EV_RESA, EV_W1, nullptr, nullptr, kper);
             for (int mb = 0; mb < nmb; mb++) {
                 const long long r0 = mb * R;
                 after_wgrad(EV_W2, ms[mb]);
-                GemmArgs d1;
-                d1.A = rbA + r0 * C; d1.lda = C; dgrad_b(d1, P_FCPROJW, l, C, 4 * C);
-                d1.C = dfch + r0 * 4 * C; d1.ldc = 4 * C; d1.aux = a.fchd + r0 * 4 * C; d1.ldaux = 4 * C;
-                d1.M = (int)R; d1.N = 4 * C; d1.K = C; d1.epi = EPI_BF16_MUL;
-                fcb_rows = gemm_colsum_rows(d1, fp8());
-                d1.colsum_part = sg_rows(l, sg_fcb) + (long long)mb * fcb_rows * 4 * C;
+                GemmArgs d1, d1g;
+                if (lc && d1_clean && !ec && lc_d1_gathered(l, mb, rbA, d1g)) {
+                    d1 = d1g;
+                } else {
+                    d1.A = rbA + r0 * C; d1.lda = C; dgrad_b(d1, P_FCPROJW, l, C, 4 * C);
+                    d1.C = dfch + r0 * 4 * C; d1.ldc = 4 * C; d1.aux = a.fchd + r0 * 4 * C; d1.ldaux = 4 * C;
+                    d1.M = (int)R; d1.N = 4 * C; d1.K = C; d1.epi = EPI_BF16_MUL;
+                    fcb_rows = gemm_colsum_rows(d1, fp8());
+                    d1.colsum_part = sg_rows(l, sg_fcb) + (long long)mb * fcb_rows * 4 * C;
+                }
                 if (ec) {
                     d1.C = nullptr;
                     d1.mxc_q = dfchc.q; d1.mxc_s = dfchc.s; d1.mxc_ld = kp_tok; d1.mxc_off = r0;
@@ -1244,7 +1291,7 @@
             if (rc) wgrad(TC_FCPROJ_WGRAD, rbA, C, a.fchg, 4 * C, G(P_FCPROJW, l), EV_RESA, EV_W1, &dcol[0],
                           ec ? &c_fchg : nullptr);
             wgrad(TC_FC_WGRAD, dfch, 4 * C, a.ln2, C, G(P_FCW, l), EV_DFCH, EV_W2, ec ? &dfchc : nullptr,
-                  rc ? &c_ln2 : nullptr);
+                  rc ? &c_ln2 : nullptr, kper);
             for (int mb = 0; mb < nmb; mb++) {
                 const long long r0 = mb * R;
                 GemmArgs d2;
@@ -1270,7 +1317,7 @@
                 }
                 tend();
             }
-            if (!rc) wgrad(TC_PROJ_WGRAD, rbB, C, a.atty, C, G(P_ATTPROJW, l), EV_RESB, EV_W3);
+            if (!rc) wgrad(TC_PROJ_WGRAD, rbB, C, a.atty, C, G(P_ATTPROJW, l), EV_RESB, EV_W3, nullptr, nullptr, kper);
             for (int mb = 0; mb < nmb; mb++) {
                 const long long r0 = mb * R;
                 GemmArgs d3;
@@ -2254,11 +2301,15 @@
     for (int k = 0; k < vit::Trainer::MAXMB; k++) if (t.ms[k]) VIT_HIP(hipStreamSynchronize(t.ms[k]));
     t.two_streams = on != 0;
     t.nmb = t.pick_nmb(t.mb_want);
+    t.lc_dirty = true;
+    t.lc_d1_clean = false;
     return vit::has_error();
 }
 int vit_trainer_set_option(vit_trainer_t* h, const char* name, int value) {
     auto& t = h->t;
     VIT_HIP(hipDeviceSynchronize());
+    t.lc_dirty = true;
+    t.lc_d1_clean = false;
     const std::string n = name ? name : "";
     if (n == "microbatch") {
         t.mb_want = value;
@@ -2284,6 +2335,8 @@
         t.clip_overlap = value < 0 ? -1 : value != 0;
     } else if (n == "last_cls") {
         t.last_cls = value != 0;
+    } else if (n == "last_cls_bwd") {
+        t.lc_bwd = value < 0 ? 0 : value;
     } else if (n == "dp_probe") {
         if (value && !t.dp_snap) {
             t.dp_snap = t.alloc<float>(t.arena_elems);
```
